# nkwangyh/CubemapSLAM

Hardware: AMD Instinct MI355X
Metric: frames/sec (extract+match+localBA) on Lafida cam0 (higher is better)
Workload: dtype u8 (extract/match), f64 (BA)

## Files before the change

cubemapslam_amd/api.py:

```python
import time
import ctypes as C
import os
import numpy as np

_HERE = os.path.dirname(os.path.abspath(__file__))
LIB_PATH = os.environ.get("CMS_HIP_LIB") or os.path.join(_HERE, "lib", "libcubemapslam_hip.so")


class CmsError(RuntimeError):
    pass


class Camera(C.Structure):
    _fields_ = [("c", C.c_double), ("d", C.c_double), ("e", C.c_double), ("u0", C.c_double), ("v0", C.c_double),
                ("invpol", C.c_double * 12), ("pol", C.c_double * 5), ("Iw", C.c_int), ("Ih", C.c_int),
                ("face", C.c_int), ("fov_deg", C.c_double)]


class OrbParams(C.Structure):
    _fields_ = [("nfeatures", C.c_int), ("scale_factor", C.c_float), ("nlevels", C.c_int),
                ("ini_th_fast", C.c_int), ("min_th_fast", C.c_int)]


class Geometry(C.Structure):
    _fields_ = [("W", C.c_int), ("F", C.c_int), ("nlevels", C.c_int), ("kp_cap", C.c_int), ("max_batch", C.c_int),
                ("level_w", C.c_int * 12), ("level_h", C.c_int * 12), ("level_quota", C.c_int * 12),
                ("level_cells", C.c_int * 12), ("scale", C.c_float * 12), ("inv_scale", C.c_float * 12),
                ("sigma2", C.c_float * 12), ("inv_sigma2", C.c_float * 12), ("pyramid_bytes_per_frame", C.c_size_t),
                ("candidate_entries_per_frame", C.c_size_t), ("fisheye_stride", C.c_int)]


class BaStats(C.Structure):
    _fields_ = [("iterations_done", C.c_int * 2), ("chi2_initial", C.c_double * 2), ("chi2_final", C.c_double * 2),
                ("lambda_final", C.c_double * 2), ("n_outliers_mid", C.c_int), ("n_outliers_final", C.c_int)]


KP_DTYPE = np.dtype([("x", "<f4"), ("y", "<f4"), ("size", "<f4"), ("angle", "<f4"), ("response", "<f4"),
                     ("octave", "<i4")])

_lib = None


def lib():
    global _lib
    if _lib is None:
        if not os.path.exists(LIB_PATH):
            raise CmsError("libcubemapslam_hip.so is missing -- build it with `python -m cubemapslam_amd.build` "
                           "(there is no CPU fallback)")
        L = C.CDLL(LIB_PATH)
        L.cms_last_error.restype = C.c_char_p
        for n in ("cms_ctx_stream", "cms_frames_input", "cms_ba_stream"):
            getattr(L, n).restype = C.c_void_p
            getattr(L, n).argtypes = [C.c_void_p]
        L.cms_ctx_create.argtypes = [C.c_void_p, C.c_int, C.c_void_p, C.c_void_p, C.c_int]
        L.cms_ctx_destroy.argtypes = [C.c_void_p]
        L.cms_ctx_destroy.restype = None
        L.cms_ctx_geometry.argtypes = [C.c_void_p, C.c_void_p]
        L.cms_remap.argtypes = [C.c_void_p, C.c_void_p, C.c_int, C.c_void_p, C.c_int]
        L.cms_set_mask.argtypes = [C.c_void_p, C.c_void_p, C.c_int]
        L.cms_extract.argtypes = [C.c_void_p, C.c_void_p, C.c_int, C.c_void_p, C.c_void_p, C.c_int, C.c_void_p]
        L.cms_remap_extract.argtypes = [C.c_void_p, C.c_void_p, C.c_int, C.c_void_p, C.c_void_p, C.c_int, C.c_void_p]
        L.cms_frames_upload.argtypes = [C.c_void_p, C.c_void_p, C.c_int, C.c_size_t, C.c_int]
        L.cms_frames_upload_async.argtypes = [C.c_void_p, C.c_void_p, C.c_int, C.c_size_t, C.c_int]
        L.cms_frames_upload_wait.argtypes = [C.c_void_p]
        L.cms_frames_upload_device.argtypes = [C.c_void_p, C.c_void_p, C.c_int]
        L.cms_frames_process_device.argtypes = [C.c_void_p, C.c_void_p, C.c_int]
        L.cms_host_alloc.argtypes = [C.c_void_p, C.c_size_t]
        L.cms_host_free.argtypes = [C.c_void_p]
        L.cms_host_free.restype = None
        L.cms_ba_profile_kernel.argtypes = [C.c_void_p, C.c_int]
        L.cms_ba_profile_get.argtypes = [C.c_void_p, C.c_void_p, C.c_void_p]
        L.cms_ba_debug_compose.argtypes = [C.c_int, C.c_void_p, C.c_int, C.c_int, C.c_void_p, C.c_void_p, C.c_int, C.c_void_p, C.c_void_p, C.c_void_p, C.c_void_p]
        L.cms_frames_process.argtypes = [C.c_void_p, C.c_int, C.c_int]
        L.cms_frames_sync.argtypes = [C.c_void_p]
        L.cms_frames_results.argtypes = [C.c_void_p, C.c_void_p, C.c_void_p, C.c_void_p]
        L.cms_frames_fetch.argtypes = [C.c_void_p, C.c_int, C.c_void_p, C.c_void_p, C.c_int, C.c_void_p]
        L.cms_debug_lut.argtypes = [C.c_void_p, C.c_void_p, C.c_void_p]
        L.cms_debug_cubemap.argtypes = [C.c_void_p, C.c_int, C.c_void_p, C.c_int]
        L.cms_debug_level.argtypes = [C.c_void_p, C.c_int, C.c_int, C.c_void_p, C.c_int]
        L.cms_debug_candidates.argtypes = [C.c_void_p, C.c_int, C.c_int, C.c_void_p, C.c_int, C.c_void_p]
        L.cms_debug_distributed.argtypes = [C.c_void_p, C.c_int, C.c_int, C.c_void_p, C.c_int, C.c_void_p]
        L.cms_profile_enable.argtypes = [C.c_void_p, C.c_int]
        L.cms_profile_get.argtypes = [C.c_void_p, C.c_void_p]
        L.cms_hamming_best2.argtypes = [C.c_void_p, C.c_void_p, C.c_int, C.c_void_p, C.c_int] + [C.c_void_p] * 9
        L.cms_hamming_best2_device.argtypes = [C.c_void_p, C.c_void_p, C.c_void_p, C.c_int] + [C.c_void_p] * 10
        L.cms_hamming_matrix.argtypes = [C.c_void_p, C.c_void_p, C.c_int, C.c_void_p, C.c_int, C.c_void_p]
        L.cms_ba_create.argtypes = [C.c_void_p, C.c_int, C.c_int, C.c_void_p, C.c_void_p, C.c_int, C.c_void_p, C.c_int,
                                    C.c_void_p, C.c_void_p, C.c_void_p, C.c_void_p, C.c_void_p, C.c_double, C.c_double,
                                    C.c_double, C.c_double]
        L.cms_ba_reset.argtypes = [C.c_void_p]
        L.cms_ba_optimize.argtypes = [C.c_void_p, C.c_int, C.c_int, C.c_void_p, C.c_void_p]
        L.cms_ba_read.argtypes = [C.c_void_p, C.c_void_p, C.c_void_p, C.c_void_p]
        L.cms_ba_destroy.argtypes = [C.c_void_p]
        L.cms_ba_destroy.restype = None
        L.cms_ba_run.argtypes = [C.c_int, C.c_int, C.c_void_p, C.c_void_p, C.c_int, C.c_void_p, C.c_int, C.c_void_p,
                                 C.c_void_p, C.c_void_p, C.c_void_p, C.c_void_p, C.c_double, C.c_double, C.c_double,
                                 C.c_double, C.c_int, C.c_int, C.c_void_p, C.c_void_p, C.c_void_p]
        L.cms_ba_linearize.argtypes = [C.c_int, C.c_int, C.c_void_p, C.c_void_p, C.c_int, C.c_void_p, C.c_int, C.c_void_p,
                                       C.c_void_p, C.c_void_p, C.c_void_p, C.c_void_p, C.c_double, C.c_double, C.c_double,
                                       C.c_double, C.c_int, C.c_double] + [C.c_void_p] * 7
        L.cms_area_set_keypoints.argtypes = [C.c_void_p, C.c_int, C.c_int, C.c_void_p]
        L.cms_area_grid.argtypes = [C.c_void_p, C.c_int]
        L.cms_features_in_area.argtypes = [C.c_void_p, C.c_int, C.c_int] + [C.c_void_p] * 7 + [C.c_int, C.c_void_p]
        L.cms_features_in_area_device.argtypes = [C.c_void_p, C.c_int, C.c_int] + [C.c_void_p] * 8 + [C.c_int, C.c_int, C.c_void_p]
        L.cms_features_in_area_batch_device.argtypes = [C.c_void_p, C.c_int] + [C.c_void_p] * 9 + [C.c_int, C.c_void_p]
        L.cms_area_set_descriptors.argtypes = [C.c_void_p, C.c_int, C.c_int, C.c_void_p]
        L.cms_search_local_points.argtypes = ([C.c_void_p, C.c_int, C.c_void_p, C.c_int] + [C.c_void_p] * 5 + [C.c_float] * 3 + [C.c_int, C.c_int] +
                                              [C.c_void_p] * 9)
        L.cms_search_by_projection.argtypes = ([C.c_void_p, C.c_int, C.c_void_p, C.c_int] + [C.c_void_p] * 5 + [C.c_float, C.c_int, C.c_int, C.c_int] +
                                               [C.c_void_p] * 3)
        L.cms_project_last_frame_device.argtypes = [C.c_void_p, C.c_int] + [C.c_void_p] * 5 + [C.c_float] + [C.c_void_p] * 5
        L.cms_rotation_filter_device.argtypes = [C.c_void_p, C.c_int] + [C.c_void_p] * 5 + [C.c_int]
        L.cms_is_in_frustum_device.argtypes = [C.c_void_p, C.c_int] + [C.c_void_p] * 6 + [C.c_float, C.c_float] + [C.c_void_p] * 8
        L.cms_search_local_points_device.argtypes = [C.c_void_p, C.c_int] + [C.c_void_p] * 5 + [C.c_float, C.c_int] + [C.c_void_p] * 3
        L.cms_create_new_map_points.argtypes = [C.c_void_p, C.c_int, C.c_void_p, C.c_void_p, C.c_void_p, C.c_int, C.c_int] + [C.c_void_p] * 5
        L.cms_kfstore_create.argtypes = [C.c_void_p, C.c_void_p, C.c_int, C.c_int, C.c_int]
        L.cms_kfstore_destroy.argtypes = [C.c_void_p]
        L.cms_kfstore_destroy.restype = None
        L.cms_kfstore_put.argtypes = [C.c_void_p, C.c_int, C.c_void_p]
        L.cms_kfstore_update.argtypes = [C.c_void_p, C.c_int] + [C.c_void_p] * 5
        L.cms_kfstore_fuse_search.argtypes = [C.c_void_p, C.c_int] + [C.c_void_p] * 8 + [C.c_float, C.c_void_p, C.c_void_p]
        L.cms_kfstore_fuse_search_sets.argtypes = [C.c_void_p, C.c_int] + [C.c_void_p] * 6 + [C.c_int] + [C.c_void_p] * 3 + [C.c_float, C.c_void_p, C.c_void_p]
        L.cms_kfstore_put_from_frame.argtypes = [C.c_void_p, C.c_int, C.c_void_p, C.c_int, C.c_int, C.c_void_p, C.c_void_p, C.c_void_p, C.c_float, C.c_void_p, C.c_int,
                                                 C.c_void_p, C.c_void_p, C.c_void_p]
        L.cms_kfstore_update_poses.argtypes = [C.c_void_p, C.c_int] + [C.c_void_p] * 4
        L.cms_kfstore_debug_fetch.argtypes = [C.c_void_p, C.c_int] + [C.c_void_p] * 12
        L.cms_ba_debug_fetch_plan.argtypes = [C.c_void_p] * 14
        L.cms_kfstore_create_new_map_points.argtypes = [C.c_void_p, C.c_int, C.c_void_p, C.c_void_p, C.c_void_p, C.c_int, C.c_int] + [C.c_void_p] * 5
        L.cms_distinctive_descriptors.argtypes = [C.c_void_p, C.c_int, C.c_void_p, C.c_void_p, C.c_void_p]
        L.cms_update_normal_and_depth.argtypes = [C.c_void_p, C.c_int] + [C.c_void_p] * 8
        L.cms_fuse_search.argtypes = [C.c_void_p, C.c_int, C.c_void_p, C.c_int] + [C.c_void_p] * 6 + [C.c_float, C.c_void_p, C.c_void_p]
        L.cms_pose_create.argtypes = [C.c_void_p, C.c_int, C.c_int, C.c_int]
        L.cms_pose_destroy.argtypes = [C.c_void_p]
        L.cms_pose_destroy.restype = None
        L.cms_pose_stream.argtypes = [C.c_void_p]
        L.cms_pose_stream.restype = C.c_void_p
        _edge = [C.c_void_p] * 5 + [C.c_double] * 4
        L.cms_pose_upload.argtypes = [C.c_void_p, C.c_int] + _edge + [C.c_void_p]
        L.cms_pose_launch.argtypes = [C.c_void_p]
        L.cms_pose_fetch.argtypes = [C.c_void_p, C.c_void_p, C.c_void_p, C.c_void_p, C.c_void_p]
        L.cms_pose_optimize_batch.argtypes = [C.c_void_p, C.c_int] + _edge + [C.c_void_p] * 4
        L.cms_pose_optimize.argtypes = [C.c_int, C.c_int] + [C.c_void_p] * 4 + [C.c_double] * 4 + [C.c_void_p] * 4
        _lib = L
    return _lib


def _p(a):
    if a is None:
        return None
    if isinstance(a, int):
        return C.c_void_p(a)
    return a.ctypes.data_as(C.c_void_p)


def _chk(rc, what):
    if rc < 0:
        raise CmsError("%s failed (%d): %s" % (what, rc, lib().cms_last_error().decode()))
    return rc


class _Handle:
    _entries = None

    def _create(self, *args, out_last=False):
        self.h = C.c_void_p()
        args = args + (C.byref(self.h),) if out_last else (C.byref(self.h),) + args
        _chk(getattr(lib(), self._entries[0])(*args), self._entries[0])

    def close(self):
        if getattr(self, "h", None):
            getattr(lib(), self._entries[1])(self.h)
            self.h = C.c_void_p()

    def __del__(self):
        try:
            self.close()
        except Exception:
            pass


def make_camera(d):
    cam = Camera()
    for k in ("c", "d", "e", "u0", "v0", "Iw", "Ih", "face", "fov_deg"):
        setattr(cam, k, d[k])
    for i in range(12):
        cam.invpol[i] = d["invpol"][i] if i < len(d["invpol"]) else 0.0
    for i in range(5):
        cam.pol[i] = d["pol"][i] if i < len(d["pol"]) else 0.0
    return cam


RT_DTYPE = np.dtype([(n, "<u2") for n in ("tx", "ty", "x0", "y0", "nd", "rows", "flags", "pad")])
RT_LDS_MAX = 32768


def remap_lut_host(cam):
    cam = make_camera(cam) if isinstance(cam, dict) else cam
    W = 3 * cam.face
    out = np.zeros((W, (W + 3) // 4 * 4), np.uint32)
    f = lib().cms_remap_lut_host
    f.argtypes = [C.c_void_p, C.c_void_p, C.c_int]
    _chk(f(C.byref(cam), _p(out), out.shape[1]), "cms_remap_lut_host")
    return out[:, :W]


def remap_tiles_host(cam, lut, tile_w, tile_h, lds_budget=RT_LDS_MAX):
    cam = make_camera(cam) if isinstance(cam, dict) else cam
    lut = np.ascontiguousarray(lut, np.uint32)
    W = 3 * cam.face
    cap = ((W + tile_w - 1) // tile_w) * ((W + tile_h - 1) // tile_h)
    out = np.zeros(cap, RT_DTYPE)
    n_live, n_all, lds = C.c_int(), C.c_int(), C.c_int()
    f = lib().cms_remap_tiles_host
    f.argtypes = [C.c_void_p, C.c_void_p] + [C.c_int] * 4 + [C.c_void_p, C.c_int] + [C.c_void_p] * 3
    _chk(f(C.byref(cam), _p(lut), lut.strides[0] // 4, tile_w, tile_h, lds_budget, _p(out), cap, C.byref(n_live), C.byref(n_all), C.byref(lds)),
         "cms_remap_tiles_host")
    return out[:n_all.value].copy(), n_live.value, lds.value


def fast_cells_host(cam, which, nfeatures=2000, scale_factor=1.2, nlevels=8, ini_th=20, min_th=7):
    cam = make_camera(cam) if isinstance(cam, dict) else cam
    orb = OrbParams(nfeatures, scale_factor, nlevels, ini_th, min_th)
    f = lib().cms_fast_cells_host
    f.argtypes = [C.c_void_p, C.c_void_p, C.c_int, C.c_void_p, C.c_int, C.c_void_p]
    n = C.c_int()
    _chk(f(C.byref(cam), C.byref(orb), which, None, 0, C.byref(n)), "cms_fast_cells_host")
    out = np.zeros(max(n.value, 1), np.int32)
    _chk(f(C.byref(cam), C.byref(orb), which, _p(out), len(out), C.byref(n)), "cms_fast_cells_host")
    out = out[:n.value]
    return out & 15, (out >> 4) & 255, (out >> 12) & 255


class Context(_Handle):
    _entries = ("cms_ctx_create", "cms_ctx_destroy")

    def __init__(self, cam, nfeatures=2000, scale_factor=1.2, nlevels=8, ini_th=20, min_th=7, max_batch=1, device=0):
        self.cam = make_camera(cam) if isinstance(cam, dict) else cam
        self.orb = OrbParams(nfeatures, scale_factor, nlevels, ini_th, min_th)
        self._create(device, C.byref(self.cam), C.byref(self.orb), max_batch)
        self.geom = Geometry()
        _chk(lib().cms_ctx_geometry(self.h, C.byref(self.geom)), "cms_ctx_geometry")
        self.W = self.geom.W
        self.max_batch = max_batch

    @property
    def stream(self):
        return lib().cms_ctx_stream(self.h)

    def set_mask(self, mask):
        mask = np.ascontiguousarray(mask, np.uint8)
        _chk(lib().cms_set_mask(self.h, _p(mask), mask.strides[0]), "cms_set_mask")

    def set_distance_bounds_mode(self, scaled):
        f = lib().cms_set_distance_bounds_mode
        f.argtypes = [C.c_void_p, C.c_int]
        _chk(f(self.h, int(scaled)), "cms_set_distance_bounds_mode")

    def set_gaussian_mode(self, column_mode):
        f = lib().cms_set_gaussian_mode
        f.argtypes = [C.c_void_p, C.c_int]
        _chk(f(self.h, int(column_mode)), "cms_set_gaussian_mode")

    def remap(self, fisheye, cubemap=None):
        fisheye = np.ascontiguousarray(fisheye, np.uint8)
        if cubemap is None:
            cubemap = np.zeros((self.W, self.W), np.uint8)
        _chk(lib().cms_remap(self.h, _p(fisheye), fisheye.strides[0], _p(cubemap), cubemap.strides[0]), "cms_remap")
        return cubemap

    def extract(self, cubemap, cap=None):
        cubemap = np.ascontiguousarray(cubemap, np.uint8)
        cap = cap or self.geom.kp_cap
        kps = np.zeros(cap, KP_DTYPE)
        desc = np.zeros((cap, 32), np.uint8)
        n = C.c_int()
        _chk(lib().cms_extract(self.h, _p(cubemap), cubemap.strides[0], _p(kps), _p(desc), cap, C.byref(n)), "cms_extract")
        return kps[:n.value].copy(), desc[:n.value].copy()

    def remap_extract(self, fisheye, cap=None):
        fisheye = np.ascontiguousarray(fisheye, np.uint8)
        cap = cap or self.geom.kp_cap
        kps = np.zeros(cap, KP_DTYPE)
        desc = np.zeros((cap, 32), np.uint8)
        n = C.c_int()
        _chk(lib().cms_remap_extract(self.h, _p(fisheye), fisheye.strides[0], _p(kps), _p(desc), cap, C.byref(n)), "cms_remap_extract")
        return kps[:n.value].copy(), desc[:n.value].copy()

    def remap_extract_rays(self, fisheye, cap=None):
        fisheye = np.ascontiguousarray(fisheye, np.uint8)
        cap = cap or self.geom.kp_cap
        kps = np.zeros(cap, KP_DTYPE); desc = np.zeros((cap, 32), np.uint8); rays = np.zeros((cap, 3), np.float32)
        n = C.c_int()
        _chk(lib().cms_remap_extract_rays(self.h, _p(fisheye), fisheye.strides[0], _p(kps), _p(desc), _p(rays), cap, C.byref(n)), "cms_remap_extract_rays")
        return kps[:n.value].copy(), desc[:n.value].copy(), rays[:n.value].copy()

    def fetch_rays(self, b):
        cap = self.geom.kp_cap
        rays = np.zeros((cap, 3), np.float32)
        n = C.c_int()
        _chk(lib().cms_frames_fetch_rays(self.h, b, _p(rays), cap, C.byref(n)), "cms_frames_fetch_rays")
        return rays[:n.value].copy()

    def rays_ptr(self):
        a = C.c_void_p()
        _chk(lib().cms_frames_rays(self.h, C.byref(a)), "cms_frames_rays")
        return a.value

    def upload(self, frames):
        frames = np.ascontiguousarray(frames, np.uint8)
        assert frames.ndim == 3
        _chk(lib().cms_frames_upload(self.h, _p(frames), frames.strides[1], frames.strides[0], frames.shape[0]), "cms_frames_upload")

    def upload_async(self, frames):
        assert frames.ndim == 3 and frames.dtype == np.uint8 and frames.flags.c_contiguous
        _chk(lib().cms_frames_upload_async(self.h, _p(frames), frames.strides[1], frames.strides[0], frames.shape[0]), "cms_frames_upload_async")

    def upload_device(self, d_ptr, B):
        _chk(lib().cms_frames_upload_device(self.h, C.c_void_p(int(d_ptr)), B), "cms_frames_upload_device")

    def process_device(self, d_ptr, B):
        _chk(lib().cms_frames_process_device(self.h, C.c_void_p(int(d_ptr)), B), "cms_frames_process_device")

    def stream_wait_extracted(self, hip_stream):
        f = lib().cms_stream_wait_extracted
        f.argtypes = [C.c_void_p, C.c_void_p]
        _chk(f(self.h, C.c_void_p(int(hip_stream))), "cms_stream_wait_extracted")

    def upload_wait(self):
        _chk(lib().cms_frames_upload_wait(self.h), "cms_frames_upload_wait")

    def process(self, B, from_fisheye=True):
        _chk(lib().cms_frames_process(self.h, B, 1 if from_fisheye else 0), "cms_frames_process")

    def sync(self):
        _chk(lib().cms_frames_sync(self.h), "cms_frames_sync")

    def fetch(self, b):
        cap = self.geom.kp_cap
        kps = np.zeros(cap, KP_DTYPE)
        desc = np.zeros((cap, 32), np.uint8)
        n = C.c_int()
        _chk(lib().cms_frames_fetch(self.h, b, _p(kps), _p(desc), cap, C.byref(n)), "cms_frames_fetch")
        return kps[:n.value].copy(), desc[:n.value].copy()

    def results_ptrs(self):
        a, b, c = C.c_void_p(), C.c_void_p(), C.c_void_p()
        _chk(lib().cms_frames_results(self.h, C.byref(a), C.byref(b), C.byref(c)), "cms_frames_results")
        return a.value, b.value, c.value

    def input_ptr(self):
        return lib().cms_frames_input(self.h)

    def profile(self, on=True):
        lib().cms_profile_enable(self.h, 1 if on else 0)

    def profile_ms(self):
        ms = np.zeros(7, np.float32)
        _chk(lib().cms_profile_get(self.h, _p(ms)), "cms_profile_get")
        return dict(zip(("remap", "pyramid", "fast", "octree", "cull", "describe", "total"), ms.tolist()))

    def debug_lut(self):
        W = self.W
        out = np.zeros((W, (W + 3) // 4 * 4), np.uint32)
        s = C.c_int()
        _chk(lib().cms_debug_lut(self.h, _p(out), C.byref(s)), "cms_debug_lut")
        return out[:, :W]

    def debug_level(self, b, l):
        w, h = self.geom.level_w[l], self.geom.level_h[l]
        out = np.zeros((h, w), np.uint8)
        _chk(lib().cms_debug_level(self.h, b, l, _p(out), w), "cms_debug_level")
        return out

    def debug_candidates(self, b, l):
        cap = self.geom.level_w[l] * self.geom.level_h[l] // 4 + 4096
        out = np.zeros((cap, 3), np.int32)
        n = C.c_int()
        _chk(lib().cms_debug_candidates(self.h, b, l, _p(out), cap, C.byref(n)), "cms_debug_candidates")
        return out[:n.value].copy()

    def debug_distributed(self, b, l):
        cap = self.geom.level_quota[l] + 8
        out = np.zeros((cap, 3), np.int32)
        n = C.c_int()
        _chk(lib().cms_debug_distributed(self.h, b, l, _p(out), cap, C.byref(n)), "cms_debug_distributed")
        return out[:n.value].copy()

    def hamming_best2(self, qdesc, tdesc, cand_off, cand_idx, tlevel=None, texcl=None):
        qdesc = np.ascontiguousarray(qdesc, np.uint8); tdesc = np.ascontiguousarray(tdesc, np.uint8)
        cand_off = np.ascontiguousarray(cand_off, np.int32); cand_idx = np.ascontiguousarray(cand_idx, np.int32)
        tl = np.ascontiguousarray(tlevel, np.int32) if tlevel is not None else None
        tx = np.ascontiguousarray(texcl, np.uint8) if texcl is not None else None
        nq = len(qdesc)
        outs = [np.zeros(max(nq, 1), np.int32) for _ in range(5)]
        _chk(lib().cms_hamming_best2(self.h, _p(qdesc), nq, _p(tdesc), len(tdesc), _p(cand_off), _p(cand_idx), _p(tl), _p(tx),
                                     *[_p(o) for o in outs]), "cms_hamming_best2")
        keys = ("best_idx", "best_dist", "best_level", "second_dist", "second_level")
        return {k: o[:nq] for k, o in zip(keys, outs)}

    def area_set_keypoints(self, b, kps):
        kps = np.ascontiguousarray(kps, KP_DTYPE)
        _chk(lib().cms_area_set_keypoints(self.h, b, len(kps), _p(kps)), "cms_area_set_keypoints")

    def area_grid(self, B):
        _chk(lib().cms_area_grid(self.h, B), "cms_area_grid")

    def features_in_area(self, b, qx, qy, qr, qmin, qmax, cap=None):
        qx = np.ascontiguousarray(qx, np.float32); qy = np.ascontiguousarray(qy, np.float32); qr = np.ascontiguousarray(qr, np.float32)
        qmin = np.ascontiguousarray(qmin, np.int32); qmax = np.ascontiguousarray(qmax, np.int32)
        nq = len(qx)
        cap = cap or max(1, 64 * nq + 1024)
        off = np.zeros(nq + 1, np.int32); idx = np.zeros(cap, np.int32); tot = C.c_int(0)
        _chk(lib().cms_features_in_area(self.h, b, nq, _p(qx), _p(qy), _p(qr), _p(qmin), _p(qmax), _p(off), _p(idx), cap, C.byref(tot)),
             "cms_features_in_area")
        return off, idx[:tot.value]

    def features_in_area_device(self, b, nq, d_q5, d_cnt, d_off, d_idx, cap, idx_base, d_total):
        _chk(lib().cms_features_in_area_device(self.h, b, nq, *[C.c_void_p(int(a)) for a in d_q5], C.c_void_p(int(d_cnt)), C.c_void_p(int(d_off)),
                                               C.c_void_p(int(d_idx)), cap, idx_base, C.c_void_p(int(d_total))), "cms_features_in_area_device")

    def features_in_area_batch_device(self, nq, d_qframe, d_q5, d_cnt, d_off, d_idx, cap, d_total):
        _chk(lib().cms_features_in_area_batch_device(self.h, nq, C.c_void_p(int(d_qframe)), *[C.c_void_p(int(a)) for a in d_q5], C.c_void_p(int(d_cnt)),
                                                     C.c_void_p(int(d_off)), C.c_void_p(int(d_idx)), cap, C.c_void_p(int(d_total))),
             "cms_features_in_area_batch_device")

    def area_set_descriptors(self, b, desc):
        desc = np.ascontiguousarray(desc, np.uint8)
        _chk(lib().cms_area_set_descriptors(self.h, b, len(desc), _p(desc)), "cms_area_set_descriptors")

    def search_local_points(self, b, pose15, pos, normal, min_dist, max_dist, mp_desc, kp_mp, viewing_cos_limit=0.5, th=1.0, nnratio=0.8,
                            th_high=100):
        pose15 = np.ascontiguousarray(pose15, np.float32).reshape(15)
        pos = np.ascontiguousarray(pos, np.float32).reshape(-1, 3); normal = np.ascontiguousarray(normal, np.float32).reshape(-1, 3)
        n = len(pos)
        min_dist = np.ascontiguousarray(min_dist, np.float32); max_dist = np.ascontiguousarray(max_dist, np.float32)
        mp_desc = np.ascontiguousarray(mp_desc, np.uint8).reshape(n, 32)
        assert kp_mp.dtype == np.int32 and kp_mp.flags.c_contiguous
        vis = np.zeros(n, np.uint8); px = np.zeros(n, np.float32); py = np.zeros(n, np.float32); lvl = np.zeros(n, np.int32)
        vc = np.zeros(n, np.float32); match = np.full(n, -1, np.int32)
        nm = C.c_int(0); rounds = C.c_int(0)
        _chk(lib().cms_search_local_points(self.h, b, _p(pose15), n, _p(pos), _p(normal), _p(min_dist), _p(max_dist), _p(mp_desc),
                                           viewing_cos_limit, th, nnratio, th_high, len(kp_mp), _p(kp_mp), _p(vis), _p(px), _p(py), _p(lvl),
                                           _p(vc), _p(match), C.addressof(nm), C.addressof(rounds)), "cms_search_local_points")
        return dict(in_view=vis, proj_x=px, proj_y=py, level=lvl, view_cos=vc, match=match, n_matches=nm.value, rounds=rounds.value)

    def search_by_projection(self, b, pose12, valid, Xw, octave, angle, mp_desc, kp_mp, th=15.0, check_ori=True, th_high=100):
        a = [np.ascontiguousarray(pose12, np.float32), np.ascontiguousarray(valid, np.uint8), np.ascontiguousarray(Xw, np.float32),
             np.ascontiguousarray(octave, np.int32), np.ascontiguousarray(angle, np.float32), np.ascontiguousarray(mp_desc, np.uint8)]
        n = len(a[1])
        match = np.full(n, -1, np.int32); nm = C.c_int(0)
        assert kp_mp.dtype == np.int32
        _chk(lib().cms_search_by_projection(self.h, b, _p(a[0]), n, *[_p(v) for v in a[1:]], th, int(check_ori), th_high, len(kp_mp), _p(kp_mp), _p(match),
                                            C.addressof(nm)), "cms_search_by_projection")
        return match, nm.value

    def search_by_projection_keyframe(self, b, pose12, kf_angle, pos, min_dist, max_dist, mp_desc, kp_mp, th=10.0, orb_dist=100, check_ori=True):
        a = [np.ascontiguousarray(pose12, np.float32).reshape(12), np.ascontiguousarray(kf_angle, np.float32), np.ascontiguousarray(pos, np.float32).reshape(-1, 3),
             np.ascontiguousarray(min_dist, np.float32), np.ascontiguousarray(max_dist, np.float32), np.ascontiguousarray(mp_desc, np.uint8).reshape(-1, 32)]
        n = len(a[1])
        assert all(len(v) == n for v in a[2:])
        assert kp_mp.dtype == np.int32 and kp_mp.flags.c_contiguous
        match = np.full(max(n, 1), -1, np.int32); nm = C.c_int(0)
        L = lib()
        L.cms_search_by_projection_keyframe.argtypes = ([C.c_void_p, C.c_int, C.c_void_p, C.c_int] + [C.c_void_p] * 5 + [C.c_float, C.c_int, C.c_int, C.c_int] +
                                                        [C.c_void_p] * 3)
        _chk(L.cms_search_by_projection_keyframe(self.h, b, _p(a[0]), n, *[_p(v) for v in a[1:]], float(th), int(orb_dist), int(check_ori), len(kp_mp), _p(kp_mp),
                                                 _p(match), C.addressof(nm)), "cms_search_by_projection_keyframe")
        return match[:n], nm.value

    def search_for_initialization(self, b2, k1, d1, prev_matched, window=100, nnratio=0.9, check_ori=True):
        k1 = np.ascontiguousarray(k1, KP_DTYPE); d1 = np.ascontiguousarray(d1, np.uint8)
        assert prev_matched.dtype == np.float32 and prev_matched.flags.c_contiguous and prev_matched.shape == (len(k1), 2)
        m12 = np.full(max(len(k1), 1), -1, np.int32); nm = C.c_int(0)
        f = lib().cms_search_for_initialization
        f.argtypes = [C.c_void_p, C.c_int, C.c_int, C.c_void_p, C.c_void_p, C.c_void_p, C.c_int, C.c_float, C.c_int, C.c_void_p, C.c_void_p]
        _chk(f(self.h, b2, len(k1), _p(k1), _p(d1), _p(prev_matched), int(window), float(nnratio), int(check_ori), _p(m12), C.addressof(nm)),
             "cms_search_for_initialization")
        return m12[:len(k1)], nm.value

    def project_last_frame_device(self, n, d_qframe, d_pose12, d_valid, d_Xw, d_oct, th, d_q5):
        v = lambda a: C.c_void_p(int(a)) if a else None
        _chk(lib().cms_project_last_frame_device(self.h, n, v(d_qframe), v(d_pose12), v(d_valid), v(d_Xw), v(d_oct), th, *[v(a) for a in d_q5]),
             "cms_project_last_frame_device")

    def rotation_filter_device(self, B, d_mp_off, d_last_angle, d_kp_mp, d_mp_match, d_n_matches, check_orientation=True):
        v = lambda a: C.c_void_p(int(a)) if a else None
        _chk(lib().cms_rotation_filter_device(self.h, B, v(d_mp_off), v(d_last_angle), v(d_kp_mp), v(d_mp_match), v(d_n_matches), int(check_orientation)),
             "cms_rotation_filter_device")

    def is_in_frustum_device(self, nmp, d_mp_frame, d_pose15, d_pos, d_normal, d_min, d_max, viewing_cos_limit, th, d_outs5, d_q3):
        v = lambda a: C.c_void_p(int(a)) if a else None
        _chk(lib().cms_is_in_frustum_device(self.h, nmp, v(d_mp_frame), v(d_pose15), v(d_pos), v(d_normal), v(d_min), v(d_max),
                                            viewing_cos_limit, th, *[v(a) for a in d_outs5], *[v(a) for a in d_q3]), "cms_is_in_frustum_device")

    def search_local_points_device(self, B, d_mp_off, d_mp_desc, d_cand_off, d_cand_idx, d_pair_dist, nnratio, th_high, d_kp_mp, d_mp_match,
                                   d_rounds=0):
        v = lambda a: C.c_void_p(int(a)) if a else None
        _chk(lib().cms_search_local_points_device(self.h, B, v(d_mp_off), v(d_mp_desc), v(d_cand_off), v(d_cand_idx), v(d_pair_dist), nnratio,
                                                  th_high, v(d_kp_mp), v(d_mp_match), v(d_rounds)), "cms_search_local_points_device")

    def hamming_best2_device(self, qdesc, q_row, nq, tdesc, cand_off, cand_idx, t_level, t_excl, outs):
        _chk(lib().cms_hamming_best2_device(self.h, _p(qdesc), _p(q_row), nq, _p(tdesc), _p(cand_off), _p(cand_idx), _p(t_level),
                                            _p(t_excl), *[_p(o) for o in outs]), "cms_hamming_best2_device")

    def hamming_matrix(self, a, b):
        a = np.ascontiguousarray(a, np.uint8); b = np.ascontiguousarray(b, np.uint8)
        out = np.zeros((len(a), len(b)), np.uint16)
        _chk(lib().cms_hamming_matrix(self.h, _p(a), len(a), _p(b), len(b), _p(out)), "cms_hamming_matrix")
        return out


    def compute_bow(self, vocab, rows, n, levelsup=4):
        rows = np.ascontiguousarray(rows, np.int32); n = np.ascontiguousarray(n, np.int32)
        assert len(rows) == len(n)
        L = lib()
        L.cms_frames_compute_bow.argtypes = [C.c_void_p, C.c_void_p, C.c_int, C.c_int, C.c_void_p, C.c_void_p]
        _chk(L.cms_frames_compute_bow(self.h, vocab.h, int(levelsup), len(rows), _p(rows), _p(n)), "cms_frames_compute_bow")

    def fetch_bow(self, b):
        L = lib()
        L.cms_frames_fetch_bow.argtypes = [C.c_void_p, C.c_int, C.c_void_p, C.c_void_p, C.c_void_p, C.c_int, C.c_void_p, C.c_void_p, C.c_void_p, C.c_void_p, C.c_int, C.c_int]
        nw, nn = C.c_int(), C.c_int()
        cap = self.geom.kp_cap
        o = _bow_arrays(cap, cap, cap)
        _chk(L.cms_frames_fetch_bow(self.h, b, C.byref(nw), _p(o["word_id"]), _p(o["word_val"]), len(o["word_id"]), C.byref(nn), _p(o["node_id"]), _p(o["node_off"]),
                                    _p(o["node_feat"]), len(o["node_id"]), cap), "cms_frames_fetch_bow")
        return _bow_trim(o, nw.value, nn.value)


class PinnedArray:

    def __init__(self, shape):
        n = int(np.prod(shape))
        self.p = C.c_void_p()
        _chk(lib().cms_host_alloc(C.byref(self.p), n), "cms_host_alloc")
        self.array = np.ctypeslib.as_array((C.c_uint8 * n).from_address(self.p.value)).reshape(shape)

    def close(self):
        if self.p:
            self.array = None
            lib().cms_host_free(self.p)
            self.p = None

    def __del__(self):
        try:
            self.close()
        except Exception:
            pass


class Keyframe(C.Structure):
    _fields_ = [("n", C.c_int), ("kps", C.c_void_p), ("desc", C.c_void_p), ("rays", C.c_void_p), ("mp", C.c_void_p),
                ("Rcw", C.c_float * 9), ("tcw", C.c_float * 3), ("Ow", C.c_float * 3),
                ("nnodes", C.c_int), ("node_id", C.c_void_p), ("node_off", C.c_void_p), ("node_feat", C.c_void_p), ("median_depth", C.c_float)]


def make_keyframe(kf):
    n = len(kf["x"])
    kps = np.zeros(n, KP_DTYPE); kps["x"] = kf["x"]; kps["y"] = kf["y"]; kps["octave"] = kf["octave"]; kps["angle"] = kf["angle"]
    keep = [kps, np.ascontiguousarray(kf["desc"], np.uint8), np.ascontiguousarray(kf["rays"], np.float32), np.ascontiguousarray(kf["mp"], np.int32),
            np.ascontiguousarray(kf["node_id"], np.int32), np.ascontiguousarray(kf["node_off"], np.int32), np.ascontiguousarray(kf["node_feat"], np.int32)]
    K = Keyframe()
    K.n = n; K.kps = keep[0].ctypes.data; K.desc = keep[1].ctypes.data; K.rays = keep[2].ctypes.data; K.mp = keep[3].ctypes.data
    K.Rcw[:] = [float(v) for v in np.asarray(kf["R"], np.float32).reshape(9)]
    K.tcw[:] = [float(v) for v in kf["t"]]; K.Ow[:] = [float(v) for v in kf["Ow"]]
    K.nnodes = len(keep[4]); K.node_id = keep[4].ctypes.data; K.node_off = keep[5].ctypes.data; K.node_feat = keep[6].ctypes.data
    K.median_depth = float(kf["median_depth"])
    return K, keep


def search_for_triangulation(ctx, K1, K2, E12=None, check_orientation=False):
    m = np.full(max(K1.n, 1), -1, np.int32)
    n = C.c_int()
    e = None if E12 is None else np.ascontiguousarray(E12, np.float32)
    lib().cms_search_for_triangulation.argtypes = [C.c_void_p, C.c_void_p, C.c_void_p, C.c_void_p, C.c_int, C.c_void_p, C.c_void_p]
    _chk(lib().cms_search_for_triangulation(ctx.h, C.byref(K1), C.byref(K2), _p(e) if e is not None else None, int(check_orientation), _p(m), C.byref(n)),
         "cms_search_for_triangulation")
    return m[:K1.n].copy(), n.value


def create_new_map_points(ctx, jobs, check_orientation=False, cap=None):
    nj = len(jobs)
    cur = (Keyframe * max(nj, 1))(*[j[0] for j in jobs])
    flat = [k for j in jobs for k in j[1]]
    neigh = (Keyframe * max(len(flat), 1))(*flat)
    off = np.concatenate([[0], np.cumsum([len(j[1]) for j in jobs])]).astype(np.int32)
    cap = cap if cap is not None else max([j[0].n for j in jobs] + [1])
    n_new = np.zeros(max(nj, 1), np.int32)
    on = np.zeros((max(nj, 1), cap), np.int32); o1 = np.zeros_like(on); o2 = np.zeros_like(on); ox = np.zeros((max(nj, 1), cap, 3), np.float32)
    _chk(lib().cms_create_new_map_points(ctx.h, nj, C.addressof(cur), _p(off), C.addressof(neigh), int(check_orientation), cap, _p(n_new), _p(on), _p(o1),
                                         _p(o2), _p(ox)), "cms_create_new_map_points")
    return [(on[j, :n_new[j]].copy(), o1[j, :n_new[j]].copy(), o2[j, :n_new[j]].copy(), ox[j, :n_new[j]].copy()) for j in range(nj)]


class BowJob(C.Structure):
    _fields_ = [("slot", C.c_int), ("b", C.c_int), ("n", C.c_int), ("nnodes", C.c_int), ("node_id", C.c_void_p), ("node_off", C.c_void_p),
                ("node_feat", C.c_void_p), ("kf_skip", C.c_void_p)]


class BowKfJob(C.Structure):
    _fields_ = [("slot1", C.c_int), ("n1", C.c_int), ("slot2", C.c_int), ("n2", C.c_int), ("skip1", C.c_void_p), ("skip2", C.c_void_p)]


class Sim3SearchJob(C.Structure):
    _fields_ = [("slot1", C.c_int), ("n1", C.c_int), ("slot2", C.c_int), ("n2", C.c_int), ("s12", C.c_float), ("R12", C.c_float * 9), ("t12", C.c_float * 3),
                ("off1", C.c_int), ("off2", C.c_int)]


class Sim3ProjJob(C.Structure):
    _fields_ = [("slot", C.c_int), ("n", C.c_int), ("Scw", C.c_float * 12), ("set", C.c_int)]


class KfProjJob(C.Structure):
    _fields_ = [("slot", C.c_int), ("b", C.c_int), ("n", C.c_int), ("pose12", C.c_float * 12), ("nmp", C.c_int), ("kf_feat", C.c_void_p), ("pos", C.c_void_p),
                ("min_dist", C.c_void_p), ("max_dist", C.c_void_p), ("mp_desc", C.c_void_p), ("kp_mp", C.c_void_p), ("match", C.c_void_p)]


class KfdbJob(C.Structure):
    _fields_ = [("mode", C.c_int), ("group", C.c_int), ("query", C.c_int), ("b", C.c_int), ("slot", C.c_int), ("nwords", C.c_int), ("word_id", C.c_void_p),
                ("word_val", C.c_void_p), ("min_score", C.c_float), ("n_connected", C.c_int), ("connected", C.c_void_p)]


KFDB_RELOC, KFDB_LOOP = 0, 1
KFDB_QUERY = {"row": 0, "slot": 1, "words": 2}


def kfdb_jobs(jobs):
    arr = (KfdbJob * max(len(jobs), 1))()
    keep = []
    for q, j in zip(arr, jobs):
        form = j["query"]
        q.mode = int(j["mode"]); q.group = int(j.get("group", 0)); q.query = KFDB_QUERY[form[0]]
        if form[0] == "row":
            q.b = int(form[1])
        elif form[0] == "slot":
            q.slot = int(form[1])
        else:
            ids = np.ascontiguousarray(form[1], np.int32); vals = np.ascontiguousarray(form[2], np.float64)
            assert len(ids) == len(vals)
            keep += [ids, vals]
            q.nwords = len(ids); q.word_id = ids.ctypes.data if len(ids) else None; q.word_val = vals.ctypes.data if len(ids) else None
        conn = np.ascontiguousarray(j.get("connected", ()), np.int32)
        keep.append(conn)
        q.min_score = float(j.get("min_score", 0.0)); q.n_connected = len(conn); q.connected = conn.ctypes.data if len(conn) else None
    return arr, keep


def kfdb_results(njobs, K, cap, cand, n_cand, common, score):
    return [([int(c) for c in cand[j, :min(int(n_cand[j]), cap)]], common[j].copy(), score[j].view(np.uint32).copy()) for j in range(njobs)]


def _bow_fv(fv):
# ... 1219 lines not shown
```

cubemapslam_amd/csrc/cms_api_area.hip:

```cpp
#include <vector>

static int cms_area_grid_attr(int device) {
  static bool done[64] = {false};
  return cms_lds_ceiling_once((const void*)k_area_grid, (CMS_AREA_MAXKP + 1) * 8, device, done);
}
static int cms_area_reserve(cms_ctx* c) {
  if (c->d_area_sorted) return CMS_OK;
  if (c->g.kp_cap > CMS_AREA_MAXKP) return cms_fail(CMS_ERR_UNSUPPORTED, "frame grid: more than 16383 key points per frame");
  { const int rca = cms_area_grid_attr(c->device); if (rca) return rca; }
  const size_t B = (size_t)c->max_batch;
  HIPCHK(hipMalloc((void**)&c->d_area_sorted, B * c->g.kp_cap * sizeof(uint16_t)));
  HIPCHK(hipMalloc((void**)&c->d_area_cell_start, B * (CMS_AREA_CELLS + 1) * sizeof(int)));
  HIPCHK(hipMalloc((void**)&c->d_area_nvalid, B * sizeof(int)));
  return CMS_OK;
}

static int cms_area_tmp_reserve(cms_ctx* c, int nq) {
  if ((size_t)nq <= c->area_tmp_cap) return CMS_OK;
  if (c->d_area_tmp) hipFree(c->d_area_tmp);
  c->d_area_tmp = nullptr; c->area_tmp_cap = 0;
  const size_t cap = (size_t)nq + (size_t)nq / 4 + 1024;
  HIPCHK(hipMalloc((void**)&c->d_area_tmp, cap * CMS_AREA_TMP * sizeof(int)));
  c->area_tmp_cap = cap;
  return CMS_OK;
}
static int cms_area_psum_reserve(cms_ctx* c, int nparts) {
  if (nparts <= c->area_psum_cap) return CMS_OK;
  if (c->d_area_psum) hipFree(c->d_area_psum);
  c->d_area_psum = nullptr; c->area_psum_cap = 0;
  const int cap = nparts + nparts / 4 + 64;
  HIPCHK(hipMalloc((void**)&c->d_area_psum, (size_t)cap * sizeof(int)));
  c->area_psum_cap = cap;
  return CMS_OK;
}

static CmsAreaArgs cms_area_args(const CmsKeyPoint* kp, const uint16_t* sorted_idx, const int* cell_start, int kp_cap, int F, float inv) {
  CmsAreaArgs a = {};
  a.kp = kp; a.sorted_idx = sorted_idx; a.cell_start = cell_start; a.kp_cap = kp_cap; a.F = F; a.inv = inv;
  return a;
}
static CmsAreaArgs cms_area_args_frames(const cms_ctx* c, int b) {
  return cms_area_args((const CmsKeyPoint*)c->d_kps + (size_t)b * c->g.kp_cap, c->d_area_sorted + (size_t)b * c->g.kp_cap,
                       c->d_area_cell_start + (size_t)b * (CMS_AREA_CELLS + 1), c->g.kp_cap, c->g.F, cms_grid_inv(c));
}
static void cms_area_queries(CmsAreaArgs& a, int nq, const void* q_frame, const void* qx, const void* qy, const void* qr, const void* qmin, const void* qmax,
                             void* cnt, void* off, void* idx, int cap, int idx_base) {
  a.nq = nq; a.q_frame = (const int*)q_frame;
  a.qx = (const float*)qx; a.qy = (const float*)qy; a.qr = (const float*)qr; a.qmin = (const int*)qmin; a.qmax = (const int*)qmax;
  a.cnt = (int*)cnt; a.off = (int*)off; a.idx = (int*)idx; a.cap = cap; a.idx_base = idx_base;
}
struct CmsWindowCols {
  size_t o0 = 0, stride = 0;
  float *qx, *qy, *qr; int *qmin, *qmax, *level, *slot, *rec, *cnt, *off, *idx;
  void take(CmsBlock& b, size_t E) {
    o0 = b.size; stride = cms_align(E * 4);
    for (int k = 0; k < 9; ++k) b.take(E * 4);
    b.take(E * 4, 4);
  }
  void at(uint8_t* p, size_t o_idx) {
    float* f = (float*)(p + o0); int* i = (int*)(p + o0);
    const size_t n = stride / 4;
    qx = f; qy = f + n; qr = f + 2 * n; qmin = i + 3 * n; qmax = i + 4 * n; level = i + 5 * n; slot = i + 6 * n; rec = i + 7 * n; cnt = i + 8 * n; off = i + 9 * n;
    idx = (int*)(p + o_idx);
  }
};
static void cms_area_queries(CmsAreaArgs& a, int nq, const CmsWindowCols& w, int cap) {
  cms_area_queries(a, nq, w.slot, w.qx, w.qy, w.qr, w.qmin, w.qmax, w.cnt, w.off, w.idx, cap, 0);
}
static int cms_area_launch(cms_ctx* c, hipStream_t s, CmsAreaArgs a, void* d_total) {
  const int nq = a.nq, qgrid = cms_area_search_grid(nq);
  int rc = cms_area_psum_reserve(c, qgrid);
  if (rc) return rc;
  rc = cms_area_tmp_reserve(c, nq);
  if (rc) return rc;
  a.tmp = c->d_area_tmp; a.psum = c->d_area_psum;
  hipLaunchKernelGGL(k_area_query, dim3(qgrid), dim3(CMS_AREA_QT), 0, s, a);
  hipLaunchKernelGGL(k_area_lists, dim3(cms_area_tile_grid(nq)), dim3(CMS_AREA_LT), 0, s, a, (int*)d_total);
  HIPCHK(hipGetLastError());
  return CMS_OK;
}

extern "C" int cms_area_set_keypoints(cms_ctx* c, int b, int n, const cms_keypoint* kps) {
  if (!c || b < 0 || b >= c->max_batch || n < 0 || n > c->g.kp_cap || (n > 0 && !kps)) return cms_fail(CMS_ERR_ARG, "cms_area_set_keypoints: bad argument");
  HIPCHK(hipSetDevice(c->device));
  if (n > 0) HIPCHK(hipMemcpyAsync(c->d_kps + (size_t)b * c->g.kp_cap, kps, (size_t)n * sizeof(cms_keypoint), hipMemcpyHostToDevice, c->stream));
  HIPCHK(hipMemcpyAsync(c->d_kp_cnt + b, &n, sizeof(int), hipMemcpyHostToDevice, c->stream));
  HIPCHK(hipStreamSynchronize(c->stream));
  return CMS_OK;
}

extern "C" int cms_area_grid(cms_ctx* c, int B) {
  if (!c || B < 1 || B > c->max_batch) return cms_fail(CMS_ERR_ARG, "cms_area_grid: bad batch");
  HIPCHK(hipSetDevice(c->device));
  int rc = cms_area_reserve(c);
  if (rc) return rc;
  hipLaunchKernelGGL(k_area_grid, dim3(B), dim3(1024), (size_t)(c->g.kp_cap + 1) * 8, c->stream, (const CmsKeyPoint*)c->d_kps, (const int*)c->d_kp_cnt, c->g.kp_cap, c->g.F, cms_grid_inv(c),
                     c->d_area_sorted, c->d_area_cell_start, c->d_area_nvalid);
  HIPCHK(hipGetLastError());
  c->area_frames = B;
  return CMS_OK;
}

extern "C" int cms_features_in_area_device(cms_ctx* c, int b, int nq, const void* d_qx, const void* d_qy, const void* d_qr, const void* d_qmin,
                                           const void* d_qmax, void* d_cnt_scratch, void* d_cand_off, void* d_cand_idx, int cap, int idx_base,
                                           void* d_total) {
  if (!c || b < 0 || b >= c->area_frames || nq < 0 || cap < 0) return cms_fail(CMS_ERR_ARG, "cms_features_in_area_device: bad argument (cms_area_grid first)");
  if (nq == 0) return CMS_OK;
  HIPCHK(hipSetDevice(c->device));
  CmsAreaArgs a = cms_area_args_frames(c, b);
  cms_area_queries(a, nq, nullptr, d_qx, d_qy, d_qr, d_qmin, d_qmax, d_cnt_scratch, d_cand_off, d_cand_idx, cap, idx_base);
  return cms_area_launch(c, c->stream, a, d_total);
}

extern "C" int cms_features_in_area_batch_device(cms_ctx* c, int nq, const void* d_qframe, const void* d_qx, const void* d_qy, const void* d_qr,
                                                 const void* d_qmin, const void* d_qmax, void* d_cnt_scratch, void* d_cand_off, void* d_cand_idx,
                                                 int cap, void* d_total) {
  if (!c || nq < 0 || cap < 0 || c->area_frames < 1 || !d_qframe) return cms_fail(CMS_ERR_ARG, "cms_features_in_area_batch_device: bad argument (cms_area_grid first)");
  if (nq == 0) return CMS_OK;
  HIPCHK(hipSetDevice(c->device));
  CmsAreaArgs a = cms_area_args_frames(c, 0);
  cms_area_queries(a, nq, d_qframe, d_qx, d_qy, d_qr, d_qmin, d_qmax, d_cnt_scratch, d_cand_off, d_cand_idx, cap, 0);
  return cms_area_launch(c, c->stream, a, d_total);
}

extern "C" int cms_features_in_area(cms_ctx* c, int b, int nq, const float* qx, const float* qy, const float* qr, const int* qmin, const int* qmax,
                                    int* cand_off, int* cand_idx, int cap, int* total) {
  if (!c || nq < 0 || cap < 0 || !cand_off || (nq > 0 && (!qx || !qy || !qr || !qmin || !qmax))) return cms_fail(CMS_ERR_ARG, "cms_features_in_area: bad argument");
  if (b < 0 || b >= c->area_frames) return cms_fail(CMS_ERR_ARG, "cms_features_in_area: no grid for this frame (cms_area_grid first)");
  cand_off[0] = 0;
  if (total) *total = 0;
  if (nq == 0) return CMS_OK;
  HIPCHK(hipSetDevice(c->device));
  const size_t qb = (size_t)nq * 4;
  const size_t bytes = 5 * qb + qb  + (qb + 4)  + (size_t)cap * 4 + 64;
  hipStream_t s = c->stream;
  int rc = c->stage.reserve(s, bytes, 0);
  if (rc) return rc;
  uint8_t* p = c->stage.d;
  void* dq[5];
  const void* hq[5] = {qx, qy, qr, qmin, qmax};
  for (int i = 0; i < 5; ++i) { dq[i] = p; p += qb; HIPCHK(hipMemcpyAsync(dq[i], hq[i], qb, hipMemcpyHostToDevice, s)); }
  void* d_cnt = p; p += qb;
  void* d_off = p; p += qb + 4;
  void* d_tot = p; p += 16;
  void* d_idx = p;
  rc = cms_features_in_area_device(c, b, nq, dq[0], dq[1], dq[2], dq[3], dq[4], d_cnt, d_off, d_idx, cap, 0, d_tot);
  if (rc) return rc;
  int tot = 0;
  HIPCHK(hipMemcpyAsync(cand_off, d_off, qb + 4, hipMemcpyDeviceToHost, s));
  HIPCHK(hipMemcpyAsync(&tot, d_tot, sizeof(int), hipMemcpyDeviceToHost, s));
  HIPCHK(hipStreamSynchronize(s));
  if (total) *total = tot;
  if (tot > cap) return cms_fail(CMS_ERR_OVERFLOW, "cms_features_in_area: candidate capacity too small");
  if (tot > 0 && cand_idx) HIPCHK(hipMemcpy(cand_idx, d_idx, (size_t)tot * 4, hipMemcpyDeviceToHost));
  return CMS_OK;
}
```

cubemapslam_amd/csrc/cms_api_frames.hip:

```cpp
#include <chrono>
#include <thread>
#include <hip/hip_runtime.h>
#include <math.h>
#include <stdio.h>
#include <stdlib.h>
#include <string.h>
#include <algorithm>
#include <string>
#include <vector>
#include "../../include/cubemapslam_hip.h"
#include "cms_types.h"
#include "cms_stage.h"
#include "orb_pattern.inc"

static bool cms_cu_mask_from_env(uint32_t* words, int* n_words) {
  const char* v = getenv("CMS_CTX_CU_MASK");
  if (!v || !*v) return false;
  int n = 0;
  while (*v && n < 8) {
    char* end = nullptr;
    words[n++] = (uint32_t)strtoul(v, &end, 16);
    if (end == v) return false;
    v = *end == ',' ? end + 1 : end;
    if (*end && *end != ',') return false;
  }
  *n_words = n;
  return n > 0;
}

struct CmsCtxBow;
static void cms_ctx_bow_free(CmsCtxBow* b);
static void cms_ctx_bow_invalidate(CmsCtxBow* b);

struct CmsHipMem;
using CmsStage = CmsStageT<CmsHipMem>;

static thread_local std::string g_cms_err;
static int cms_fail(int code, const char* what, hipError_t e = hipSuccess) {
  char buf[512];
  if (e != hipSuccess) snprintf(buf, sizeof(buf), "%s: %s", what, hipGetErrorString(e));
  else snprintf(buf, sizeof(buf), "%s", what);
  g_cms_err = buf;
  return code;
}
#define HIPCHK(call)                                                        \
  do {                                                                      \
    hipError_t _e = (call);                                                 \
    if (_e != hipSuccess) return cms_fail(CMS_ERR_HIP, #call, _e);          \
  } while (0)

extern "C" const char* cms_last_error(void) { return g_cms_err.c_str(); }
extern "C" int cms_device_count(void) {
  int n = 0;
  if (hipGetDeviceCount(&n) != hipSuccess) return 0;
  return n;
}

struct cms_ctx {
  int device = 0;
  cms_camera cam;
  cms_orb_params orb;
  int max_batch = 0;
  CmsGeom g;
  float scale[CMS_MAX_LEVELS], inv_scale[CMS_MAX_LEVELS], sigma2[CMS_MAX_LEVELS], inv_sigma2[CMS_MAX_LEVELS];
  hipStream_t stream = nullptr;
  int fstride = 0;
  size_t fish_pitch = 0;
  int lut_stride = 0, mstride = 0;
  bool have_mask = false;
  int dirty_frames = 0;
  uint8_t* d_fish = nullptr; uint32_t* d_lut = nullptr; uint8_t* d_pyr = nullptr; uint8_t* d_mask = nullptr;
  cms_remap_tile* d_rtiles = nullptr; int rt_mode = 1, rt_tw = 64, rt_live = 0, rt_all = 0, rt_lds = 0;
  CmsResizeTab* d_tab = nullptr; float* d_pattern = nullptr;
  uint32_t* d_cand = nullptr; uint16_t* d_node = nullptr; int* d_cand_cnt = nullptr; int* d_overflow = nullptr;
  uint32_t* d_qt_out = nullptr; int* d_qt_cnt = nullptr;
  uint32_t* d_cell_cand = nullptr; int* d_cell_cnt = nullptr;
  int* d_cells_all = nullptr; int* d_cells_live = nullptr; int n_cells_all = 0, n_cells_live = 0;
  uint16_t* d_area_sorted = nullptr; int* d_area_cell_start = nullptr; int* d_area_nvalid = nullptr; int area_frames = 0;
  int* d_area_psum = nullptr; int area_psum_cap = 0;
  int* d_area_tmp = nullptr; size_t area_tmp_cap = 0;
  uint8_t* h_fish_stage = nullptr; int fish_stage_frames = 0;
  hipStream_t copy_stream = nullptr; hipEvent_t ev_upload_done = nullptr, ev_remap_done = nullptr;
  bool upload_pending = false, remap_recorded = false;
  int dist_bounds_scaled = 0;
  hipEvent_t ev_block = nullptr; int last_batch = 0;
  hipEvent_t ev_extracted = nullptr; bool extracted_recorded = false;
  CmsKeyPoint* d_kps = nullptr; uint32_t* d_aux = nullptr; uint8_t* d_desc = nullptr; int* d_kp_cnt = nullptr;
  uint32_t* d_order = nullptr; uint32_t* d_aux_sorted = nullptr; int* d_walk_cnt = nullptr; float* d_rays = nullptr;
  CmsStage stage;
  bool prof = false;
  bool desc_spatial = false;
  hipEvent_t ev[8] = {nullptr, nullptr, nullptr, nullptr, nullptr, nullptr, nullptr, nullptr};
  size_t fast_lds = 0, qt_lds = 0;
  CmsCtxBow* bow = nullptr;
};

static inline double cms_horner12(const double* c, double x) {
  double r = 0.0;
  for (int i = 11; i >= 0; --i) r = r * x + c[i];
  return r;
}
static void cms_cubemap_to_fisheye(const cms_camera& cam, double up, double vp, double* uf, double* vf) {
  const int F = cam.face;
  const double half = F / 2.0;
  float i = (float)up, j = (float)vp;
  *uf = -1; *vf = -1;
  const float fi = i / (float)F, fj = j / (float)F;
  int face = CMS_FACE_UNKNOWN;
  if (fi >= 0 && fi < 1 && fj >= 1 && fj < 2) face = CMS_FACE_LEFT;
  else if (fi >= 1 && fi < 2 && fj >= 0 && fj < 1) face = CMS_FACE_UPPER;
  else if (fi >= 1 && fi < 2 && fj >= 1 && fj < 2) face = CMS_FACE_FRONT;
  else if (fi >= 1 && fi < 2 && fj >= 2 && fj < 3) face = CMS_FACE_LOWER;
  else if (fi >= 2 && fi < 3 && fj >= 1 && fj < 2) face = CMS_FACE_RIGHT;
  if (face == CMS_FACE_UNKNOWN) return;
  i = i - (float)((int)(i / (float)F) * F);
  j = j - (float)((int)(j / (float)F) * F);
  const double lx = ((double)i - half) * 1.0 / half, ly = ((double)j - half) * 1.0 / half, lz = 1.0;
  double x, y, z;
  switch (face) {
    case CMS_FACE_FRONT: x = lx; y = ly; z = lz; break;
    case CMS_FACE_LEFT: x = -lz; y = ly; z = lx; break;
    case CMS_FACE_RIGHT: x = lz; y = ly; z = -lx; break;
    case CMS_FACE_LOWER: x = lx; y = lz; z = -ly; break;
    default: x = lx; y = -lz; z = ly; break;
  }
  double norm = sqrt(x * x + y * y);
  if (norm == 0.0) norm = 1e-14;
  const double theta = atan(-z / norm);
  const double rho = cms_horner12(cam.invpol, theta);
  const double uu = x / norm * rho, vv = y / norm * rho;
  *uf = uu * cam.c + vv * cam.d + cam.u0;
  *vf = uu * cam.e + vv + cam.v0;
  if (*uf < 0 || *uf >= cam.Iw || *vf < 0 || *vf >= cam.Ih) { *uf = -1; *vf = -1; }
}
static void cms_build_lut(const cms_camera& cam, int lut_stride, std::vector<uint32_t>& lut) {
  const int W = 3 * cam.face;
  lut.assign((size_t)W * lut_stride, 0u);
  for (int y = 0; y < W; ++y)
    for (int x = 0; x < W; ++x) {
      double u, v;
      cms_cubemap_to_fisheye(cam, (double)x, (double)y, &u, &v);
      if (u < 0 || v < 0 || u >= cam.Iw || v >= cam.Ih) continue;
      const float mu = (float)u, mv = (float)v;
      const int sx = (int)lrint((double)(mu * 32.f)), sy = (int)lrint((double)(mv * 32.f));
      const uint32_t X = (uint32_t)(sx >> 5), Y = (uint32_t)(sy >> 5), ax = (uint32_t)(sx & 31), ay = (uint32_t)(sy & 31);
      lut[(size_t)y * lut_stride + x] = X | (Y << 11) | (ax << 22) | (ay << 27);
    }
}

extern "C" int cms_remap_lut_host(const cms_camera* cam, uint32_t* lut, int lut_stride) {
  if (!cam || !lut || cam->face < 1 || lut_stride < 3 * cam->face) return cms_fail(CMS_ERR_ARG, "cms_remap_lut_host: bad argument");
  std::vector<uint32_t> v;
  cms_build_lut(*cam, lut_stride, v);
  memcpy(lut, v.data(), v.size() * 4);
  return CMS_OK;
}
extern "C" int cms_remap_tiles_host(const cms_camera* cam, const uint32_t* lut, int lut_stride, int tile_w, int tile_h, int lds_budget,
                                    cms_remap_tile* out, int cap, int* n_live, int* n_all, int* lds_bytes) {
  if (!cam || !lut || !out || !n_live || !n_all || !lds_bytes || cam->face < 1 || lut_stride < 3 * cam->face || !cms_rt_shape_ok(tile_w, tile_h) || lds_budget < 0)
    return cms_fail(CMS_ERR_ARG, "cms_remap_tiles_host: bad argument");
  std::vector<cms_remap_tile> v;
  cms_rt_build(cam->face, lut, lut_stride, tile_w, tile_h, lds_budget, v, n_live, lds_bytes);
  *n_all = (int)v.size();
  if ((int)v.size() > cap) return cms_fail(CMS_ERR_OVERFLOW, "cms_remap_tiles_host: caller capacity too small");
  memcpy(out, v.data(), v.size() * sizeof(cms_remap_tile));
  return CMS_OK;
}

static inline short cms_sat_short(float v) {
  const long iv = lrint((double)v);
  return (short)(iv < -32768 ? -32768 : iv > 32767 ? 32767 : iv);
}
static void cms_resize_table(int sn, int dn, bool clamp_frac, CmsResizeTab* out) {
  const double inv_scale = (double)dn / sn, scale = 1. / inv_scale;
  for (int d = 0; d < dn; ++d) {
    float f = (float)((d + 0.5) * scale - 0.5);
    int s = (int)floorf(f);
    f -= s;
    if (clamp_frac) {
      if (s < 0) { f = 0; s = 0; }
      if (s >= sn - 1) { f = 0; s = sn - 1; }
    }
    out[d].s = (short)s;
    out[d].a0 = cms_sat_short((1.f - f) * 2048);
    out[d].a1 = cms_sat_short(f * 2048);
    out[d].pad = 0;
  }
}

#include "cms_api_util.h"

struct CmsLevelSetup {
  float scale[CMS_MAX_LEVELS], inv_scale[CMS_MAX_LEVELS], sigma2[CMS_MAX_LEVELS], inv_sigma2[CMS_MAX_LEVELS];
  size_t tab_off = 0;
  int maxq = 0, wCellMax = 0, hCellMax = 0;
};
static int cms_level_geometry(const cms_camera* cam, const cms_orb_params* orb, CmsGeom& g, CmsLevelSetup* x) {
  if (orb->nlevels < 1 || orb->nlevels > CMS_MAX_LEVELS) return cms_fail(CMS_ERR_UNSUPPORTED, "nlevels must be 1..12");
  if (cam->face < 32 || 3 * cam->face > 4095) return cms_fail(CMS_ERR_UNSUPPORTED, "face size must satisfy 32 <= F and 3F <= 4095");
  memset(&g, 0, sizeof(g));
  const int L = orb->nlevels, F = cam->face, W = 3 * F;
  float *scale = x->scale, *inv_scale = x->inv_scale, *sigma2 = x->sigma2, *inv_sigma2 = x->inv_sigma2;
  g.nlevels = L; g.W = W; g.F = F; g.ini_th = orb->ini_th_fast; g.min_th = orb->min_th_fast;
  const double scaleFactor = orb->scale_factor;
  scale[0] = 1.0f; sigma2[0] = 1.0f;
  for (int i = 1; i < L; ++i) { scale[i] = (float)(scale[i - 1] * scaleFactor); sigma2[i] = scale[i] * scale[i]; }
  for (int i = 0; i < L; ++i) { inv_scale[i] = 1.0f / scale[i]; inv_sigma2[i] = 1.0f / sigma2[i]; }
  {
    const float factor = (float)(1.0f / scaleFactor);
    float nDesired = orb->nfeatures * (1 - factor) / (1 - (float)pow((double)factor, (double)L));
    int sum = 0;
    for (int l = 0; l < L - 1; ++l) { g.lv[l].quota = (int)lrint((double)nDesired); sum += g.lv[l].quota; nDesired *= factor; }
    g.lv[L - 1].quota = orb->nfeatures - sum > 0 ? orb->nfeatures - sum : 0;
  }
  size_t off = 0, cand_off = 0; size_t& tab_off = x->tab_off;
  int cell0 = 0, kp_off = 0; int &maxq = x->maxq, &wCellMax = x->wCellMax, &hCellMax = x->hCellMax;
  for (int l = 0; l < L; ++l) {
    CmsLevel& lv = g.lv[l];
    lv.w = (int)lrint((double)((float)W * inv_scale[l]));
    lv.h = lv.w;
    if (lv.w < 2 * CMS_MINB + 30) { return cms_fail(CMS_ERR_UNSUPPORTED, "pyramid level too small for the FAST cell grid"); }
    lv.stride = (int)cms_align((size_t)lv.w + 8, 128);
    lv.off = off;
    off += cms_align((size_t)lv.stride * (lv.h + 1), 256);
    const float width = (float)(lv.w - 2 * CMS_MINB), height = (float)(lv.h - 2 * CMS_MINB);
    lv.nCols = (int)(width / 30.f); lv.nRows = (int)(height / 30.f);
    lv.wCell = (int)ceilf(width / lv.nCols); lv.hCell = (int)ceilf(height / lv.nRows);
    lv.cell0 = cell0; cell0 += lv.nCols * lv.nRows;
    lv.cand_cap = (lv.w * lv.h) / 4 + 4096;
    lv.cand_off = cand_off; cand_off += cms_align((size_t)lv.cand_cap, 64);
    lv.kp_off = kp_off; kp_off += lv.quota + 3;
    lv.scale = scale[l];
    lv.patch_size = (float)(int)(31 * scale[l]);
    lv.tab_off = tab_off; tab_off += (size_t)lv.w + lv.h;
    if (lv.quota > maxq) maxq = lv.quota;
    if (lv.wCell > wCellMax) wCellMax = lv.wCell;
    if (lv.hCell > hCellMax) hCellMax = lv.hCell;
// ... 742 lines not shown
```

cubemapslam_amd/csrc/cms_api_reloc.hip:

```cpp
#include <algorithm>
#include <cstring>
#include <vector>

namespace {
int reloc_run(cms_ctx* c, cms_kfstore* st, int njobs, const cms_kfproj_job* jobs, const float* kf_angle, float th, int orb_dist, int check_orientation,
              int* n_matches, const char* who) {
  const int kp_cap = c->g.kp_cap;
  std::vector<int> mp_off((size_t)njobs + 1, 0);
  for (int j = 0; j < njobs; ++j) mp_off[(size_t)j + 1] = mp_off[(size_t)j] + jobs[j].nmp;
  const int n = mp_off[(size_t)njobs];
  for (int j = 0; j < njobs; ++j) n_matches[j] = 0;
  if (n == 0) return CMS_OK;
  if (c->g.nlevels > 16) return cms_fail(CMS_ERR_UNSUPPORTED, "SearchByProjection (key frame): more than 16 pyramid levels");
  HIPCHK(hipSetDevice(c->device));
  hipStream_t s = c->stream;
  if (st) {
    const int rc = kfstore_wait_puts(st, s, njobs, [&](int j) { return jobs[j].slot; });
    if (rc) return rc;
  }
  const size_t n4 = (size_t)n * 4, j4 = (size_t)njobs * 4, kp4 = (size_t)kp_cap * 4;
  CmsBlock blk;
  const size_t o_pose = blk.take(12 * j4), o_jframe = blk.take(j4), o_jkp0 = blk.take(j4), o_mpoff = blk.take(j4, 4), o_ptjob = blk.take(n4), o_feat = blk.take(n4),
               o_pos = blk.take(3 * n4), o_min = blk.take(n4), o_max = blk.take(n4), o_desc = blk.take((size_t)n * 32), o_kpmp = blk.take(njobs * kp4);
  const size_t in_bytes = blk.size;
  const size_t o_match = blk.take(n4), o_nm = blk.take(j4), o_tot = blk.take(16);
  const size_t out_begin = o_kpmp, out_end = blk.size;
  const size_t o_qf = blk.take(n4), o_qx = blk.take(n4), o_qy = blk.take(n4), o_qr = blk.take(n4), o_qmin = blk.take(n4), o_qmax = blk.take(n4), o_ang = blk.take(n4),
               o_cnt = blk.take(n4), o_off = blk.take(n4, 4);
  const size_t o_idx = blk.size;
  return cms_retry_capacity(64 * n + 1024, who, [&](int cap, int& tot) -> int {
    const size_t o_pd = o_idx + cms_align((size_t)cap * 4);
    int rc = c->stage.reserve(s, o_pd + cms_align((size_t)cap * 2), out_end);
    if (rc) return rc;
    uint8_t* p = c->stage.d;
    uint8_t* h = c->stage.h;
    std::memcpy(h + o_mpoff, mp_off.data(), j4 + 4);
    for (int j = 0; j < njobs; ++j) {
      const cms_kfproj_job& q = jobs[j];
      const size_t m0 = (size_t)mp_off[(size_t)j], m = (size_t)q.nmp;
      std::memcpy(h + o_pose + 48 * (size_t)j, q.pose12, 48);
      reinterpret_cast<int*>(h + o_jframe)[j] = q.b;
      reinterpret_cast<int*>(h + o_jkp0)[j] = st ? st->h_kf[(size_t)q.slot].f0 : -1;
      int* km = reinterpret_cast<int*>(h + o_kpmp) + (size_t)j * kp_cap;
      for (int k = 0; k < kp_cap; ++k) km[k] = k < q.n ? q.kp_mp[k] : -1;
      if (m == 0) continue;
      int* pj = reinterpret_cast<int*>(h + o_ptjob) + m0;
      for (size_t k = 0; k < m; ++k) pj[k] = j;
      std::memcpy(h + o_feat + 4 * m0, st ? (const void*)q.kf_feat : (const void*)kf_angle, 4 * m);
      std::memcpy(h + o_pos + 12 * m0, q.pos, 12 * m); std::memcpy(h + o_min + 4 * m0, q.min_dist, 4 * m); std::memcpy(h + o_max + 4 * m0, q.max_dist, 4 * m);
      std::memcpy(h + o_desc + 32 * m0, q.mp_desc, 32 * m);
    }
    rc = c->stage.up(s, in_bytes, who);
    if (rc) return rc;
    CmsProjectKfArgs a = {};
    a.n = n; a.pt_job = (const int*)(p + o_ptjob); a.pose12 = (const float*)(p + o_pose); a.job_frame = (const int*)(p + o_jframe); a.job_kp0 = (const int*)(p + o_jkp0);
    a.kf_kp = st ? st->d_kp : nullptr; a.kf_feat = (const int*)(p + o_feat); a.kf_angle = (const float*)(p + o_feat);
    a.pos = (const float*)(p + o_pos); a.min_dist = (const float*)(p + o_min); a.max_dist = (const float*)(p + o_max);
    a.th = th; a.cos_fov = cms_cos_fov(c); a.log_scale = cms_log_scale(c); a.nlevels = c->g.nlevels; a.F = c->g.F;
    a.bounds_scaled = c->dist_bounds_scaled;
    cms_level_table(a.sf, c, c->scale, 0.0f);
    a.q_frame = (int*)(p + o_qf); a.qx = (float*)(p + o_qx); a.qy = (float*)(p + o_qy); a.qr = (float*)(p + o_qr); a.qmin = (int*)(p + o_qmin); a.qmax = (int*)(p + o_qmax);
    a.angle = (float*)(p + o_ang);
    hipLaunchKernelGGL(k_project_keyframe, dim3((n + 255) / 256), dim3(256), 0, s, a);
    HIPCHK(hipGetLastError());
    rc = cms_features_in_area_batch_device(c, n, p + o_qf, p + o_qx, p + o_qy, p + o_qr, p + o_qmin, p + o_qmax, p + o_cnt, p + o_off, p + o_idx, cap, p + o_tot);
    if (rc) return rc;
    CmsSearchLocalArgs g = track_search_local_args(c, p + o_mpoff, p + o_desc, p + o_off, p + o_idx, p + o_pd, (int*)(p + o_kpmp), p + o_match, nullptr, -1.0f, orb_dist, 0,
                                                   p + o_tot, cap);
    g.wg_frame = (const int*)(p + o_jframe);
    hipLaunchKernelGGL(k_search_local, dim3(njobs), dim3(1024), 0, s, g);
    CmsRotFilterArgs r = {};
    r.mp_off = g.mp_off; r.last_angle = (const float*)(p + o_ang); r.kp = g.kp; r.kp_mp = g.kp_mp; r.mp_match = g.mp_match; r.n_matches = (int*)(p + o_nm);
    r.check_orientation = check_orientation; r.total = g.total; r.cap = cap; r.wg_frame = g.wg_frame; r.kp_cap = kp_cap;
    hipLaunchKernelGGL(k_rot_filter, dim3(njobs), dim3(1024), 0, s, r);
    HIPCHK(hipGetLastError());
    rc = c->stage.back_and_wait(s, out_begin, out_end, who);
    if (rc) return rc;
    tot = *reinterpret_cast<const int*>(h + o_tot);
    if (tot > cap) return CMS_OK;
    for (int j = 0; j < njobs; ++j) {
      const cms_kfproj_job& q = jobs[j];
      if (q.nmp == 0) continue;
      const int* km = reinterpret_cast<const int*>(h + o_kpmp) + (size_t)j * kp_cap;
      const int* rows = reinterpret_cast<const int*>(h + o_match) + mp_off[(size_t)j];
      if (q.n > 0) std::memcpy(q.kp_mp, km, (size_t)q.n * 4);
      track_rows_to_frame(c, q.b, q.nmp, rows, q.match);
      for (int k = 0; k < q.nmp; ++k) if (q.match[k] >= 0 && q.match[k] < q.n) q.kp_mp[q.match[k]] = k;
      n_matches[j] = reinterpret_cast<const int*>(h + o_nm)[j];
    }
    return CMS_OK;
  });
}
int reloc_check_job(const cms_ctx* c, const cms_kfproj_job& q, const char* who) {
  if (q.b < 0 || q.b >= c->area_frames) return cms_fail(CMS_ERR_ARG, (std::string(who) + ": no grid for this frame (cms_area_grid first)").c_str());
  if (q.n < 0 || q.n > c->g.kp_cap || q.nmp < 0 || (q.n > 0 && !q.kp_mp) || (q.nmp > 0 && (!q.pos || !q.min_dist || !q.max_dist || !q.mp_desc || !q.match)))
    return cms_fail(CMS_ERR_ARG, (std::string(who) + ": bad argument").c_str());
  return CMS_OK;
}
}

extern "C" int cms_kfstore_search_by_projection(cms_kfstore* st, cms_ctx* src, int njobs, const cms_kfproj_job* jobs, float th, int orb_dist, int check_orientation,
                                                int* n_matches) {
  const char* who = "cms_kfstore_search_by_projection";
  if (!st || !src || njobs < 0 || (njobs > 0 && (!jobs || !n_matches))) return cms_fail(CMS_ERR_ARG, "cms_kfstore_search_by_projection: bad argument");
  if (njobs == 0) return CMS_OK;
  if (src->device != st->c->device) return cms_fail(CMS_ERR_ARG, "cms_kfstore_search_by_projection: the frame context and the store must share the device");
  if (src->g.kp_cap > CMS_TRACK_KPMAX) return cms_fail(CMS_ERR_UNSUPPORTED, "cms_kfstore_search_by_projection: more than 4096 key points per frame");
  std::vector<uint8_t> row_named((size_t)std::max(src->area_frames, 1), 0);
  for (int j = 0; j < njobs; ++j) {
    const cms_kfproj_job& q = jobs[j];
    if (q.slot < 0 || q.slot >= st->maxkf || !st->used[(size_t)q.slot]) return cms_fail(CMS_ERR_ARG, "cms_kfstore_search_by_projection: empty slot");
    const int rc = reloc_check_job(src, q, who);
    if (rc) return rc;
    if (row_named[(size_t)q.b]) return cms_fail(CMS_ERR_ARG, "cms_kfstore_search_by_projection: two jobs name the same frame row");
    row_named[(size_t)q.b] = 1;
    if (q.nmp > 0 && !q.kf_feat) return cms_fail(CMS_ERR_ARG, "cms_kfstore_search_by_projection: bad argument");
    const int kn = st->h_kf[(size_t)q.slot].n;
    for (int k = 0; k < q.nmp; ++k) {
      if (q.kf_feat[k] < 0 || q.kf_feat[k] >= kn) return cms_fail(CMS_ERR_ARG, "cms_kfstore_search_by_projection: key-frame feature index out of range");
      if (k > 0 && q.kf_feat[k] <= q.kf_feat[k - 1]) return cms_fail(CMS_ERR_ARG, "cms_kfstore_search_by_projection: key-frame feature indices must ascend");
    }
  }
  return reloc_run(src, st, njobs, jobs, nullptr, th, orb_dist, check_orientation, n_matches, who);
}

extern "C" int cms_search_by_projection_keyframe(cms_ctx* c, int b, const float* pose12, int nmp, const float* kf_angle, const float* pos, const float* min_dist,
                                                 const float* max_dist, const uint8_t* mp_desc, float th, int orb_dist, int check_orientation, int nkp, int* kp_mp,
                                                 int* match, int* n_matches) {
  const char* who = "cms_search_by_projection_keyframe";
  if (!c || !pose12 || (nmp > 0 && !kf_angle)) return cms_fail(CMS_ERR_ARG, "cms_search_by_projection_keyframe: bad argument");
  if (c->g.kp_cap > CMS_TRACK_KPMAX) return cms_fail(CMS_ERR_UNSUPPORTED, "cms_search_by_projection_keyframe: more than 4096 key points per frame");
  cms_kfproj_job q = {};
  q.slot = -1; q.b = b; q.n = nkp; std::memcpy(q.pose12, pose12, 48); q.nmp = nmp; q.pos = pos; q.min_dist = min_dist; q.max_dist = max_dist; q.mp_desc = mp_desc; q.kp_mp = kp_mp; q.match = match;
  const int rc = reloc_check_job(c, q, who);
  if (rc) return rc;
  int nm = 0;
  const int rr = reloc_run(c, nullptr, 1, &q, kf_angle, th, orb_dist, check_orientation, &nm, who);
  if (n_matches) *n_matches = nm;
  return rr;
}
```

cubemapslam_amd/csrc/cms_api_track.hip:

```cpp
#include <cmath>
#include <vector>

extern "C" int cms_area_set_descriptors(cms_ctx* c, int b, int n, const uint8_t* desc) {
  if (!c || b < 0 || b >= c->max_batch || n < 0 || n > c->g.kp_cap || (n > 0 && !desc)) return cms_fail(CMS_ERR_ARG, "cms_area_set_descriptors: bad argument");
  HIPCHK(hipSetDevice(c->device));
  if (n > 0) HIPCHK(hipMemcpyAsync(c->d_desc + (size_t)b * c->g.kp_cap * 32, desc, (size_t)n * 32, hipMemcpyHostToDevice, c->stream));
  HIPCHK(hipStreamSynchronize(c->stream));
  return CMS_OK;
}

extern "C" int cms_set_distance_bounds_mode(cms_ctx* c, int scaled) {
  if (!c || scaled < 0 || scaled > 1) return cms_fail(CMS_ERR_ARG, "cms_set_distance_bounds_mode: mode must be 0 or 1");
  c->dist_bounds_scaled = scaled;
  return CMS_OK;
}

extern "C" int cms_is_in_frustum_device(cms_ctx* c, int nmp, const void* d_mp_frame, const void* d_pose15, const void* d_pos, const void* d_normal,
                                        const void* d_min_dist, const void* d_max_dist, float viewing_cos_limit, float th, void* d_in_view,
                                        void* d_proj_x, void* d_proj_y, void* d_level, void* d_view_cos, void* d_qr, void* d_qmin, void* d_qmax) {
  if (!c || nmp < 0 || (nmp > 0 && (!d_pose15 || !d_pos || !d_normal || !d_min_dist || !d_max_dist || !d_in_view || !d_proj_x || !d_proj_y ||
                                    !d_level || !d_view_cos)) || (d_qr && (!d_qmin || !d_qmax)))
    return cms_fail(CMS_ERR_ARG, "cms_is_in_frustum_device: bad argument");
  if (nmp == 0) return CMS_OK;
  if (c->g.nlevels > 16) return cms_fail(CMS_ERR_UNSUPPORTED, "cms_is_in_frustum_device: more than 16 pyramid levels");
  HIPCHK(hipSetDevice(c->device));
  CmsFrustumArgs a;
  a.pose15 = (const float*)d_pose15; a.mp_frame = (const int*)d_mp_frame; a.n = nmp;
  a.P = (const float*)d_pos; a.normal = (const float*)d_normal; a.min_dist = (const float*)d_min_dist; a.max_dist = (const float*)d_max_dist;
  a.viewing_cos_limit = viewing_cos_limit; a.th = th; a.bounds_scaled = c->dist_bounds_scaled;
  a.log_scale = cms_log_scale(c);
  a.nlevels = c->g.nlevels; a.F = c->g.F;
  cms_level_table(a.sf, c, c->scale, 0.0f);
  a.in_view = (uint8_t*)d_in_view; a.proj_x = (float*)d_proj_x; a.proj_y = (float*)d_proj_y; a.level = (int*)d_level; a.view_cos = (float*)d_view_cos;
  a.qr = (float*)d_qr; a.qmin = (int*)d_qmin; a.qmax = (int*)d_qmax;
  hipLaunchKernelGGL(k_in_frustum, dim3((nmp + 255) / 256), dim3(256), 0, c->stream, a);
  HIPCHK(hipGetLastError());
  return CMS_OK;
}

static CmsSearchLocalArgs track_search_local_args(const cms_ctx* c, const void* mp_off, const void* mp_desc, const void* cand_off, const void* cand_idx, void* pair_dist,
                                                  int* kp_mp, void* mp_match, void* rounds, float nnratio, int th_high, int frame0, const void* total, int cap) {
  CmsSearchLocalArgs a = {};
  a.mp_off = (const int*)mp_off; a.mp_desc = (const uint4*)mp_desc; a.cand_off = (const int*)cand_off; a.cand_idx = (const int*)cand_idx;
  a.t_desc = (const uint4*)c->d_desc; a.kp = (const CmsKeyPoint*)c->d_kps; a.kp_cap = c->g.kp_cap;
  a.pair_dist = (uint16_t*)pair_dist; a.kp_mp = kp_mp; a.mp_match = (int*)mp_match; a.rounds = (int*)rounds;
  a.nnratio = nnratio; a.th_high = th_high; a.frame0 = frame0; a.total = (const int*)total; a.cap = cap;
  return a;
}

extern "C" int cms_search_local_points_device(cms_ctx* c, int B, const void* d_mp_off, const void* d_mp_desc, const void* d_cand_off,
                                              const void* d_cand_idx, void* d_pair_dist, float nnratio, int th_high, void* d_kp_mp,
                                              void* d_mp_match, void* d_rounds) {
  if (!c || B < 1 || B > c->area_frames || !d_mp_off || !d_mp_desc || !d_cand_off || !d_cand_idx || !d_pair_dist || !d_kp_mp || !d_mp_match)
    return cms_fail(CMS_ERR_ARG, "cms_search_local_points_device: bad argument (cms_area_grid first)");
  if (c->g.kp_cap > CMS_TRACK_KPMAX) return cms_fail(CMS_ERR_UNSUPPORTED, "cms_search_local_points_device: more than 4096 key points per frame");
  HIPCHK(hipSetDevice(c->device));
  const CmsSearchLocalArgs a = track_search_local_args(c, d_mp_off, d_mp_desc, d_cand_off, d_cand_idx, d_pair_dist, (int*)d_kp_mp, d_mp_match, d_rounds, nnratio, th_high, 0, nullptr, 0);
  hipLaunchKernelGGL(k_search_local, dim3(B), dim3(1024), 0, c->stream, a);
  HIPCHK(hipGetLastError());
  return CMS_OK;
}

static void track_stage_one_frame(const cms_ctx* c, uint8_t* h, size_t o_qf, size_t o_mpoff, size_t o_kpmp, int b, int n, int nkp, const int* kp_mp) {
  { int* qf = reinterpret_cast<int*>(h + o_qf); for (int i = 0; i < n; ++i) qf[i] = b; }
  { int* mo = reinterpret_cast<int*>(h + o_mpoff); mo[0] = 0; mo[1] = n; }
  { int* km = reinterpret_cast<int*>(h + o_kpmp); for (int k = 0; k < c->g.kp_cap; ++k) km[k] = k < nkp ? kp_mp[k] : -1; }
}
static int* track_kp_mp_of_frame(const cms_ctx* c, uint8_t* p, size_t o_kpmp, int b) { return (int*)(p + o_kpmp) - (size_t)b * c->g.kp_cap; }
static int track_rows_to_frame(const cms_ctx* c, int b, int n, const int* rows, int* match) {
  int nm = 0;
  for (int i = 0; i < n; ++i) { match[i] = rows[i] >= 0 ? rows[i] - b * c->g.kp_cap : -1; nm += rows[i] >= 0; }
  return nm;
}

extern "C" int cms_search_local_points(cms_ctx* c, int b, const float* pose15, int nmp, const float* pos, const float* normal,
                                       const float* min_dist, const float* max_dist, const uint8_t* mp_desc, float viewing_cos_limit, float th,
                                       float nnratio, int th_high, int nkp, int* kp_mp, uint8_t* in_view, float* proj_x, float* proj_y,
                                       int* level, float* view_cos, int* mp_match, int* n_matches, int* rounds) {
  if (!c || !pose15 || nmp < 0 || nkp < 0 || nkp > (c ? c->g.kp_cap : 0) || (nmp > 0 && (!pos || !normal || !min_dist || !max_dist || !mp_desc || !mp_match)) ||
      (nkp > 0 && !kp_mp))
    return cms_fail(CMS_ERR_ARG, "cms_search_local_points: bad argument");
  if (b < 0 || b >= c->area_frames) return cms_fail(CMS_ERR_ARG, "cms_search_local_points: no grid for this frame (cms_area_grid first)");
  if (c->g.kp_cap > CMS_TRACK_KPMAX) return cms_fail(CMS_ERR_UNSUPPORTED, "cms_search_local_points: more than 4096 key points per frame");
  if (n_matches) *n_matches = 0;
  if (rounds) *rounds = 0;
  if (nmp == 0) return CMS_OK;
  HIPCHK(hipSetDevice(c->device));
  hipStream_t s = c->stream;
  const size_t n4 = (size_t)nmp * 4, kp4 = (size_t)c->g.kp_cap * 4;
  CmsBlock blk;
  const size_t o_pose = blk.take(64), o_pos = blk.take(3 * n4), o_nrm = blk.take(3 * n4), o_min = blk.take(n4), o_max = blk.take(n4), o_desc = blk.take((size_t)nmp * 32),
               o_qf = blk.take(n4), o_mpoff = blk.take(16), o_kpmp = blk.take(kp4);
  const size_t in_bytes = blk.size;
  const size_t o_vis = blk.take(nmp), o_px = blk.take(n4), o_py = blk.take(n4), o_lvl = blk.take(n4), o_vc = blk.take(n4), o_match = blk.take(n4), o_tot = blk.take(16),
               o_rounds = blk.take(16);
  const size_t out_begin = o_kpmp, out_end = blk.size;
  const size_t o_qr = blk.take(n4), o_qmin = blk.take(n4), o_qmax = blk.take(n4), o_cnt = blk.take(n4), o_off = blk.take(n4, 4);
  const size_t o_idx = blk.size;
  return cms_retry_capacity(64 * nmp + 1024, "cms_search_local_points", [&](int cap, int& tot) -> int {
    const size_t o_pd = o_idx + cms_align((size_t)cap * 4);
    int rc = c->stage.reserve(s, o_pd + cms_align((size_t)cap * 2), out_end);
    if (rc) return rc;
    uint8_t* p = c->stage.d;
    uint8_t* h = c->stage.h;
    memcpy(h + o_pose, pose15, 60);
    memcpy(h + o_pos, pos, 3 * n4); memcpy(h + o_nrm, normal, 3 * n4); memcpy(h + o_min, min_dist, n4); memcpy(h + o_max, max_dist, n4);
    memcpy(h + o_desc, mp_desc, (size_t)nmp * 32);
    track_stage_one_frame(c, h, o_qf, o_mpoff, o_kpmp, b, nmp, nkp, kp_mp);
    rc = c->stage.up(s, in_bytes, "cms_search_local_points");
    if (rc) return rc;
    rc = cms_is_in_frustum_device(c, nmp, nullptr, p + o_pose, p + o_pos, p + o_nrm, p + o_min, p + o_max, viewing_cos_limit, th, p + o_vis,
                                  p + o_px, p + o_py, p + o_lvl, p + o_vc, p + o_qr, p + o_qmin, p + o_qmax);
    if (rc) return rc;
    rc = cms_features_in_area_batch_device(c, nmp, p + o_qf, p + o_px, p + o_py, p + o_qr, p + o_qmin, p + o_qmax, p + o_cnt, p + o_off, p + o_idx,
                                           cap, p + o_tot);
    if (rc) return rc;
    const CmsSearchLocalArgs a = track_search_local_args(c, p + o_mpoff, p + o_desc, p + o_off, p + o_idx, p + o_pd, track_kp_mp_of_frame(c, p, o_kpmp, b), p + o_match,
                                                         p + o_rounds, nnratio, th_high, b, p + o_tot, cap);
    hipLaunchKernelGGL(k_search_local, dim3(1), dim3(1024), 0, s, a);
    HIPCHK(hipGetLastError());
    rc = c->stage.back_and_wait(s, out_begin, out_end, "cms_search_local_points");
    if (rc) return rc;
    tot = *reinterpret_cast<const int*>(h + o_tot);
    if (tot > cap) return CMS_OK;
    if (nkp > 0) memcpy(kp_mp, h + o_kpmp, (size_t)nkp * 4);
    if (in_view) memcpy(in_view, h + o_vis, nmp);
    if (proj_x) memcpy(proj_x, h + o_px, n4);
    if (proj_y) memcpy(proj_y, h + o_py, n4);
    if (level) memcpy(level, h + o_lvl, n4);
    if (view_cos) memcpy(view_cos, h + o_vc, n4);
    const int nm = track_rows_to_frame(c, b, nmp, reinterpret_cast<const int*>(h + o_match), mp_match);
    if (n_matches) *n_matches = nm;
    if (rounds) *rounds = *reinterpret_cast<const int*>(h + o_rounds);
    return CMS_OK;
  });
}

extern "C" int cms_project_last_frame_device(cms_ctx* c, int n, const void* d_qframe, const void* d_pose12, const void* d_valid, const void* d_Xw,
                                             const void* d_oct, float th, void* d_qx, void* d_qy, void* d_qr, void* d_qmin, void* d_qmax) {
  if (!c || n < 0 || (n > 0 && (!d_pose12 || !d_valid || !d_Xw || !d_oct || !d_qx || !d_qy || !d_qr || !d_qmin || !d_qmax)))
    return cms_fail(CMS_ERR_ARG, "cms_project_last_frame_device: bad argument");
  if (n == 0) return CMS_OK;
  HIPCHK(hipSetDevice(c->device));
  CmsProjectLastArgs a;
  a.pose12 = (const float*)d_pose12; a.q_frame = (const int*)d_qframe; a.n = n; a.valid = (const uint8_t*)d_valid; a.Xw = (const float*)d_Xw;
  a.oct = (const int*)d_oct; a.th = th; a.F = c->g.F;
  a.cos_fov = cms_cos_fov(c);
  cms_level_table(a.sf, c, c->scale, 0.0f);
  a.qx = (float*)d_qx; a.qy = (float*)d_qy; a.qr = (float*)d_qr; a.qmin = (int*)d_qmin; a.qmax = (int*)d_qmax;
  hipLaunchKernelGGL(k_project_last, dim3((n + 255) / 256), dim3(256), 0, c->stream, a);
  HIPCHK(hipGetLastError());
  return CMS_OK;
}
extern "C" int cms_rotation_filter_device(cms_ctx* c, int B, const void* d_mp_off, const void* d_last_angle, void* d_kp_mp, void* d_mp_match,
                                          void* d_n_matches, int check_orientation) {
  if (!c || B < 1 || !d_mp_off || !d_last_angle || !d_kp_mp || !d_mp_match) return cms_fail(CMS_ERR_ARG, "cms_rotation_filter_device: bad argument");
  HIPCHK(hipSetDevice(c->device));
  CmsRotFilterArgs a = {};
  a.mp_off = (const int*)d_mp_off; a.last_angle = (const float*)d_last_angle; a.kp = (const CmsKeyPoint*)c->d_kps; a.kp_mp = (int*)d_kp_mp;
  a.mp_match = (int*)d_mp_match; a.n_matches = (int*)d_n_matches; a.check_orientation = check_orientation; a.total = nullptr; a.cap = 0;
  hipLaunchKernelGGL(k_rot_filter, dim3(B), dim3(1024), 0, c->stream, a);
  HIPCHK(hipGetLastError());
  return CMS_OK;
}

extern "C" int cms_search_by_projection(cms_ctx* c, int b, const float* pose12, int nlast, const uint8_t* valid, const float* Xw, const int* octave,
                                        const float* angle, const uint8_t* mp_desc, float th, int check_orientation, int th_high, int nkp, int* kp_mp,
                                        int* match, int* n_matches) {
  if (!c || !pose12 || nlast < 0 || nkp < 0 || nkp > (c ? c->g.kp_cap : 0) || (nlast > 0 && (!valid || !Xw || !octave || !angle || !mp_desc || !match)) ||
      (nkp > 0 && !kp_mp))
    return cms_fail(CMS_ERR_ARG, "cms_search_by_projection: bad argument");
  if (b < 0 || b >= c->area_frames) return cms_fail(CMS_ERR_ARG, "cms_search_by_projection: no grid for this frame (cms_area_grid first)");
  if (c->g.kp_cap > CMS_TRACK_KPMAX) return cms_fail(CMS_ERR_UNSUPPORTED, "cms_search_by_projection: more than 4096 key points per frame");
  if (n_matches) *n_matches = 0;
  if (nlast == 0) return CMS_OK;
  for (int i = 0; i < nlast; ++i)
    if (valid[i] && (octave[i] < 0 || octave[i] >= c->g.nlevels)) return cms_fail(CMS_ERR_ARG, "cms_search_by_projection: octave out of range");
  HIPCHK(hipSetDevice(c->device));
  hipStream_t s = c->stream;
  const size_t n4 = (size_t)nlast * 4, kp4 = (size_t)c->g.kp_cap * 4;
  CmsBlock blk;
  const size_t o_pose = blk.take(64), o_valid = blk.take(nlast), o_xw = blk.take(3 * n4), o_oct = blk.take(n4), o_ang = blk.take(n4), o_desc = blk.take((size_t)nlast * 32),
               o_qf = blk.take(n4), o_mpoff = blk.take(16), o_kpmp = blk.take(kp4);
  const size_t in_bytes = blk.size;
  const size_t o_match = blk.take(n4), o_nm = blk.take(16), o_tot = blk.take(16);
  const size_t out_begin = o_kpmp, out_end = blk.size;
  const size_t o_qx = blk.take(n4), o_qy = blk.take(n4), o_qr = blk.take(n4), o_qmin = blk.take(n4), o_qmax = blk.take(n4), o_cnt = blk.take(n4), o_off = blk.take(n4, 4);
  const size_t o_idx = blk.size;
  return cms_retry_capacity(64 * nlast + 1024, "cms_search_by_projection", [&](int cap, int& tot) -> int {
    const size_t o_pd = o_idx + cms_align((size_t)cap * 4);
    int rc = c->stage.reserve(s, o_pd + cms_align((size_t)cap * 2), out_end);
    if (rc) return rc;
    uint8_t* p = c->stage.d;
    uint8_t* h = c->stage.h;
    memcpy(h + o_pose, pose12, 48);
    memcpy(h + o_valid, valid, nlast); memcpy(h + o_xw, Xw, 3 * n4); memcpy(h + o_oct, octave, n4); memcpy(h + o_ang, angle, n4);
    memcpy(h + o_desc, mp_desc, (size_t)nlast * 32);
    track_stage_one_frame(c, h, o_qf, o_mpoff, o_kpmp, b, nlast, nkp, kp_mp);
    rc = c->stage.up(s, in_bytes, "cms_search_by_projection");
    if (rc) return rc;
    rc = cms_project_last_frame_device(c, nlast, nullptr, p + o_pose, p + o_valid, p + o_xw, p + o_oct, th, p + o_qx, p + o_qy, p + o_qr, p + o_qmin, p + o_qmax);
    if (rc) return rc;
    rc = cms_features_in_area_batch_device(c, nlast, p + o_qf, p + o_qx, p + o_qy, p + o_qr, p + o_qmin, p + o_qmax, p + o_cnt, p + o_off, p + o_idx, cap, p + o_tot);
    if (rc) return rc;
    const CmsSearchLocalArgs a = track_search_local_args(c, p + o_mpoff, p + o_desc, p + o_off, p + o_idx, p + o_pd, track_kp_mp_of_frame(c, p, o_kpmp, b), p + o_match,
                                                         nullptr, -1.0f, th_high, b, p + o_tot, cap);
    hipLaunchKernelGGL(k_search_local, dim3(1), dim3(1024), 0, s, a);
    CmsRotFilterArgs r = {};
    r.mp_off = a.mp_off; r.last_angle = (const float*)(p + o_ang); r.kp = a.kp; r.kp_mp = a.kp_mp;
    r.mp_match = a.mp_match; r.n_matches = (int*)(p + o_nm); r.check_orientation = check_orientation; r.total = a.total; r.cap = cap;
    hipLaunchKernelGGL(k_rot_filter, dim3(1), dim3(1024), 0, s, r);
    HIPCHK(hipGetLastError());
    rc = c->stage.back_and_wait(s, out_begin, out_end, "cms_search_by_projection");
    if (rc) return rc;
    tot = *reinterpret_cast<const int*>(h + o_tot);
    if (tot > cap) return CMS_OK;
    if (nkp > 0) memcpy(kp_mp, h + o_kpmp, (size_t)nkp * 4);
    track_rows_to_frame(c, b, nlast, reinterpret_cast<const int*>(h + o_match), match);
    if (n_matches) *n_matches = *reinterpret_cast<const int*>(h + o_nm);
    return CMS_OK;
  });
}

extern "C" int cms_search_for_initialization(cms_ctx* c, int b2, int n1, const cms_keypoint* kps1, const uint8_t* desc1, float* prev_matched,
                                             int window_size, float nnratio, int check_orientation, int* matches12, int* n_matches) {
  if (!c || n1 < 0 || (n1 > 0 && (!kps1 || !desc1 || !prev_matched || !matches12)) || window_size < 0)
    return cms_fail(CMS_ERR_ARG, "cms_search_for_initialization: bad argument");
  if (b2 < 0 || b2 >= c->area_frames) return cms_fail(CMS_ERR_ARG, "cms_search_for_initialization: no grid for this frame (cms_area_grid first)");
  if (n_matches) *n_matches = 0;
  if (n1 == 0) return CMS_OK;
  HIPCHK(hipSetDevice(c->device));
  static bool lds_done[64] = {false};
  { const int rca = cms_lds_ceiling_once((const void*)k_init_greedy, 160 * 1024 - 1024, c->device, lds_done); if (rca) return rca; }
  const size_t lds = (size_t)c->g.kp_cap * 8;
  if (lds > 160 * 1024 - 1024) return cms_fail(CMS_ERR_UNSUPPORTED, "cms_search_for_initialization: too many key points per frame for the LDS tables");
  hipStream_t s = c->stream;
  std::vector<int> qi;
  for (int i = 0; i < n1; ++i) if (kps1[i].octave <= 0) qi.push_back(i);
  const int nq = (int)qi.size();
  for (int i = 0; i < n1; ++i) matches12[i] = -1;
  if (nq == 0) return CMS_OK;
  const size_t q4 = (size_t)nq * 4, n4 = (size_t)n1 * 4;
  CmsBlock blk;
  const size_t o_qi = blk.take(q4), o_qx = blk.take(q4), o_qy = blk.take(q4), o_qr = blk.take(q4), o_qmin = blk.take(q4), o_qmax = blk.take(q4), o_qf = blk.take(q4),
               o_desc = blk.take((size_t)n1 * 32), o_ang = blk.take(n4), o_prev = blk.take(2 * n4);
  const size_t in_bytes = blk.size;
  const size_t o_m12 = blk.take(n4), o_nm = blk.take(16), o_tot = blk.take(16);
  const size_t out_begin = o_prev, out_end = blk.size;
  const size_t o_bin = blk.take(n1), o_cnt = blk.take(q4), o_off = blk.take(q4, 4);
  const size_t o_idx = blk.size;
  return cms_retry_capacity(128 * nq + 4096, "cms_search_for_initialization", [&](int cap, int& tot) -> int {
    const size_t o_pd = o_idx + cms_align((size_t)cap * 4);
    int rc = c->stage.reserve(s, o_pd + cms_align((size_t)cap * 2), out_end);
    if (rc) return rc;
    uint8_t* p = c->stage.d;
    uint8_t* h = c->stage.h;
    {
      int* hq = reinterpret_cast<int*>(h + o_qi); float* hx = reinterpret_cast<float*>(h + o_qx); float* hy = reinterpret_cast<float*>(h + o_qy);
      float* hr = reinterpret_cast<float*>(h + o_qr); int* hmin = reinterpret_cast<int*>(h + o_qmin); int* hmax = reinterpret_cast<int*>(h + o_qmax);
      int* hf = reinterpret_cast<int*>(h + o_qf);
      for (int q = 0; q < nq; ++q) {
        hq[q] = qi[q]; hx[q] = prev_matched[2 * qi[q]]; hy[q] = prev_matched[2 * qi[q] + 1]; hr[q] = (float)window_size; hmin[q] = 0; hmax[q] = 0; hf[q] = b2;
      }
      float* ha = reinterpret_cast<float*>(h + o_ang);
      for (int i = 0; i < n1; ++i) ha[i] = kps1[i].angle;
      memcpy(h + o_desc, desc1, (size_t)n1 * 32);
      memcpy(h + o_prev, prev_matched, 2 * n4);
    }
    rc = c->stage.up(s, in_bytes, "cms_search_for_initialization");
    if (rc) return rc;
    rc = cms_features_in_area_batch_device(c, nq, p + o_qf, p + o_qx, p + o_qy, p + o_qr, p + o_qmin, p + o_qmax, p + o_cnt, p + o_off, p + o_idx, cap, p + o_tot);
    if (rc) return rc;
    CmsInitArgs a;
    a.nq = nq; a.q_i1 = (const int*)(p + o_qi); a.cand_off = (const int*)(p + o_off); a.cand_idx = (const int*)(p + o_idx);
    a.desc1 = (const uint4*)(p + o_desc); a.t_desc = (const uint4*)c->d_desc; a.kp2 = (const CmsKeyPoint*)c->d_kps; a.row0 = b2 * c->g.kp_cap; a.kp_cap = c->g.kp_cap;
    a.angle1 = (const float*)(p + o_ang); a.pair_dist = (uint16_t*)(p + o_pd);
    a.n1 = n1; a.matches12 = (int*)(p + o_m12); a.prev_matched = (float*)(p + o_prev); a.n_matches = (int*)(p + o_nm); a.bin_of = (int8_t*)(p + o_bin);
    a.nnratio = nnratio; a.check_orientation = check_orientation; a.total = (const int*)(p + o_tot); a.cap = cap;
    hipLaunchKernelGGL(k_init_dist, dim3(nq), dim3(64), 0, s, a);
    hipLaunchKernelGGL(k_init_greedy, dim3(1), dim3(64), lds, s, a);
    HIPCHK(hipGetLastError());
    rc = c->stage.back_and_wait(s, out_begin, out_end, "cms_search_for_initialization");
    if (rc) return rc;
    tot = *reinterpret_cast<const int*>(h + o_tot);
    if (tot > cap) return CMS_OK;
    memcpy(matches12, h + o_m12, n4);
    memcpy(prev_matched, h + o_prev, 2 * n4);
    if (n_matches) *n_matches = *reinterpret_cast<const int*>(h + o_nm);
    return CMS_OK;
  });
}
```

cubemapslam_amd/csrc/cms_api_tri.hip:

```cpp
#include <algorithm>
#include <cmath>
#include <cstdlib>
#include <cstring>
#include <memory>
#include <mutex>
#include <vector>

namespace {
inline float tri_h_small(const float* a, const float* b, int bs) {
  float t = a[0] * b[0];
  t = t + a[1] * b[bs];
  t = t + a[2] * b[2 * bs];
  return t;
}
void tri_h_e12(const float* R1w, const float* t1w, const float* R2w, const float* t2w, float* E12) {
  float R12[9], M[9], t12[3];
  for (int r = 0; r < 3; ++r)
    for (int c = 0; c < 3; ++c) {
      double s = 0;
      for (int k = 0; k < 3; ++k) s += (double)R1w[3 * r + k] * (double)R2w[3 * c + k];
      R12[3 * r + c] = (float)(s * 1.0);
      M[3 * r + c] = (float)(s * -1.0);
    }
  for (int r = 0; r < 3; ++r) t12[r] = (float)((double)tri_h_small(M + 3 * r, t2w, 1) * 1.0 + (double)t1w[r] * 1.0);
// ... 236 lines not shown
  int max_n1 = 1;
  CmsBlock blk;
  const size_t o_pair = blk.take(sizeof(CmsTriPair), 16), o_job = blk.take(sizeof(CmsTriJob), 16), o_m = blk.size;
  int rc = tri_flatten_upload(c, 2, kf_at, 1, "cms_search_for_triangulation: bad key frame (at most 4096 features)", kfs, median, dev, o_work, max_n1,
                              [&](int mn1) { return o_m + cms_align((size_t)mn1 * 4 + 16) + 256; });
  if (rc) return rc;
  uint8_t* p = c->stage.d + o_work;
  const size_t o_n = o_m + cms_align((size_t)max_n1 * 4 + 16);
  CmsTriPair pr;
  pr.kf2 = 1; pr.skip = 0;
  if (E12) std::memcpy(pr.E12, E12, sizeof(pr.E12));
  else tri_h_e12(kfs[0].Rcw, kfs[0].tcw, kfs[1].Rcw, kfs[1].tcw, pr.E12);
  float C2[3];
  for (int r = 0; r < 3; ++r) C2[r] = (float)((double)tri_h_small(kfs[1].Rcw + 3 * r, kfs[0].Ow, 1) * 1.0 + (double)kfs[1].tcw[r] * 1.0);
  track_rays_to_cubemap(c->g.F, C2[0], C2[1], C2[2], pr.ex, pr.ey);
  CmsTriJob jb; jb.kf1 = 0; jb.pair0 = 0; jb.npairs = 1;
  hipStream_t s = c->stream;
  HIPCHK(hipMemcpyAsync(p + o_pair, &pr, sizeof(pr), hipMemcpyHostToDevice, s));
  HIPCHK(hipMemcpyAsync(p + o_job, &jb, sizeof(jb), hipMemcpyHostToDevice, s));
  CmsTriArgs a;
  std::memset(&a, 0, sizeof(a));
  a.kf = dev.kf; a.pair = (const CmsTriPair*)(p + o_pair); a.job = (const CmsTriJob*)(p + o_job);
  a.kp = dev.kp; a.desc = dev.desc; a.rays = dev.rays; a.mp = dev.mp; a.feat_node = dev.feat_node;
  a.node_id = dev.node_id; a.node_off = dev.node_off; a.node_feat = dev.node_feat;
  a.F = c->g.F;
  a.check_orientation = check_orientation;
  cms_level_table(a.sf, c, c->scale, 1.0f); cms_level_table(a.sigma2, c, c->sigma2, 1.0f);
  hipLaunchKernelGGL(k_tri_search, dim3(1), dim3(1024), 0, s, a, (int*)(p + o_m), (int*)(p + o_n));
  HIPCHK(hipGetLastError());
  HIPCHK(hipMemcpyAsync(matches12, p + o_m, (size_t)kf1->n * 4, hipMemcpyDeviceToHost, s));
  HIPCHK(hipMemcpyAsync(n_matches, p + o_n, 4, hipMemcpyDeviceToHost, s));
  HIPCHK(hipStreamSynchronize(s));
  return CMS_OK;
}

struct CmsStoreBow;
static void cms_store_bow_free(CmsStoreBow* b);
static void cms_store_bow_invalidate(CmsStoreBow* b, int slot);
struct CmsStoreKfdb;
static CmsStoreKfdb* cms_store_kfdb_new(int max_keyframes);
static void cms_store_kfdb_free(CmsStoreKfdb* d);
static void cms_store_kfdb_refill(CmsStoreKfdb* d, int slot);
struct CmsStoreMpUpd;
static void cms_store_mpupd_free(CmsStoreMpUpd* u);
struct cms_kfstore {
  cms_ctx* c = nullptr;
  CmsStoreBow* bow = nullptr;
  CmsStoreKfdb* kfdb = nullptr;
  CmsStoreMpUpd* mpupd = nullptr;
  int maxkf = 0, maxf = 0, maxn = 0;
  CmsTriKF* d_kf = nullptr; CmsKeyPoint* d_kp = nullptr; uint8_t* d_desc = nullptr; float* d_rays = nullptr; int* d_mp = nullptr; int* d_fn = nullptr;
  int* d_nid = nullptr; int* d_noff = nullptr; int* d_nfeat = nullptr;
  uint8_t* d_work = nullptr; size_t work_bytes = 0;
  uint16_t* d_sorted = nullptr; int* d_cell_start = nullptr; int* d_nvalid = nullptr; int* d_kp_cnt = nullptr;
  std::vector<CmsTriKF> h_kf; std::vector<float> h_median; std::vector<uint8_t> used;
  struct PutCall { hipEvent_t ev = nullptr; ~PutCall() { if (ev) (void)hipEventDestroy(ev); } };
  int* h_ff = nullptr; size_t ff_stride = 0; std::vector<std::shared_ptr<PutCall>> ff_call;
  void* h_items = nullptr; int items_gen = 0; std::shared_ptr<PutCall> items_call[2];
  unsigned upd_call = 0; hipEvent_t upd_ev[4] = {nullptr, nullptr, nullptr, nullptr}; bool upd_ev_set[4] = {false, false, false, false};
  std::vector<uint8_t> busy; hipEvent_t order_ev = nullptr;
  std::mutex put_mu; std::vector<std::shared_ptr<PutCall>> pending_puts;
  float* h_upd = nullptr; std::vector<uint8_t> upd_par;
};

static hipError_t kfstore_order_behind_puts(cms_kfstore* st);
template <class SlotOfJob>
static int kfstore_wait_puts(const cms_kfstore* st, hipStream_t stream, int njobs, SlotOfJob&& slot_of_job) {
  for (int j = 0; j < njobs; ++j) {
    const auto& call = st->ff_call[(size_t)slot_of_job(j)];
    if (call) HIPCHK(hipStreamWaitEvent(stream, call->ev, 0));
  }
  return CMS_OK;
}
extern "C" void cms_kfstore_destroy(cms_kfstore* st) {
  if (!st) return;
  if (st->c) (void)hipSetDevice(st->c->device);
  void* bufs[] = {st->d_kf, st->d_kp, st->d_desc, st->d_rays, st->d_mp, st->d_fn, st->d_nid, st->d_noff, st->d_nfeat, st->d_work,
                  st->d_sorted, st->d_cell_start, st->d_nvalid, st->d_kp_cnt};
  for (void* b : bufs) if (b) (void)hipFree(b);
  cms_store_bow_free(st->bow);
  cms_store_kfdb_free(st->kfdb);
  cms_store_mpupd_free(st->mpupd);
  if (st->h_ff) (void)hipHostFree(st->h_ff);
  if (st->h_items) (void)hipHostFree(st->h_items);
  if (st->h_upd) (void)hipHostFree(st->h_upd);
  for (hipEvent_t e : st->upd_ev) if (e) (void)hipEventDestroy(e);
  if (st->order_ev) (void)hipEventDestroy(st->order_ev);
  delete st;
}

extern "C" int cms_kfstore_create(cms_kfstore** out, cms_ctx* c, int max_keyframes, int max_features, int max_nodes) {
  if (!out || !c || max_keyframes < 1 || max_features < 1 || max_features > CMS_AREA_MAXKP || max_nodes < 1)
    return cms_fail(CMS_ERR_ARG, "cms_kfstore_create: bad argument (at most 16383 features per key frame)");
  HIPCHK(hipSetDevice(c->device));
  { const int rca = cms_area_grid_attr(c->device); if (rca) return rca; }
  cms_kfstore* st = new cms_kfstore();
  st->c = c; st->maxkf = max_keyframes; st->maxf = max_features; st->maxn = max_nodes;
  const size_t K = (size_t)max_keyframes, Fq = (size_t)max_features, Nq = (size_t)max_nodes;
#define KF_ALLOC(ptr, bytes) do { if (hipMalloc((void**)&(ptr), (bytes)) != hipSuccess) { cms_kfstore_destroy(st); return cms_fail(CMS_ERR_HIP, "cms_kfstore_create: out of device memory"); } } while (0)
  KF_ALLOC(st->d_kf, K * sizeof(CmsTriKF));
  KF_ALLOC(st->d_kp, K * Fq * sizeof(CmsKeyPoint));
  KF_ALLOC(st->d_desc, K * Fq * 32);
  KF_ALLOC(st->d_rays, K * Fq * 12);
  KF_ALLOC(st->d_mp, K * Fq * 4);
  KF_ALLOC(st->d_fn, K * Fq * 4);
  KF_ALLOC(st->d_nid, K * Nq * 4);
  KF_ALLOC(st->d_noff, K * (Nq + 1) * 4);
  KF_ALLOC(st->d_nfeat, K * Fq * 4);
  KF_ALLOC(st->d_sorted, K * Fq * sizeof(uint16_t));
  KF_ALLOC(st->d_cell_start, K * (CMS_AREA_CELLS + 1) * sizeof(int));
  KF_ALLOC(st->d_nvalid, K * sizeof(int));
  KF_ALLOC(st->d_kp_cnt, K * sizeof(int));
#undef KF_ALLOC
  st->kfdb = cms_store_kfdb_new(max_keyframes);
  if (!st->kfdb) { cms_kfstore_destroy(st); return cms_fail(CMS_ERR_HIP, "cms_kfstore_create: out of device memory"); }
  st->h_kf.assign(K, CmsTriKF{}); st->h_median.assign(K, 1.0f); st->used.assign(K, 0); st->busy.assign(K, 0);
  st->ff_call.assign(K, nullptr);
  *out = st;
  return CMS_OK;
}

extern "C" int cms_kfstore_put(cms_kfstore* st, int slot, const cms_keyframe* kf) {
  if (!st || !kf || slot < 0 || slot >= st->maxkf) return cms_fail(CMS_ERR_ARG, "cms_kfstore_put: bad argument");
  int rc = tri_check_keyframe(*kf, "cms_kfstore_put: bad key frame");
  if (rc) return rc;
  if (kf->n > st->maxf || kf->nnodes > st->maxn) return cms_fail(CMS_ERR_ARG, "cms_kfstore_put: key frame larger than the store's slots");
  cms_ctx* c = st->c;
  HIPCHK(hipSetDevice(c->device));
  HIPCHK(kfstore_order_behind_puts(st));
  hipStream_t s = c->stream;
  const size_t f0 = (size_t)slot * st->maxf, n0 = (size_t)slot * st->maxn, o0 = (size_t)slot * (st->maxn + 1);
  CmsTriKF d;
  d.f0 = (int)f0; d.n = kf->n; d.node0 = (int)n0; d.nnodes = kf->nnodes; d.noff0 = (int)o0; d.nfeat0 = (int)f0;
  std::memcpy(d.Rcw, kf->Rcw, sizeof(d.Rcw)); std::memcpy(d.tcw, kf->tcw, sizeof(d.tcw)); std::memcpy(d.Ow, kf->Ow, sizeof(d.Ow));
  std::vector<int> fn((size_t)kf->n + 1, -1);
  tri_feat_node(*kf, fn.data());
  const int zero = 0;
  if (kf->n > 0) {
    HIPCHK(hipMemcpyAsync(st->d_kp + f0, kf->kps, (size_t)kf->n * sizeof(CmsKeyPoint), hipMemcpyHostToDevice, s));
    HIPCHK(hipMemcpyAsync(st->d_desc + 32 * f0, kf->desc, 32 * (size_t)kf->n, hipMemcpyHostToDevice, s));
    HIPCHK(hipMemcpyAsync(st->d_rays + 3 * f0, kf->rays, 12 * (size_t)kf->n, hipMemcpyHostToDevice, s));
    HIPCHK(hipMemcpyAsync(st->d_mp + f0, kf->mp, 4 * (size_t)kf->n, hipMemcpyHostToDevice, s));
    HIPCHK(hipMemcpyAsync(st->d_fn + f0, fn.data(), 4 * (size_t)kf->n, hipMemcpyHostToDevice, s));
  }
  if (kf->nnodes > 0) {
    HIPCHK(hipMemcpyAsync(st->d_nid + n0, kf->node_id, 4 * (size_t)kf->nnodes, hipMemcpyHostToDevice, s));
    HIPCHK(hipMemcpyAsync(st->d_noff + o0, kf->node_off, 4 * ((size_t)kf->nnodes + 1), hipMemcpyHostToDevice, s));
    if (kf->node_off[kf->nnodes] > 0) HIPCHK(hipMemcpyAsync(st->d_nfeat + f0, kf->node_feat, 4 * (size_t)kf->node_off[kf->nnodes], hipMemcpyHostToDevice, s));
  } else {
    HIPCHK(hipMemcpyAsync(st->d_noff + o0, &zero, 4, hipMemcpyHostToDevice, s));
  }
  HIPCHK(hipMemcpyAsync(st->d_kf + slot, &d, sizeof(d), hipMemcpyHostToDevice, s));
  HIPCHK(hipMemcpyAsync(st->d_kp_cnt + slot, &kf->n, sizeof(int), hipMemcpyHostToDevice, s));
  hipLaunchKernelGGL(k_area_grid, dim3(1), dim3(1024), (size_t)(st->maxf + 1) * 8, s, (const CmsKeyPoint*)(st->d_kp + f0), (const int*)(st->d_kp_cnt + slot), st->maxf, c->g.F,
                     cms_grid_inv(c), st->d_sorted + f0, st->d_cell_start + (size_t)slot * (CMS_AREA_CELLS + 1), st->d_nvalid + slot);
  HIPCHK(hipGetLastError());
  HIPCHK(hipStreamSynchronize(s));
  st->h_kf[(size_t)slot] = d; st->h_median[(size_t)slot] = kf->median_depth; st->used[(size_t)slot] = 1;
  cms_store_bow_invalidate(st->bow, slot);
  cms_store_kfdb_refill(st->kfdb, slot);
  return CMS_OK;
}

struct CmsKfFromFrame {
  const CmsKeyPoint* kp; const uint8_t* desc; const float* rays; const uint16_t* sorted; const int* cell_start; const int* nvalid;
  CmsKeyPoint* o_kp; uint8_t* o_desc; float* o_rays; uint16_t* o_sorted; int* o_cell_start; int* o_nvalid; int* o_kp_cnt;
  int* o_mp; int* o_fn; int* o_nid; int* o_noff; int* o_nfeat; CmsTriKF* o_kf;
  const int* h_mp; const int* h_fn; const int* h_nid; const int* h_noff; const int* h_nfeat;
  CmsTriKF kf; int n, nnodes, nfeat;
};
extern "C" __global__ void __launch_bounds__(256) k_kf_put_from_frame(const CmsKfFromFrame* __restrict__ items) {
  const CmsKfFromFrame a = items[blockIdx.y];
  const int gs = gridDim.x * blockDim.x, t0 = blockIdx.x * blockDim.x + threadIdx.x;
  const int n = a.n;
  {
    const uint32_t* s = reinterpret_cast<const uint32_t*>(a.kp); uint32_t* d = reinterpret_cast<uint32_t*>(a.o_kp);
    for (int i = t0; i < 6 * n; i += gs) d[i] = s[i];
  }
  {
    const uint4* s = reinterpret_cast<const uint4*>(a.desc); uint4* d = reinterpret_cast<uint4*>(a.o_desc);
    for (int i = t0; i < 2 * n; i += gs) d[i] = s[i];
  }
  for (int i = t0; i < 3 * n; i += gs) a.o_rays[i] = a.rays[i];
  for (int i = t0; i < n; i += gs) { a.o_sorted[i] = a.sorted[i]; a.o_mp[i] = a.h_mp ? a.h_mp[i] : -1; a.o_fn[i] = a.h_fn[i]; }
  for (int i = t0; i <= CMS_AREA_CELLS; i += gs) a.o_cell_start[i] = a.cell_start[i];
  for (int i = t0; i < a.nnodes; i += gs) a.o_nid[i] = a.h_nid[i];
  for (int i = t0; i <= a.nnodes; i += gs) a.o_noff[i] = a.nnodes > 0 ? a.h_noff[i] : 0;
  for (int i = t0; i < a.nfeat; i += gs) a.o_nfeat[i] = a.h_nfeat[i];
  if (t0 == 0) { *a.o_nvalid = *a.nvalid; *a.o_kp_cnt = n; *a.o_kf = a.kf; }
}
static hipError_t kfstore_order_behind_puts(cms_kfstore* st) {
  std::vector<std::shared_ptr<cms_kfstore::PutCall>> w;
  { std::lock_guard<std::mutex> lk(st->put_mu); w.swap(st->pending_puts); }
  for (auto& c : w) { const hipError_t e = hipStreamWaitEvent(st->c->stream, c->ev, 0); if (e != hipSuccess) return e; }
  return hipSuccess;
}
static int kfstore_ff_reserve(cms_kfstore* st) {
  if (st->h_ff) return CMS_OK;
  st->ff_stride = ((size_t)3 * st->maxf + 2 * (size_t)st->maxn + 1 + 63) & ~(size_t)63;
  HIPCHK(hipHostMalloc((void**)&st->h_ff, (size_t)st->maxkf * st->ff_stride * sizeof(int), hipHostMallocMapped | hipHostMallocCoherent));
  HIPCHK(hipHostMalloc((void**)&st->h_items, 2 * (size_t)st->maxkf * sizeof(CmsKfFromFrame), hipHostMallocMapped | hipHostMallocCoherent));
  return CMS_OK;
}
static int kf_put_check(cms_kfstore* st, int slot, cms_ctx* src, int b, int n, const float* Rcw, const float* tcw, const float* Ow,
                        const int* mp, int nnodes, const int* node_id, const int* node_off, const int* node_feat) {
  if (slot < 0 || slot >= st->maxkf || b < 0 || b >= src->max_batch || n < 0 || nnodes < 0 || !Rcw || !tcw || !Ow ||
      (nnodes > 0 && (!node_id || !node_off || !node_feat)))
    return cms_fail(CMS_ERR_ARG, "cms_kfstore_put_from_frame: bad argument");
  cms_ctx* c = st->c;
  if (b >= src->area_frames) return cms_fail(CMS_ERR_ARG, "cms_kfstore_put_from_frame: no frame grid for this frame (cms_area_grid on the batch first)");
  if (n > st->maxf || n > src->g.kp_cap || nnodes > st->maxn) return cms_fail(CMS_ERR_ARG, "cms_kfstore_put_from_frame: key frame larger than the store's slots");
  {
    cms_keyframe chk;
    std::memset(&chk, 0, sizeof(chk));
    chk.n = n; chk.nnodes = nnodes; chk.node_id = node_id; chk.node_off = node_off; chk.node_feat = node_feat;
    chk.kps = reinterpret_cast<const cms_keypoint*>(st); chk.desc = reinterpret_cast<const uint8_t*>(st); chk.rays = reinterpret_cast<const float*>(st); chk.mp = reinterpret_cast<const int*>(st);
    const int rc = tri_check_keyframe(chk, "cms_kfstore_put_from_frame: bad key frame");
    if (rc) return rc;
  }
  const int nfeat = nnodes > 0 ? node_off[nnodes] : 0;
  if (nfeat > st->maxf) return cms_fail(CMS_ERR_ARG, "cms_kfstore_put_from_frame: FeatureVector lists more features than the slot holds");
  (void)c; (void)mp;
  return CMS_OK;
}
static int kf_put_fill(cms_kfstore* st, int slot, cms_ctx* src, int b, int n, const float* Rcw, const float* tcw, const float* Ow,
                       const int* mp, int nnodes, const int* node_id, const int* node_off, const int* node_feat, CmsKfFromFrame& a) {
  const int nfeat = nnodes > 0 ? node_off[nnodes] : 0;
  if (st->ff_call[(size_t)slot]) { HIPCHK(hipEventSynchronize(st->ff_call[(size_t)slot]->ev)); st->ff_call[(size_t)slot].reset(); }
  int* h = st->h_ff + (size_t)slot * st->ff_stride;
  int* h_mp = h; int* h_fn = h + st->maxf; int* h_nfeat = h + 2 * (size_t)st->maxf; int* h_nid = h + 3 * (size_t)st->maxf; int* h_noff = h_nid + st->maxn;
  if (mp && n > 0) std::memcpy(h_mp, mp, 4 * (size_t)n);
  {
    static thread_local std::vector<int> fn;
    fn.assign((size_t)std::max(n, 1), -1);
    for (int e = 0; e < nnodes; ++e)
      for (int q = node_off[e]; q < node_off[e + 1]; ++q) fn[(size_t)node_feat[q]] = e;
    if (n > 0) std::memcpy(h_fn, fn.data(), 4 * (size_t)n);
  }
  if (nnodes > 0) { std::memcpy(h_nid, node_id, 4 * (size_t)nnodes); std::memcpy(h_noff, node_off, 4 * ((size_t)nnodes + 1)); std::memcpy(h_nfeat, node_feat, 4 * (size_t)nfeat); }
  const size_t f0 = (size_t)slot * st->maxf, n0 = (size_t)slot * st->maxn, o0 = (size_t)slot * (st->maxn + 1);
  std::memset(&a, 0, sizeof(a));
  CmsTriKF& d = a.kf;
  d.f0 = (int)f0; d.n = n; d.node0 = (int)n0; d.nnodes = nnodes; d.noff0 = (int)o0; d.nfeat0 = (int)f0;
  std::memcpy(d.Rcw, Rcw, sizeof(d.Rcw)); std::memcpy(d.tcw, tcw, sizeof(d.tcw)); std::memcpy(d.Ow, Ow, sizeof(d.Ow));
  const size_t sb = (size_t)b * src->g.kp_cap;
  a.kp = (const CmsKeyPoint*)src->d_kps + sb; a.desc = src->d_desc + 32 * sb; a.rays = src->d_rays + 3 * sb; a.sorted = src->d_area_sorted + sb;
  a.cell_start = src->d_area_cell_start + (size_t)b * (CMS_AREA_CELLS + 1); a.nvalid = src->d_area_nvalid + b;
  a.o_kp = st->d_kp + f0; a.o_desc = st->d_desc + 32 * f0; a.o_rays = st->d_rays + 3 * f0; a.o_sorted = st->d_sorted + f0;
  a.o_cell_start = st->d_cell_start + (size_t)slot * (CMS_AREA_CELLS + 1); a.o_nvalid = st->d_nvalid + slot; a.o_kp_cnt = st->d_kp_cnt + slot;
  a.o_mp = st->d_mp + f0; a.o_fn = st->d_fn + f0; a.o_nid = st->d_nid + n0; a.o_noff = st->d_noff + o0; a.o_nfeat = st->d_nfeat + f0; a.o_kf = st->d_kf + slot;
  a.h_mp = mp ? h_mp : nullptr; a.h_fn = h_fn; a.h_nid = h_nid; a.h_noff = h_noff; a.h_nfeat = h_nfeat;
  a.n = n; a.nnodes = nnodes; a.nfeat = nfeat;
  return CMS_OK;
}
extern "C" int cms_kfstore_put_from_frames(cms_kfstore* st, cms_ctx* src, int n_items, const cms_kf_from_frame* items) {
  if (!st || !src || n_items < 0 || n_items > st->maxkf || (n_items > 0 && !items)) return cms_fail(CMS_ERR_ARG, "cms_kfstore_put_from_frames: bad argument");
  if (n_items == 0) return CMS_OK;
  cms_ctx* c = st->c;
  if (src->device != c->device || src->g.F != c->g.F || src->g.W != c->g.W) return cms_fail(CMS_ERR_ARG, "cms_kfstore_put_from_frame: the frame context and the store must share device and cubemap geometry");
  HIPCHK(hipSetDevice(c->device));
  { const int rc = kfstore_ff_reserve(st); if (rc) return rc; }
  {
    std::vector<uint8_t> seen((size_t)st->maxkf, 0);
    for (int i = 0; i < n_items; ++i) {
      const cms_kf_from_frame& q = items[i];
      const int rc = kf_put_check(st, q.slot, src, q.b, q.n, q.Rcw, q.tcw, q.Ow, q.mp, q.nnodes, q.node_id, q.node_off, q.node_feat);
      if (rc) return rc;
      if (seen[(size_t)q.slot]) return cms_fail(CMS_ERR_ARG, "cms_kfstore_put_from_frames: a slot is named twice");
      seen[(size_t)q.slot] = 1;
    }
  }
  const int gen = (st->items_gen ^= 1);
  if (st->items_call[gen]) { HIPCHK(hipEventSynchronize(st->items_call[gen]->ev)); st->items_call[gen].reset(); }
  CmsKfFromFrame* h_items = reinterpret_cast<CmsKfFromFrame*>(st->h_items) + (size_t)gen * st->maxkf;
  int max_n = 0;
  for (int i = 0; i < n_items; ++i) {
    const cms_kf_from_frame& q = items[i];
    const int rc = kf_put_fill(st, q.slot, src, q.b, q.n, q.Rcw, q.tcw, q.Ow, q.mp, q.nnodes, q.node_id, q.node_off, q.node_feat, h_items[i]);
    if (rc) return rc;
    max_n = std::max(max_n, q.n);
  }
  hipStream_t s = src->stream;
  {
    bool wait = false;
    for (int i = 0; i < n_items; ++i) wait = wait || (st->busy[(size_t)items[i].slot] != 0);
    if (wait && c->stream != s) {
      if (!st->order_ev) HIPCHK(hipEventCreateWithFlags(&st->order_ev, hipEventDisableTiming));
      HIPCHK(hipEventRecord(st->order_ev, c->stream));
      HIPCHK(hipStreamWaitEvent(s, st->order_ev, 0));
      std::fill(st->busy.begin(), st->busy.end(), 0);
    }
  }
  hipLaunchKernelGGL(k_kf_put_from_frame, dim3(std::max(1, std::min(32, (6 * max_n + 255) / 256)), n_items), dim3(256), 0, s, (const CmsKfFromFrame*)h_items);
  HIPCHK(hipGetLastError());
  auto call = std::make_shared<cms_kfstore::PutCall>();
  HIPCHK(hipEventCreateWithFlags(&call->ev, hipEventDisableTiming));
  HIPCHK(hipEventRecord(call->ev, s));
  if (c->stream != s) { std::lock_guard<std::mutex> lk(st->put_mu); st->pending_puts.push_back(call); }
  for (int i = 0; i < n_items; ++i) {
    const cms_kf_from_frame& q = items[i];
    st->ff_call[(size_t)q.slot] = call;
    st->h_kf[(size_t)q.slot] = h_items[i].kf; st->h_median[(size_t)q.slot] = q.median_depth; st->used[(size_t)q.slot] = 1;
    cms_store_bow_invalidate(st->bow, q.slot);
    cms_store_kfdb_refill(st->kfdb, q.slot);
  }
  st->items_call[gen] = call;
  return CMS_OK;
// ... 366 lines not shown
```

cubemapslam_amd/csrc/cms_area_kernels.hip:

```cpp
#include <hip/hip_runtime.h>
#include <stdint.h>
#include "cms_types.h"
#include "cms_area_table.h"
#include "cms_area_offsets.h"

#define CMS_AREA_CELLS (5 * CMS_AREA_G * CMS_AREA_G)
#define CMS_AREA_MAXKP 16383

extern "C" __global__ void __launch_bounds__(1024)
k_area_grid(const CmsKeyPoint* __restrict__ kps, const int* __restrict__ kp_cnt, int kp_cap, int F, float inv,
            uint16_t* __restrict__ sorted_idx, int* __restrict__ cell_start, int* __restrict__ n_valid_out) {
  extern __shared__ uint32_t area_lds[];
  uint32_t* keys = area_lds;
  uint32_t* sorted = area_lds + (kp_cap + 1);
  __shared__ int s_nvalid;
  const int b = blockIdx.x, tid = threadIdx.x, T = blockDim.x;
  const int n = min(kp_cnt[b], min(kp_cap, CMS_AREA_MAXKP));
  const CmsKeyPoint* kp = kps + (size_t)b * kp_cap;
  if (tid == 0) s_nvalid = 0;
  __syncthreads();
  for (int i = tid; i < n; i += T) {
    const float x = kp[i].x, y = kp[i].y;
    const double fi = (double)(x / (float)F), fj = (double)(y / (float)F);
    int f = -1;
    if (fi >= 0 && fi < 1 && fj >= 1 && fj < 2) f = 1;
    else if (fi >= 1 && fi < 2 && fj >= 0 && fj < 1) f = 3;
    else if (fi >= 1 && fi < 2 && fj >= 1 && fj < 2) f = 0;
    else if (fi >= 1 && fi < 2 && fj >= 2 && fj < 3) f = 4;
    else if (fi >= 2 && fi < 3 && fj >= 1 && fj < 2) f = 2;
    uint32_t key = 0xFFFFC000u | (uint32_t)i;
    if (f >= 0) {
      const int px = (int)(x * inv) % CMS_AREA_G, py = (int)(y * inv) % CMS_AREA_G;
      key = ((uint32_t)((f * CMS_AREA_G + px) * CMS_AREA_G + py) << 14) | (uint32_t)i;
      atomicAdd(&s_nvalid, 1);
    }
    keys[i] = key;
  }
  __syncthreads();
  for (int i = tid; i < n; i += T) {
    const uint32_t k = keys[i];
    int r = 0;
    for (int q = 0; q < n; ++q) r += keys[q] < k ? 1 : 0;
    sorted[r] = k;
  }
  __syncthreads();
  const int nv = s_nvalid;
  uint16_t* si = sorted_idx + (size_t)b * kp_cap;
  int* cs = cell_start + (size_t)b * (CMS_AREA_CELLS + 1);
  for (int s = tid; s < nv; s += T) {
    const int c = (int)(sorted[s] >> 14), prev = s ? (int)(sorted[s - 1] >> 14) : -1;
    si[s] = (uint16_t)(sorted[s] & 0x3FFFu);
    for (int cc = prev + 1; cc <= c; ++cc) cs[cc] = s;
  }
  const int last = nv ? (int)(sorted[nv - 1] >> 14) : -1;
  for (int cc = last + 1 + tid; cc <= CMS_AREA_CELLS; cc += T) cs[cc] = nv;
  if (tid == 0) n_valid_out[b] = nv;
}

struct CmsAreaArgs {
  const CmsKeyPoint* kp;
  const uint16_t* sorted_idx;
  const int* cell_start;
  const float* qx; const float* qy; const float* qr; const int* qmin; const int* qmax;
  const int* q_frame;
  int kp_cap;
  int nq, F; float inv;
  int* cnt;
  int* off;
  int* idx; int cap; int idx_base;
  int* tmp;
  int* psum;
};
#define CMS_AREA_TMP 8

__device__ __forceinline__ int cms_area_pick(int k, int v0, int v1, int v2) { return k == 0 ? v0 : (k == 1 ? v1 : v2); }

template <bool FILL>
__device__ __forceinline__ int cms_area_search(const CmsAreaArgs& a, int qq, bool in, int gl, int base) {
  const float x = a.qx[qq], y = a.qy[qq], r = a.qr[qq];
  const bool live = in && !(r < 0.0f);
  const int minLevel = a.qmin[qq], maxLevel = a.qmax[qq];
  const bool check = (minLevel > 0) || (maxLevel >= 0);
  CmsAreaRectI rc[3] = {};
  const int nr = live ? cms_area_rects(x, y, r, a.F, a.inv, rc) : 0;
  int n = 0;
  int* tmpq = a.tmp + (size_t)qq * CMS_AREA_TMP;
  const int fr = a.q_frame ? a.q_frame[qq] : 0;
  const CmsKeyPoint* kp = a.kp + (size_t)fr * a.kp_cap;
  const uint16_t* sorted_idx = a.sorted_idx + (size_t)fr * a.kp_cap;
  const int* cell_start = a.cell_start + (size_t)fr * (CMS_AREA_CELLS + 1);
  const int idx_base = a.idx_base + (a.q_frame ? fr * a.kp_cap : 0);
  for (int k = 0; k < 3; ++k) {
    const bool has = k < nr;
    const int x0 = has ? max(0, cms_area_pick(k, rc[0].x0, rc[1].x0, rc[2].x0)) : 0, x1 = has ? min(CMS_AREA_G - 1, cms_area_pick(k, rc[0].x1, rc[1].x1, rc[2].x1)) : -1;
    const int y0 = has ? max(0, cms_area_pick(k, rc[0].y0, rc[1].y0, rc[2].y0)) : 0, y1 = has ? min(CMS_AREA_G - 1, cms_area_pick(k, rc[0].y1, rc[1].y1, rc[2].y1)) : -1;
    const int face = has ? cms_area_pick(k, rc[0].face, rc[1].face, rc[2].face) : 0;
    const int ncol = (x1 >= x0 && y1 >= y0) ? x1 - x0 + 1 : 0;
    int maxcol = ncol;
    for (int o = 32; o > 0; o >>= 1) maxcol = max(maxcol, __shfl_xor(maxcol, o));
    for (int cb = 0; cb < maxcol; cb += CMS_AREA_QL) {
      const int ix = x0 + cb + gl;
      const bool col = cb + gl < ncol;
      int s0 = 0, s1 = 0;
      if (col) {
        const int c0 = (face * CMS_AREA_G + ix) * CMS_AREA_G + y0;
        s0 = cell_start[c0]; s1 = cell_start[c0 + (y1 - y0) + 1];
      }
      int h0 = 0, h1 = 0, h2 = 0, h3 = 0;
      int nh = 0;
      for (int s = s0; s < s1; ++s) {
        const int j = sorted_idx[s];
        const CmsKeyPoint p = kp[j];
        if (check) {
          if (p.octave < minLevel) continue;
          if (maxLevel >= 0 && p.octave > maxLevel) continue;
        }
        if (fabsf(p.x - x) < r && fabsf(p.y - y) < r) {
          if (nh == 0) h0 = j; else if (nh == 1) h1 = j; else if (nh == 2) h2 = j; else if (nh == 3) h3 = j;
          ++nh;
        }
      }
      int incl = nh;
#pragma unroll
      for (int o = 1; o < CMS_AREA_QL; o <<= 1) { const int t = __shfl_up(incl, o, CMS_AREA_QL); if (gl >= o) incl += t; }
      const int tot = __shfl(incl, CMS_AREA_QL - 1, CMS_AREA_QL);
      if (!FILL && nh > 0) {
        int w = n + incl - nh;
        if (w < CMS_AREA_TMP) {
          if (nh <= 4) {
            tmpq[w] = idx_base + h0;
            if (nh > 1 && w + 1 < CMS_AREA_TMP) tmpq[w + 1] = idx_base + h1;
            if (nh > 2 && w + 2 < CMS_AREA_TMP) tmpq[w + 2] = idx_base + h2;
            if (nh > 3 && w + 3 < CMS_AREA_TMP) tmpq[w + 3] = idx_base + h3;
          } else {
            for (int s = s0; s < s1 && w < CMS_AREA_TMP; ++s) {
              const int j = sorted_idx[s];
              const CmsKeyPoint p = kp[j];
              if (check && (p.octave < minLevel || (maxLevel >= 0 && p.octave > maxLevel))) continue;
              if (fabsf(p.x - x) < r && fabsf(p.y - y) < r) { tmpq[w] = idx_base + j; ++w; }
            }
          }
        }
      }
      if (FILL && nh > 0) {
        int w = base + n + incl - nh;
        if (nh <= 4) {
          if (cms_area_fits(w, a.cap)) a.idx[w] = idx_base + h0;
          if (nh > 1 && cms_area_fits(w + 1, a.cap)) a.idx[w + 1] = idx_base + h1;
          if (nh > 2 && cms_area_fits(w + 2, a.cap)) a.idx[w + 2] = idx_base + h2;
          if (nh > 3 && cms_area_fits(w + 3, a.cap)) a.idx[w + 3] = idx_base + h3;
        } else {
          for (int s = s0; s < s1; ++s) {
            const int j = sorted_idx[s];
            const CmsKeyPoint p = kp[j];
            if (check && (p.octave < minLevel || (maxLevel >= 0 && p.octave > maxLevel))) continue;
            if (fabsf(p.x - x) < r && fabsf(p.y - y) < r) { if (cms_area_fits(w, a.cap)) a.idx[w] = idx_base + j; ++w; }
          }
        }
      }
      n += tot;
    }
  }
  return n;
}

extern "C" __global__ void __launch_bounds__(CMS_AREA_QT) k_area_query(CmsAreaArgs a) {
  __shared__ int part[CMS_AREA_QT / 64];
  const int gl = threadIdx.x & (CMS_AREA_QL - 1);
  const int q = (blockIdx.x * CMS_AREA_QT + threadIdx.x) / CMS_AREA_QL;
  const bool in = q < a.nq;
  const int n = cms_area_search<false>(a, in ? q : 0, in, gl, 0);
  if (in && gl == 0) a.cnt[q] = n;
  int v = n;
  for (int o = CMS_AREA_QL; o < 64; o <<= 1) v += __shfl_xor(v, o);
  if ((threadIdx.x & 63) == 0) part[threadIdx.x >> 6] = v;
  __syncthreads();
  if (threadIdx.x == 0) { int t = 0; for (int w = 0; w < CMS_AREA_QT / 64; ++w) t += part[w]; a.psum[blockIdx.x] = t; }
}

extern "C" __global__ void __launch_bounds__(CMS_AREA_LT) k_area_lists(CmsAreaArgs a, int* __restrict__ total) {
  __shared__ int s_cnt[CMS_AREA_TILE], s_off[CMS_AREA_TILE];
  __shared__ int part[CMS_AREA_TILE_K * CMS_AREA_LW], pbefore[CMS_AREA_LW];
  const int tid = threadIdx.x, lane = tid & 63, wv = tid >> 6;
  const int tile = blockIdx.x, q0 = tile * CMS_AREA_TILE;
  int before = 0;
  {
    const int4* p4 = (const int4*)a.psum;
    const int n4 = cms_area_parts_before(tile) / 4;
    for (int b = tid; b < n4; b += CMS_AREA_LT) { const int4 v = p4[b]; before += (v.x + v.y) + (v.z + v.w); }
  }
  for (int o = 32; o > 0; o >>= 1) before += __shfl_xor(before, o);
  if (lane == 0) pbefore[wv] = before;
  int c[CMS_AREA_TILE_K], incl[CMS_AREA_TILE_K];
#pragma unroll
  for (int k = 0; k < CMS_AREA_TILE_K; ++k) {
    const int q = q0 + cms_area_tile_slot(tid, k);
    c[k] = q < a.nq ? a.cnt[q] : 0;
    int s = c[k];
#pragma unroll
    for (int o = 1; o < 64; o <<= 1) { const int t = __shfl_up(s, o); if (lane >= o) s += t; }
    incl[k] = s;
    if (lane == 63) part[k * CMS_AREA_LW + wv] = s;
  }
  __syncthreads();
  int tile_base = 0;
  for (int w = 0; w < CMS_AREA_LW; ++w) tile_base += pbefore[w];
#pragma unroll
  for (int k = 0; k < CMS_AREA_TILE_K; ++k) {
// ... 31 lines not shown
```

cubemapslam_amd/csrc/cms_track_kernels.hip:

```cpp
#include <hip/hip_runtime.h>
#include <stdint.h>

struct CmsFrustumArgs {
  const float* pose15;
  const int* mp_frame;
  int n;
  const float* P; const float* normal; const float* min_dist; const float* max_dist;
  float viewing_cos_limit, log_scale, th;
  int nlevels, F;
  int bounds_scaled;
  float sf[16];
  uint8_t* in_view; float* proj_x; float* proj_y; int* level; float* view_cos;
  float* qr; int* qmin; int* qmax;
};

#include "cms_project_helpers.h"

__device__ __forceinline__ bool track_distance_in_bounds(int scaled, float min_in, float max_in, const float* PO, float& dist, float& raw_max) {
  float maxDistance, minDistance;
  track_distance_bounds(scaled, min_in, max_in, minDistance, maxDistance, raw_max);
  double s = 0;
#pragma unroll
  for (int k = 0; k < 3; ++k) s = __dadd_rn(s, __dmul_rn((double)PO[k], (double)PO[k]));
  dist = (float)sqrt(s);
  return !(dist < minDistance || dist > maxDistance);
}
extern "C" __global__ void __launch_bounds__(256) k_in_frustum(CmsFrustumArgs a) {
  const int i = blockIdx.x * blockDim.x + threadIdx.x;
  if (i >= a.n) return;
  const float* ps = a.pose15 + 15 * (size_t)(a.mp_frame ? a.mp_frame[i] : 0);
  uint8_t vis = 0; float u = -1.0f, v = -1.0f, vc = 0.0f; int lvl = -1;
  const float px = a.P[3 * (size_t)i], py = a.P[3 * (size_t)i + 1], pz = a.P[3 * (size_t)i + 2];
  float Pc[3];
#pragma unroll
  for (int r = 0; r < 3; ++r) {
    float t = __fmul_rn(ps[3 * r], px);
    t = __fadd_rn(t, __fmul_rn(ps[3 * r + 1], py));
    t = __fadd_rn(t, __fmul_rn(ps[3 * r + 2], pz));
    Pc[r] = (float)((double)t * 1.0 + (double)ps[9 + r] * 1.0);
  }
  const float mnMax = (float)(3 * a.F);
  do {
    const int face = track_rays_to_cubemap(a.F, Pc[0], Pc[1], Pc[2], u, v);
    if (face < 0) break;
    if (u < 0.0f || u > mnMax || v < 0.0f || v > mnMax) break;
    const float PO[3] = {__fsub_rn(px, ps[12]), __fsub_rn(py, ps[13]), __fsub_rn(pz, ps[14])};
    float maxd, dist;
    if (!track_distance_in_bounds(a.bounds_scaled, a.min_dist[i], a.max_dist[i], PO, dist, maxd)) break;
    double d = 0;
#pragma unroll
    for (int k = 0; k < 3; ++k) d = __dadd_rn(d, __dmul_rn((double)PO[k], (double)a.normal[3 * (size_t)i + k]));
    vc = (float)(d / (double)dist);
    if (vc < a.viewing_cos_limit) break;
    lvl = track_predict_scale(maxd, dist, a.log_scale, a.nlevels); vis = 1;
  } while (false);
  if (!vis) { u = -1.0f; v = -1.0f; vc = 0.0f; }
  a.in_view[i] = vis; a.proj_x[i] = u; a.proj_y[i] = v; a.level[i] = lvl; a.view_cos[i] = vc;
  if (a.qr) {
    float r = (double)vc > 0.998 ? 2.5f : 4.0f;
    if (a.th != 1.0f) r = __fmul_rn(r, a.th);
    a.qr[i] = vis ? __fmul_rn(r, a.sf[lvl]) : -1.0f;
    a.qmin[i] = lvl - 1; a.qmax[i] = lvl;
  }
}

struct CmsSearchLocalArgs {
  const int* mp_off;
  const uint4* mp_desc;
  const int* cand_off; const int* cand_idx;
  const uint4* t_desc; const CmsKeyPoint* kp; int kp_cap;
  uint16_t* pair_dist;
  int* kp_mp;
  int* mp_match;
  int* rounds;
  float nnratio; int th_high;
  int frame0;
  const int* wg_frame;
  const int* total; int cap;
};

__device__ __forceinline__ int track_hamming256(const uint4& a0, const uint4& a1, const uint4& b0, const uint4& b1) {
  return __popc(a0.x ^ b0.x) + __popc(a0.y ^ b0.y) + __popc(a0.z ^ b0.z) + __popc(a0.w ^ b0.w) +
         __popc(a1.x ^ b1.x) + __popc(a1.y ^ b1.y) + __popc(a1.z ^ b1.z) + __popc(a1.w ^ b1.w);
}

#define CMS_TRACK_KPMAX 4096
extern "C" __global__ void __launch_bounds__(1024) k_search_local(CmsSearchLocalArgs a) {
  __shared__ int min_open[CMS_TRACK_KPMAX];
  const int f = blockIdx.x, tid = threadIdx.x, nt = blockDim.x;
  if (a.total && *a.total > a.cap) return;
  const int m0 = a.mp_off[f], m1 = a.mp_off[f + 1];
  const int frame = a.wg_frame ? a.wg_frame[f] : f + a.frame0;
  const int row0 = frame * a.kp_cap;
  int* const kp_mp = a.wg_frame ? a.kp_mp + ((ptrdiff_t)f - frame) * a.kp_cap : a.kp_mp;
  {
    const int sub = tid & 3;
    for (int i = m0 + (tid >> 2); i < m1; i += nt >> 2) {
      const int c0 = a.cand_off[i], c1 = a.cand_off[i + 1];
      if (c0 == c1) continue;
      const uint4 q0 = a.mp_desc[2 * (size_t)i], q1 = a.mp_desc[2 * (size_t)i + 1];
      for (int c = c0 + sub; c < c1; c += 4) {
        const size_t row = (size_t)a.cand_idx[c];
        a.pair_dist[c] = (uint16_t)track_hamming256(q0, q1, a.t_desc[2 * row], a.t_desc[2 * row + 1]);
      }
    }
  }
  for (int i = m0 + tid; i < m1; i += nt) a.mp_match[i] = a.cand_off[i] == a.cand_off[i + 1] ? -1 : -2;
  __syncthreads();
  int round = 0;
  for (;;) {
    for (int k = tid; k < a.kp_cap; k += nt) min_open[k] = 0x7FFFFFFF;
    __syncthreads();
    for (int i = m0 + tid; i < m1; i += nt) {
      if (a.mp_match[i] != -2) continue;
      for (int c = a.cand_off[i]; c < a.cand_off[i + 1]; ++c) {
        const int row = a.cand_idx[c];
        if (kp_mp[row] < 0) atomicMin(&min_open[row - row0], i);
      }
    }
    __syncthreads();
    int open = 0;
    for (int i = m0 + tid; i < m1; i += nt) {
      if (a.mp_match[i] != -2) continue;
      bool ok = true;
      for (int c = a.cand_off[i]; c < a.cand_off[i + 1] && ok; ++c) {
        const int row = a.cand_idx[c];
        ok = kp_mp[row] >= 0 || min_open[row - row0] == i;
      }
      if (ok) a.mp_match[i] = -3; else ++open;
    }
    __syncthreads();
    for (int i = m0 + tid; i < m1; i += nt) {
      if (a.mp_match[i] != -3) continue;
      int bestDist = 256, bestLevel = -1, bestDist2 = 256, bestLevel2 = -1, bestRow = -1;
      for (int c = a.cand_off[i]; c < a.cand_off[i + 1]; ++c) {
        const int row = a.cand_idx[c];
        if (kp_mp[row] >= 0) continue;
        const int dist = a.pair_dist[c];
        if (dist < bestDist) { bestDist2 = bestDist; bestDist = dist; bestLevel2 = bestLevel; bestLevel = a.kp[row].octave; bestRow = row; }
        else if (dist < bestDist2) { bestLevel2 = a.kp[row].octave; bestDist2 = dist; }
      }
      int m = -1;
      const bool ratio_ok = a.nnratio < 0.0f || !(bestLevel == bestLevel2 && (float)bestDist > __fmul_rn(a.nnratio, (float)bestDist2));
      if (bestDist <= a.th_high && ratio_ok) m = bestRow;
      if (m >= 0) kp_mp[m] = i;
      a.mp_match[i] = m;
    }
    ++round;
    if (__syncthreads_count(open > 0) == 0) break;
  }
  if (a.rounds && tid == 0) a.rounds[f] = round;
}


struct CmsProjectLastArgs {
  const float* pose12;
  const int* q_frame;
  int n; const uint8_t* valid; const float* Xw; const int* oct;
  float th, cos_fov; int F; float sf[16];
  float* qx; float* qy; float* qr; int* qmin; int* qmax;
};
extern "C" __global__ void __launch_bounds__(256) k_project_last(CmsProjectLastArgs a) {
  const int i = blockIdx.x * blockDim.x + threadIdx.x;
  if (i >= a.n) return;
  float u = -1.0f, v = -1.0f, r = -1.0f;
  const int o = a.oct[i];
  if (a.valid[i]) {
    const float* ps = a.pose12 + 12 * (size_t)(a.q_frame ? a.q_frame[i] : 0);
    const float p0 = a.Xw[3 * (size_t)i], p1 = a.Xw[3 * (size_t)i + 1], p2 = a.Xw[3 * (size_t)i + 2];
    float xc[3];
#pragma unroll
    for (int k = 0; k < 3; ++k) {
      float t = __fmul_rn(ps[3 * k], p0);
      t = __fadd_rn(t, __fmul_rn(ps[3 * k + 1], p1));
      t = __fadd_rn(t, __fmul_rn(ps[3 * k + 2], p2));
      xc[k] = (float)((double)t * 1.0 + (double)ps[9 + k] * 1.0);
    }
    if (!(xc[2] < a.cos_fov) && track_rays_to_cubemap(a.F, xc[0], xc[1], xc[2], u, v) >= 0) r = __fmul_rn(a.th, a.sf[o & 15]);
  }
  a.qx[i] = u; a.qy[i] = v; a.qr[i] = r; a.qmin[i] = o - 1; a.qmax[i] = o + 1;
}

struct CmsProjectKfArgs {
  int n;
  const int* pt_job;
  const float* pose12;
  const int* job_frame;
  const int* job_kp0;
  const CmsKeyPoint* kf_kp;
  const int* kf_feat;
  const float* kf_angle;
  const float* pos; const float* min_dist; const float* max_dist;
  float th, cos_fov, log_scale; int nlevels, F, bounds_scaled; float sf[16];
  int* q_frame; float* qx; float* qy; float* qr; int* qmin; int* qmax; float* angle;
  int* level;
};
extern "C" __global__ void __launch_bounds__(256) k_project_keyframe(CmsProjectKfArgs a) {
  const int i = blockIdx.x * blockDim.x + threadIdx.x;
  if (i >= a.n) return;
  const int j = a.pt_job[i];
  const float* ps = a.pose12 + 12 * (size_t)j;
  const float p[3] = {a.pos[3 * (size_t)i], a.pos[3 * (size_t)i + 1], a.pos[3 * (size_t)i + 2]};
  float xc[3], PO[3];
#pragma unroll
  for (int k = 0; k < 3; ++k) {
    float t = __fmul_rn(ps[3 * k], p[0]);
    t = __fadd_rn(t, __fmul_rn(ps[3 * k + 1], p[1]));
    t = __fadd_rn(t, __fmul_rn(ps[3 * k + 2], p[2]));
    xc[k] = (float)((double)t * 1.0 + (double)ps[9 + k] * 1.0);
    double s = 0;
#pragma unroll
    for (int r = 0; r < 3; ++r) s = __dadd_rn(s, __dmul_rn((double)ps[3 * r + k], (double)ps[9 + r]));
    PO[k] = __fsub_rn(p[k], (float)(-1.0 * s));
  }
  float u = -1.0f, v = -1.0f, r = -1.0f, maxd, dist;
  int lvl = -1;
  if (!(xc[2] < a.cos_fov) && track_rays_to_cubemap(a.F, xc[0], xc[1], xc[2], u, v) >= 0 &&
      track_distance_in_bounds(a.bounds_scaled, a.min_dist[i], a.max_dist[i], PO, dist, maxd)) {
    lvl = track_predict_scale(maxd, dist, a.log_scale, a.nlevels);
    r = __fmul_rn(a.th, a.sf[lvl]);
  }
  const int kp0 = a.job_kp0[j];
  a.angle[i] = kp0 >= 0 ? a.kf_kp[(size_t)kp0 + a.kf_feat[i]].angle : a.kf_angle[i];
  a.q_frame[i] = a.job_frame[j];
  a.qx[i] = u; a.qy[i] = v; a.qr[i] = r; a.qmin[i] = lvl - 1; a.qmax[i] = lvl + 1;
  if (a.level) a.level[i] = lvl;
}


__device__ __forceinline__ int track_rot_bin(float angle_ref, float angle_cur) {
  float rot = __fsub_rn(angle_ref, angle_cur);
  if (rot < 0.0f) rot = __fadd_rn(rot, 360.0f);
  int bin = (int)roundf(__fmul_rn(rot, 1.0f / 12));
  return bin == 30 ? 0 : bin;
}
__device__ __forceinline__ void track_three_maxima(const int* hist, int* keep) {
  int max1 = 0, max2 = 0, max3 = 0, i1 = -1, i2 = -1, i3 = -1;
  for (int b = 0; b < 30; ++b) {
    const int s = hist[b];
    if (s > max1) { max3 = max2; max2 = max1; max1 = s; i3 = i2; i2 = i1; i1 = b; }
    else if (s > max2) { max3 = max2; max2 = s; i3 = i2; i2 = b; }
    else if (s > max3) { max3 = s; i3 = b; }
  }
  if ((float)max2 < __fmul_rn(0.1f, (float)max1)) { i2 = -1; i3 = -1; } else if ((float)max3 < __fmul_rn(0.1f, (float)max1)) i3 = -1;
  keep[0] = i1; keep[1] = i2; keep[2] = i3;
}

struct CmsRotFilterArgs {
  const int* mp_off; const float* last_angle; const CmsKeyPoint* kp; int* kp_mp; int* mp_match; int* n_matches; int check_orientation;
  const int* total; int cap;
  const int* wg_frame; int kp_cap;
};
extern "C" __global__ void __launch_bounds__(1024) k_rot_filter(CmsRotFilterArgs a) {
  __shared__ int hist[32];
  __shared__ int keep[3];
  __shared__ int s_n;
  const int f = blockIdx.x, tid = threadIdx.x, nt = blockDim.x;
  if (a.total && *a.total > a.cap) return;
  const int m0 = a.mp_off[f], m1 = a.mp_off[f + 1];
  int* const kp_mp = a.wg_frame ? a.kp_mp + ((ptrdiff_t)f - a.wg_frame[f]) * a.kp_cap : a.kp_mp;
  if (tid < 32) hist[tid] = 0;
  if (tid == 0) s_n = 0;
  __syncthreads();
  auto bin_of = [&](int i, int row) { return track_rot_bin(a.last_angle[i], a.kp[row].angle); };
  for (int i = m0 + tid; i < m1; i += nt) {
    const int row = a.mp_match[i];
    if (row >= 0 && a.check_orientation) atomicAdd(&hist[bin_of(i, row)], 1);
  }
  __syncthreads();
  if (tid == 0) track_three_maxima(hist, keep);
  __syncthreads();
  int mine = 0;
  for (int i = m0 + tid; i < m1; i += nt) {
    const int row = a.mp_match[i];
    if (row < 0) continue;
    if (a.check_orientation) {
      const int b = bin_of(i, row);
      if (b != keep[0] && b != keep[1] && b != keep[2]) { kp_mp[row] = -1; a.mp_match[i] = -1; continue; }
    }
    ++mine;
  }
  atomicAdd(&s_n, mine);
  __syncthreads();
  if (tid == 0 && a.n_matches) a.n_matches[f] = s_n;
}

struct CmsInitArgs {
  int nq; const int* q_i1;
  const int* cand_off; const int* cand_idx;
  const uint4* desc1; const uint4* t_desc; const CmsKeyPoint* kp2; int row0, kp_cap;
  const float* angle1; uint16_t* pair_dist;
  int n1; int* matches12; float* prev_matched; int* n_matches; int8_t* bin_of;
  float nnratio; int check_orientation;
  const int* total; int cap;
};
extern "C" __global__ void __launch_bounds__(64) k_init_dist(CmsInitArgs a) {
  if (*a.total > a.cap) return;
  const int q = blockIdx.x, i1 = a.q_i1[q];
  const uint4 q0 = a.desc1[2 * (size_t)i1], q1 = a.desc1[2 * (size_t)i1 + 1];
// ... 83 lines not shown
```

include/cubemapslam_hip.h:

```cpp
#ifndef CUBEMAPSLAM_HIP_H
#define CUBEMAPSLAM_HIP_H
#include <stddef.h>
#include <stdint.h>
#ifdef __cplusplus
extern "C" {
#endif

#define CMS_OK 0
#define CMS_ERR_ARG (-1)
#define CMS_ERR_HIP (-2)
#define CMS_ERR_UNSUPPORTED (-3)
#define CMS_ERR_OVERFLOW (-4)
#define CMS_ERR_NO_DEVICE (-5)

enum { CMS_FACE_UNKNOWN = -1, CMS_FACE_FRONT = 0, CMS_FACE_LEFT = 1, CMS_FACE_RIGHT = 2, CMS_FACE_UPPER = 3, CMS_FACE_LOWER = 4 };

typedef struct {
  double c, d, e, u0, v0;
  double invpol[12];
  double pol[5];
  int Iw, Ih;
  int face;
  double fov_deg;
} cms_camera;

typedef struct { int nfeatures; float scale_factor; int nlevels; int ini_th_fast; int min_th_fast; } cms_orb_params;

typedef struct { float x, y, size, angle, response; int octave; } cms_keypoint;

typedef struct {
  int W, F, nlevels, kp_cap, max_batch;
  int level_w[12], level_h[12], level_quota[12], level_cells[12];
  float scale[12], inv_scale[12], sigma2[12], inv_sigma2[12];
  size_t pyramid_bytes_per_frame, candidate_entries_per_frame;
  int fisheye_stride;
} cms_geometry;

typedef struct cms_ctx cms_ctx;

const char* cms_last_error(void);
int cms_device_count(void);

int cms_ctx_create(cms_ctx** out, int device, const cms_camera* cam, const cms_orb_params* orb, int max_batch);
void cms_ctx_destroy(cms_ctx* ctx);
int cms_ctx_geometry(const cms_ctx* ctx, cms_geometry* out);
void* cms_ctx_stream(cms_ctx* ctx);

int cms_remap(cms_ctx* ctx, const uint8_t* fisheye, int fstride, uint8_t* cubemap, int cstride);
int cms_set_mask(cms_ctx* ctx, const uint8_t* mask, int mstride);
int cms_set_gaussian_mode(cms_ctx* ctx, int column_mode);
int cms_extract(cms_ctx* ctx, const uint8_t* cubemap, int cstride, cms_keypoint* kps, uint8_t* desc, int cap, int* n);
int cms_remap_extract(cms_ctx* ctx, const uint8_t* fisheye, int fstride, cms_keypoint* kps, uint8_t* desc, int cap, int* n);
int cms_remap_extract_rays(cms_ctx* ctx, const uint8_t* fisheye, int fstride, cms_keypoint* kps, uint8_t* desc, float* rays, int cap, int* n);
int cms_frames_rays(cms_ctx* ctx, void** d_rays);
int cms_frames_fetch_rays(cms_ctx* ctx, int b, float* rays, int cap, int* n);

void* cms_frames_input(cms_ctx* ctx);
int cms_frames_upload(cms_ctx* ctx, const uint8_t* fisheye, int fstride, size_t frame_pitch, int B);
int cms_frames_upload_async(cms_ctx* ctx, const uint8_t* fisheye, int fstride, size_t frame_pitch, int B);
int cms_frames_upload_wait(cms_ctx* ctx);
int cms_stream_wait_extracted(cms_ctx* ctx, void* hip_stream);
int cms_frames_upload_device(cms_ctx* ctx, const void* d_src, int B);
int cms_stream_copy_device(cms_ctx* ctx, void* d_dst, const void* d_src, size_t bytes);
int cms_host_alloc(void** out, size_t bytes);
void cms_host_free(void* p);
int cms_frames_process(cms_ctx* ctx, int B, int from_fisheye);
int cms_frames_process_device(cms_ctx* ctx, const void* d_src, int B);
int cms_frames_sync(cms_ctx* ctx);
int cms_frames_results(cms_ctx* ctx, void** d_kps, void** d_desc, void** d_counts);
int cms_frames_fetch(cms_ctx* ctx, int b, cms_keypoint* kps, uint8_t* desc, int cap, int* n);

typedef struct { uint16_t tx, ty, x0, y0, nd, rows, flags, pad; } cms_remap_tile;
int cms_remap_lut_host(const cms_camera* cam, uint32_t* lut, int lut_stride);
int cms_remap_tiles_host(const cms_camera* cam, const uint32_t* lut, int lut_stride, int tile_w, int tile_h, int lds_budget,
                         cms_remap_tile* out, int cap, int* n_live, int* n_all, int* lds_bytes);

int cms_fast_cells_host(const cms_camera* cam, const cms_orb_params* orb, int which, int* out, int cap, int* n);

int cms_debug_lut(cms_ctx* ctx, uint32_t* out, int* stride);
int cms_debug_cubemap(cms_ctx* ctx, int b, uint8_t* dst, int dstride);
int cms_debug_level(cms_ctx* ctx, int b, int level, uint8_t* dst, int dstride);
int cms_debug_candidates(cms_ctx* ctx, int b, int level, int* xys, int cap, int* n);
int cms_debug_distributed(cms_ctx* ctx, int b, int level, int* xys, int cap, int* n);

int cms_profile_enable(cms_ctx* ctx, int on);
int cms_profile_get(cms_ctx* ctx, float* ms7);

int cms_hamming_best2(cms_ctx* ctx, const uint8_t* qdesc, int nq, const uint8_t* tdesc, int nt, const int* cand_off,
                      const int* cand_idx, const int* t_level, const uint8_t* t_excluded, int* best_idx, int* best_dist,
                      int* best_level, int* second_dist, int* second_level);
int cms_hamming_best2_device(cms_ctx* ctx, const void* qdesc, const void* q_row, int nq, const void* tdesc, const void* cand_off,
                             const void* cand_idx, const void* t_level, const void* t_excluded, void* best_idx,
                             void* best_dist, void* best_level, void* second_dist, void* second_level);
int cms_hamming_matrix(cms_ctx* ctx, const uint8_t* a, int na, const uint8_t* b, int nb, uint16_t* out);

typedef struct cms_ba cms_ba;
typedef struct {
  int iterations_done[2];
  double chi2_initial[2], chi2_final[2], lambda_final[2];
  int n_outliers_mid, n_outliers_final;
} cms_ba_stats;
int cms_ba_create(cms_ba** out, int device, int K, const double* poses, const uint8_t* fixed, int P, const double* points,
                  int E, const int* e_pose, const int* e_point, const double* e_obs, const double* e_invsig2,
                  const int8_t* e_face, double fx, double fy, double cx, double cy);
typedef struct cms_ba_window {
  int K; const double* poses; const uint8_t* fixed; int P; const double* points; int E; const int* e_pose; const int* e_point;
  const double* e_obs; const double* e_invsig2; const int8_t* e_face; double fx, fy, cx, cy;
  int flags;
} cms_ba_window;
#define CMS_BA_INPUTS_PINNED 1
#define CMS_BA_PLAN_ON_DEVICE 2
int cms_ba_create_many(cms_ba** out, int n, int device, const cms_ba_window* windows, int threads);
int cms_ba_read_many(cms_ba** bas, int n, double** poses, double** points, uint8_t** outlier_flags);
int cms_ba_reset(cms_ba* ba);
int cms_ba_optimize(cms_ba* ba, int its_robust, int its_final, const volatile uint8_t* stop, cms_ba_stats* stats);
int cms_ba_optimize_many(cms_ba** bas, int n, int its_robust, int its_final, const volatile uint8_t* stop, cms_ba_stats* stats);
int cms_ba_optimize_global(cms_ba* ba, int iterations, int robust, const volatile uint8_t* stop, cms_ba_stats* stats);
int cms_ba_optimize_global_many(cms_ba** bas, int n, int iterations, int robust, const volatile uint8_t* stop, cms_ba_stats* stats);
int cms_ba_debug_solve_tiled(int device, int n, const double* A, const double* b, double* x, int* status);
int cms_ba_debug_solve_timed(int device, int which, int n, const double* A, const double* b, double* x, int* status, int reps, double* ms);
int cms_ba_read(cms_ba* ba, double* poses, double* points, uint8_t* outlier_flags);
void* cms_ba_stream(cms_ba* ba);
int cms_ba_set_stream(cms_ba* ba, void* hip_stream);
int cms_ba_debug_clocks(cms_ba* ba, long long* out16);
int cms_ba_profile_kernel(cms_ba* ba, int kernel_id);
int cms_ba_profile_get(cms_ba* ba, double* total_ms, long* launches);
int cms_ba_debug_compose(int K, const uint8_t* fixed, int P, int E, const int* e_pose, const int* e_point, int lookahead,
                         int* pinv, int* chunk_pt0, int* n_chunks, uint8_t* rank);
int cms_ba_debug_plan(int K, const uint8_t* fixed, int P, int E, const int* e_pose, const int* e_point, int* pinv, int* perm, uint32_t* info,
                      int* chunk_pt0, int* rm_chunk, uint32_t* run_lane, int* counts, uint32_t* run_mf, uint32_t* run_fl);
int cms_ba_debug_fetch_plan(cms_ba* ba, int* pinv, int* perm, uint32_t* info, int* pt_off, int* e_pose, int* e_point, int8_t* e_face, int* chunk_e0,
                            int* rm_chunk, uint32_t* rm_cost, uint32_t* run_mf, uint32_t* run_fl, int* counts);
int cms_ba_debug_plan_fast(int K, const uint8_t* fixed, int P, int E, const int* e_pose, const int* e_point, int* pinv, int* perm, uint32_t* info,
                           int* chunk_pt0, int* rm_chunk, int* counts, uint32_t* run_mf, uint32_t* run_fl);
int cms_ba_debug_run_fg(int K, const uint8_t* fixed, int P, int E, const int* e_pose, const int* e_point, int fast, uint32_t* run_fg, int* rm_cut, int* counts);
int cms_ba_debug_match(int which, int n, const int* slots, int np, int* choice_out);
void cms_ba_destroy(cms_ba* ba);
int cms_ba_pool_trim(int device, size_t* released);
int cms_ba_set_deterministic(int on);
int cms_ba_get_deterministic(void);
int cms_ba_run(int device, int K, double* poses, const uint8_t* fixed, int P, double* points, int E, const int* e_pose,
               const int* e_point, const double* e_obs, const double* e_invsig2, const int8_t* e_face, double fx, double fy,
               double cx, double cy, int its_robust, int its_final, const volatile uint8_t* stop, uint8_t* outlier_flags,
               cms_ba_stats* stats);
int cms_ba_linearize(int device, int K, const double* poses, const uint8_t* fixed, int P, const double* points, int E,
                     const int* e_pose, const int* e_point, const double* e_obs, const double* e_invsig2,
                     const int8_t* e_face, double fx, double fy, double cx, double cy, int robust, double huber_delta,
                     double* err, double* Hpp, double* bp, double* Hll, double* bl, double* Hpl, double* robust_chi2_sum);

int cms_area_set_keypoints(cms_ctx* ctx, int b, int n, const cms_keypoint* kps);
int cms_area_grid(cms_ctx* ctx, int B);
int cms_features_in_area(cms_ctx* ctx, int b, int nq, const float* qx, const float* qy, const float* qr, const int* min_level,
                         const int* max_level, int* cand_off, int* cand_idx, int cap, int* total);
int cms_features_in_area_device(cms_ctx* ctx, int b, int nq, const void* d_qx, const void* d_qy, const void* d_qr, const void* d_min_level,
                                const void* d_max_level, void* d_cnt_scratch, void* d_cand_off, void* d_cand_idx, int cap, int idx_base,
                                void* d_total);
int cms_features_in_area_batch_device(cms_ctx* ctx, int nq, const void* d_qframe, const void* d_qx, const void* d_qy, const void* d_qr,
                                      const void* d_min_level, const void* d_max_level, void* d_cnt_scratch, void* d_cand_off,
                                      void* d_cand_idx, int cap, void* d_total);

int cms_area_set_descriptors(cms_ctx* ctx, int b, int n, const uint8_t* desc);
int cms_set_distance_bounds_mode(cms_ctx* ctx, int scaled);
int cms_search_by_projection(cms_ctx* ctx, int b, const float* pose12, int nlast, const uint8_t* valid, const float* Xw, const int* octave,
                             const float* angle, const uint8_t* mp_desc, float th, int check_orientation, int th_high, int nkp, int* kp_mp,
                             int* match, int* n_matches);
int cms_search_for_initialization(cms_ctx* ctx, int b2, int n1, const cms_keypoint* kps1, const uint8_t* desc1, float* prev_matched,
                                  int window_size, float nnratio, int check_orientation, int* matches12, int* n_matches);
int cms_project_last_frame_device(cms_ctx* ctx, int n, const void* d_qframe, const void* d_pose12, const void* d_valid, const void* d_Xw,
                                  const void* d_oct, float th, void* d_qx, void* d_qy, void* d_qr, void* d_qmin, void* d_qmax);
int cms_rotation_filter_device(cms_ctx* ctx, int B, const void* d_mp_off, const void* d_last_angle, void* d_kp_mp, void* d_mp_match,
                               void* d_n_matches, int check_orientation);
int cms_search_local_points(cms_ctx* ctx, int b, const float* pose15, int nmp, const float* pos, const float* normal,
                            const float* min_dist, const float* max_dist, const uint8_t* mp_desc, float viewing_cos_limit, float th,
                            float nnratio, int th_high, int nkp, int* kp_mp, uint8_t* in_view, float* proj_x, float* proj_y, int* level,
                            float* view_cos, int* mp_match, int* n_matches, int* rounds);
int cms_is_in_frustum_device(cms_ctx* ctx, int nmp, const void* d_mp_frame, const void* d_pose15, const void* d_pos, const void* d_normal,
                             const void* d_min_dist, const void* d_max_dist, float viewing_cos_limit, float th, void* d_in_view,
                             void* d_proj_x, void* d_proj_y, void* d_level, void* d_view_cos, void* d_qr, void* d_qmin, void* d_qmax);
int cms_search_local_points_device(cms_ctx* ctx, int B, const void* d_mp_off, const void* d_mp_desc, const void* d_cand_off,
                                   const void* d_cand_idx, void* d_pair_dist, float nnratio, int th_high, void* d_kp_mp, void* d_mp_match,
                                   void* d_rounds);

typedef struct {
  int n; const cms_keypoint* kps; const uint8_t* desc; const float* rays; const int* mp;
  float Rcw[9], tcw[3], Ow[3];
  int nnodes; const int* node_id; const int* node_off; const int* node_feat;
  float median_depth;
} cms_keyframe;
int cms_create_new_map_points(cms_ctx* ctx, int njobs, const cms_keyframe* cur, const int* neigh_off, const cms_keyframe* neigh,
                              int check_orientation, int cap_per_job, int* n_new, int* out_neigh, int* out_idx1, int* out_idx2,
                              float* out_x3d);
int cms_search_for_triangulation(cms_ctx* ctx, const cms_keyframe* kf1, const cms_keyframe* kf2, const float* E12, int check_orientation,
                                 int* matches12, int* n_matches);
typedef struct cms_kfstore cms_kfstore;
int cms_kfstore_create(cms_kfstore** out, cms_ctx* ctx, int max_keyframes, int max_features, int max_nodes);
void cms_kfstore_destroy(cms_kfstore* st);
int cms_kfstore_put(cms_kfstore* st, int slot, const cms_keyframe* kf);
int cms_kfstore_update(cms_kfstore* st, int slot, const float* Rcw, const float* tcw, const float* Ow, const float* median_depth, const int* mp);
int cms_kfstore_put_from_frame(cms_kfstore* st, int slot, cms_ctx* src, int b, int n, const float* Rcw, const float* tcw, const float* Ow, float median_depth,
                               const int* mp, int nnodes, const int* node_id, const int* node_off, const int* node_feat);
typedef struct {
  int slot, b, n;
  const float* Rcw; const float* tcw; const float* Ow; float median_depth;
  const int* mp; int nnodes; const int* node_id; const int* node_off; const int* node_feat;
} cms_kf_from_frame;
int cms_kfstore_put_from_frames(cms_kfstore* st, cms_ctx* src, int n_items, const cms_kf_from_frame* items);
int cms_kfstore_update_poses(cms_kfstore* st, int n, const int* slots, const float* Rcw, const float* tcw, const float* Ow);
int cms_kfstore_debug_fetch(cms_kfstore* st, int slot, cms_keypoint* kps, uint8_t* desc, float* rays, int* mp, int* feat_node, uint16_t* sorted,
                            int* node_id, int* node_off, int* node_feat, int* cell_start, uint32_t* header, int* misc);
int cms_kfstore_fuse_search(cms_kfstore* st, int njobs, const int* job_slot, const int* mp_off, const uint8_t* skip, const float* pos,
                            const float* normal, const float* min_dist, const float* max_dist, const uint8_t* mp_desc, float th, int* best_idx,
                            int* best_dist);
int cms_kfstore_fuse_search_sets(cms_kfstore* st, int nsets, const int* set_off, const float* pos, const float* normal, const float* min_dist,
                                 const float* max_dist, const uint8_t* mp_desc, int njobs, const int* job_slot, const int* job_set, const uint8_t* skip,
                                 float th, int* best_idx, int* best_dist);
int cms_kfstore_create_new_map_points(cms_kfstore* st, int njobs, const int* cur_slot, const int* neigh_off, const int* neigh_slot,
                                      int check_orientation, int cap_per_job, int* n_new, int* out_neigh, int* out_idx1, int* out_idx2,
                                      float* out_x3d);
int cms_distinctive_descriptors(cms_ctx* ctx, int npts, const int* obs_off, const uint8_t* desc, int* best_idx);
int cms_update_normal_and_depth(cms_ctx* ctx, int npts, const int* obs_off, const float* pos, const float* obs_Ow, const float* ref_Ow,
                                const int* ref_level, float* normal, float* min_dist, float* max_dist);
int cms_fuse_search(cms_ctx* ctx, int b, const float* pose15, int nmp, const uint8_t* skip, const float* pos, const float* normal,
                    const float* min_dist, const float* max_dist, const uint8_t* mp_desc, float th, int* best_idx, int* best_dist);

int cms_search_by_bow(cms_ctx* ctx, int b, int n, int nnodes, const int* node_id, const int* node_off, const int* node_feat,
                      const cms_keyframe* kf, const uint8_t* kf_skip, float nnratio, int check_orientation,
                      int* kf_idx , int* n_matches);
typedef struct {
  int slot;
  int b, n;
  int nnodes; const int* node_id; const int* node_off; const int* node_feat;
  const uint8_t* kf_skip;
} cms_bow_job;
int cms_kfstore_search_by_bow(cms_kfstore* st, cms_ctx* src, int njobs, const cms_bow_job* jobs, float nnratio,
                              int check_orientation, int* kf_idx , int* n_matches );

typedef struct {
  int slot1, n1;
  int slot2, n2;
  const uint8_t* skip1;
  const uint8_t* skip2;
} cms_bow_kf_job;
int cms_kfstore_search_by_bow_keyframes(cms_kfstore* st, cms_ctx* src, int njobs, const cms_bow_kf_job* jobs,
                                        float nnratio, int check_orientation,
                                        int* idx2 , int* n_matches );

typedef struct cms_vocab cms_vocab;
int cms_vocab_create(cms_vocab** out, int device, int k, int L, int scoring, int weighting, int n_nodes, const int* parent, const uint8_t* is_leaf,
                     const uint8_t* desc, const double* weight);
void cms_vocab_destroy(cms_vocab* v);
int cms_vocab_info(const cms_vocab* v, int* info);
int cms_vocab_profile_enable(int on);
int cms_vocab_profile_get(float* ms2);
int cms_vocab_transform(cms_vocab* v, cms_ctx* ctx, int n, const uint8_t* desc, int levelsup, int* nwords, int* word_id, double* word_val, int* nnodes,
                        int* node_id, int* node_off, int* node_feat);
int cms_frames_compute_bow(cms_ctx* ctx, cms_vocab* v, int levelsup, int n_rows, const int* rows, const int* n);
int cms_frames_fetch_bow(cms_ctx* ctx, int b, int* nwords, int* word_id, double* word_val, int word_cap, int* nnodes, int* node_id, int* node_off,
                         int* node_feat, int node_cap, int feat_cap);
int cms_kfstore_compute_bow(cms_kfstore* st, cms_vocab* v, int levelsup, int n_slots, const int* slots);
int cms_kfstore_fetch_bow(cms_kfstore* st, int slot, int* nwords, int* word_id, double* word_val, int word_cap, int* nnodes, int* node_id, int* node_off,
                          int* node_feat, int node_cap, int feat_cap);
int cms_kfstore_search_by_bow_frames(cms_kfstore* st, cms_ctx* src, int njobs, const cms_bow_job* jobs, float nnratio, int check_orientation,
                                     int* kf_idx, int* n_matches);

int cms_kfstore_set_bow(cms_kfstore* st, int slot, int nwords, const int* word_id, const double* word_val);
int cms_kfdb_add(cms_kfstore* st, int n, const int* slots, const int* groups);
int cms_kfdb_erase(cms_kfstore* st, int n, const int* slots);
int cms_kfdb_clear(cms_kfstore* st, int group);
int cms_kfdb_set_covisibles(cms_kfstore* st, int n, const int* slots, const int* neigh);
#define CMS_KFDB_RELOC 0
#define CMS_KFDB_LOOP 1
#define CMS_KFDB_QUERY_ROW 0
#define CMS_KFDB_QUERY_SLOT 1
#define CMS_KFDB_QUERY_WORDS 2
typedef struct cms_kfdb_job {
  int mode, group, query;
  int b, slot;
  int nwords; const int* word_id; const double* word_val;
  float min_score; int n_connected; const int* connected;
} cms_kfdb_job;
int cms_kfdb_detect(cms_kfstore* st, cms_ctx* src, int njobs, const cms_kfdb_job* jobs, int cand_cap, int* cand_slot, int* n_cand, int* diag_common,
                    float* diag_score);
int cms_kfstore_bow_score(cms_kfstore* st, int npairs, const int* slot_a, const int* slot_b, double* score);
int cms_kfdb_profile_enable(int on);
int cms_kfdb_profile_get(float* ms);

typedef struct {
  int slot;
  int b, n;
  float pose12[12];
  int nmp;
  const int* kf_feat;
  const float* pos; const float* min_dist; const float* max_dist; const uint8_t* mp_desc;
  int* kp_mp;
  int* match;
} cms_kfproj_job;
int cms_kfstore_search_by_projection(cms_kfstore* st, cms_ctx* src, int njobs, const cms_kfproj_job* jobs, float th, int orb_dist,
                                     int check_orientation, int* n_matches );
int cms_search_by_projection_keyframe(cms_ctx* ctx, int b, const float* pose12, int nmp, const float* kf_angle, const float* pos,
                                      const float* min_dist, const float* max_dist, const uint8_t* mp_desc, float th, int orb_dist,
                                      int check_orientation, int nkp, int* kp_mp, int* match, int* n_matches);

int cms_pnp_ransac_parameters(int N, double probability, int minInliers, int maxIterations, int minSet, float epsilon,
                              int* min_inliers, int* max_its, float* epsilon_out);
typedef struct cms_pnp cms_pnp;
int cms_pnp_create(cms_pnp** out, int device, int max_jobs, int max_corr_total, int max_hyp_total);
void cms_pnp_destroy(cms_pnp* p);
typedef struct {
  int N;
  const float* p3d;
  const float* p2d;
  const float* bearing;
  const float* sigma2;
  const int* kp_idx;
  int b, n;
  float th2; int min_inliers, max_its, min_set;
  int n_iterations;
  int n_draws; const int* draws;
  int iterations, best_inliers; float best_Tcw[12]; uint8_t* best_mask;
  int status, no_more, n_inliers, iterations_run; float Tcw[12]; uint8_t* inliers;
} cms_pnp_job;
int cms_pnp_iterate(cms_pnp* p, cms_ctx* ctx , int njobs, cms_pnp_job* jobs);
int cms_pnp_iterate_frames(cms_pnp* p, cms_ctx* ctx, int njobs, cms_pnp_job* jobs);

int cms_sim3_ransac_parameters(int N, double probability, int minInliers, int maxIterations, int* max_its);
typedef struct cms_sim3 cms_sim3;
int cms_sim3_create(cms_sim3** out, int device, int max_jobs, int max_corr_total, int max_hyp_total);
void cms_sim3_destroy(cms_sim3* p);
typedef struct {
  int N;
  const float* x3dc1;
  const float* x3dc2;
  const float* max_err1;
  const float* max_err2;
// ... 113 lines not shown
```

Measured before the change: 25110.

## Replace O(n^2) area-grid rank sort with counting sort; LDS-resident greedy local search

The area grid kernel drops its quadratic rank-by-comparison sort of keypoints in favor of a per-cell histogram, a wave-shuffle prefix scan and a scatter, followed by a small within-cell rank that keeps the index order deterministic. The local-points search kernel gains an LDS-resident path: it packs candidate row, Hamming distance and octave into LDS once, keeps taken flags in LDS, and iterates greedy rounds over compacted worklists instead of rescanning global memory every round. This path falls back to the old global-memory path when the budgets are exceeded or the inputs look malformed. The change also adds debug entry points, and the larger dynamic LDS allocations may limit occupancy.

Result: no change. 25300, median of 5 (+0.8%).

```diff
diff --git a/cubemapslam_amd/api.py b/cubemapslam_amd/api.py
--- a/cubemapslam_amd/api.py
+++ b/cubemapslam_amd/api.py
@@ -101,6 +101,7 @@
                                        C.c_double, C.c_int, C.c_double] + [C.c_void_p] * 7
         L.cms_area_set_keypoints.argtypes = [C.c_void_p, C.c_int, C.c_int, C.c_void_p]
         L.cms_area_grid.argtypes = [C.c_void_p, C.c_int]
+        L.cms_debug_area_grid.argtypes = [C.c_void_p, C.c_int, C.c_void_p, C.c_void_p, C.c_void_p]
         L.cms_features_in_area.argtypes = [C.c_void_p, C.c_int, C.c_int] + [C.c_void_p] * 7 + [C.c_int, C.c_void_p]
         L.cms_features_in_area_device.argtypes = [C.c_void_p, C.c_int, C.c_int] + [C.c_void_p] * 8 + [C.c_int, C.c_int, C.c_void_p]
         L.cms_features_in_area_batch_device.argtypes = [C.c_void_p, C.c_int] + [C.c_void_p] * 9 + [C.c_int, C.c_void_p]
@@ -405,6 +406,11 @@
     def area_grid(self, B):
         _chk(lib().cms_area_grid(self.h, B), "cms_area_grid")
 
+    def debug_area_grid(self, b):
+        si = np.zeros(max(1, self.geom.kp_cap), np.uint16); cs = np.zeros(5 * 50 * 50 + 1, np.int32); nv = C.c_int(0)
+        _chk(lib().cms_debug_area_grid(self.h, b, _p(si), _p(cs), C.byref(nv)), "cms_debug_area_grid")
+        return si[:nv.value].copy(), cs, nv.value
+
     def features_in_area(self, b, qx, qy, qr, qmin, qmax, cap=None):
         qx = np.ascontiguousarray(qx, np.float32); qy = np.ascontiguousarray(qy, np.float32); qr = np.ascontiguousarray(qr, np.float32)
         qmin = np.ascontiguousarray(qmin, np.int32); qmax = np.ascontiguousarray(qmax, np.int32)
@@ -498,6 +504,11 @@
         v = lambda a: C.c_void_p(int(a)) if a else None
         _chk(lib().cms_search_local_points_device(self.h, B, v(d_mp_off), v(d_mp_desc), v(d_cand_off), v(d_cand_idx), v(d_pair_dist), nnratio,
                                                   th_high, v(d_kp_mp), v(d_mp_match), v(d_rounds)), "cms_search_local_points_device")
+
+    def debug_search_local_budget(self, max_points, max_cands):
+        L = lib()
+        L.cms_debug_search_local_budget.argtypes = [C.c_void_p, C.c_int, C.c_int]
+        _chk(L.cms_debug_search_local_budget(self.h, max_points, max_cands), "cms_debug_search_local_budget")
 
     def hamming_best2_device(self, qdesc, q_row, nq, tdesc, cand_off, cand_idx, t_level, t_excl, outs):
         _chk(lib().cms_hamming_best2_device(self.h, _p(qdesc), _p(q_row), nq, _p(tdesc), _p(cand_off), _p(cand_idx), _p(t_level),
diff --git a/cubemapslam_amd/csrc/cms_api_area.hip b/cubemapslam_amd/csrc/cms_api_area.hip
--- a/cubemapslam_amd/csrc/cms_api_area.hip
+++ b/cubemapslam_amd/csrc/cms_api_area.hip
@@ -2,7 +2,7 @@
 
 static int cms_area_grid_attr(int device) {
   static bool done[64] = {false};
-  return cms_lds_ceiling_once((const void*)k_area_grid, (CMS_AREA_MAXKP + 1) * 8, device, done);
+  return cms_lds_ceiling_once((const void*)k_area_grid, (int)cms_area_grid_lds(CMS_AREA_MAXKP), device, done);
 }
 static int cms_area_reserve(cms_ctx* c) {
   if (c->d_area_sorted) return CMS_OK;
@@ -94,10 +94,23 @@
   HIPCHK(hipSetDevice(c->device));
   int rc = cms_area_reserve(c);
   if (rc) return rc;
-  hipLaunchKernelGGL(k_area_grid, dim3(B), dim3(1024), (size_t)(c->g.kp_cap + 1) * 8, c->stream, (const CmsKeyPoint*)c->d_kps, (const int*)c->d_kp_cnt, c->g.kp_cap, c->g.F, cms_grid_inv(c),
+  hipLaunchKernelGGL(k_area_grid, dim3(B), dim3(CMS_AREA_GT), cms_area_grid_lds(c->g.kp_cap), c->stream, (const CmsKeyPoint*)c->d_kps, (const int*)c->d_kp_cnt, c->g.kp_cap, c->g.F, cms_grid_inv(c),
                      c->d_area_sorted, c->d_area_cell_start, c->d_area_nvalid);
   HIPCHK(hipGetLastError());
   c->area_frames = B;
+  return CMS_OK;
+}
+
+extern "C" int cms_debug_area_grid(cms_ctx* c, int b, uint16_t* sorted_idx, int* cell_start, int* n_valid) {
+  if (!c || !sorted_idx || !cell_start || !n_valid || b < 0 || b >= c->area_frames) return cms_fail(CMS_ERR_ARG, "cms_debug_area_grid: bad argument (cms_area_grid first)");
+  HIPCHK(hipSetDevice(c->device));
+  HIPCHK(hipStreamSynchronize(c->stream));
+  int nv = 0;
+  HIPCHK(hipMemcpy(&nv, c->d_area_nvalid + b, sizeof(int), hipMemcpyDeviceToHost));
+  *n_valid = nv;
+  if (nv < 0 || nv > c->g.kp_cap) return cms_fail(CMS_ERR_HIP, "cms_debug_area_grid: the grid's count is out of range");
+  if (nv > 0) HIPCHK(hipMemcpy(sorted_idx, c->d_area_sorted + (size_t)b * c->g.kp_cap, (size_t)nv * sizeof(uint16_t), hipMemcpyDeviceToHost));
+  HIPCHK(hipMemcpy(cell_start, c->d_area_cell_start + (size_t)b * (CMS_AREA_CELLS + 1), (CMS_AREA_CELLS + 1) * sizeof(int), hipMemcpyDeviceToHost));
   return CMS_OK;
 }
 
diff --git a/cubemapslam_amd/csrc/cms_api_frames.hip b/cubemapslam_amd/csrc/cms_api_frames.hip
--- a/cubemapslam_amd/csrc/cms_api_frames.hip
+++ b/cubemapslam_amd/csrc/cms_api_frames.hip
@@ -83,6 +83,7 @@
   hipStream_t copy_stream = nullptr; hipEvent_t ev_upload_done = nullptr, ev_remap_done = nullptr;
   bool upload_pending = false, remap_recorded = false;
   int dist_bounds_scaled = 0;
+  int sl_lds_points = CMS_TRACK_LDS_POINTS, sl_lds_cands = CMS_TRACK_LDS_CANDS;
   hipEvent_t ev_block = nullptr; int last_batch = 0;
   hipEvent_t ev_extracted = nullptr; bool extracted_recorded = false;
   CmsKeyPoint* d_kps = nullptr; uint32_t* d_aux = nullptr; uint8_t* d_desc = nullptr; int* d_kp_cnt = nullptr;
diff --git a/cubemapslam_amd/csrc/cms_api_reloc.hip b/cubemapslam_amd/csrc/cms_api_reloc.hip
--- a/cubemapslam_amd/csrc/cms_api_reloc.hip
+++ b/cubemapslam_amd/csrc/cms_api_reloc.hip
@@ -68,7 +68,8 @@
     CmsSearchLocalArgs g = track_search_local_args(c, p + o_mpoff, p + o_desc, p + o_off, p + o_idx, p + o_pd, (int*)(p + o_kpmp), p + o_match, nullptr, -1.0f, orb_dist, 0,
                                                    p + o_tot, cap);
     g.wg_frame = (const int*)(p + o_jframe);
-    hipLaunchKernelGGL(k_search_local, dim3(njobs), dim3(1024), 0, s, g);
+    rc = track_search_local_launch(c, s, njobs, g);
+    if (rc) return rc;
     CmsRotFilterArgs r = {};
     r.mp_off = g.mp_off; r.last_angle = (const float*)(p + o_ang); r.kp = g.kp; r.kp_mp = g.kp_mp; r.mp_match = g.mp_match; r.n_matches = (int*)(p + o_nm);
     r.check_orientation = check_orientation; r.total = g.total; r.cap = cap; r.wg_frame = g.wg_frame; r.kp_cap = kp_cap;
diff --git a/cubemapslam_amd/csrc/cms_api_track.hip b/cubemapslam_amd/csrc/cms_api_track.hip
--- a/cubemapslam_amd/csrc/cms_api_track.hip
+++ b/cubemapslam_amd/csrc/cms_api_track.hip
@@ -45,7 +45,21 @@
   a.t_desc = (const uint4*)c->d_desc; a.kp = (const CmsKeyPoint*)c->d_kps; a.kp_cap = c->g.kp_cap;
   a.pair_dist = (uint16_t*)pair_dist; a.kp_mp = kp_mp; a.mp_match = (int*)mp_match; a.rounds = (int*)rounds;
   a.nnratio = nnratio; a.th_high = th_high; a.frame0 = frame0; a.total = (const int*)total; a.cap = cap;
+  a.lds_points = c->sl_lds_points; a.lds_cands = c->sl_lds_cands;
   return a;
+}
+static int track_search_local_launch(const cms_ctx* c, hipStream_t s, int grid, const CmsSearchLocalArgs& a) {
+  static bool done[64] = {false};
+  const int rc = cms_lds_ceiling_once((const void*)k_search_local, (int)track_search_local_lds(CMS_TRACK_LDS_POINTS, CMS_TRACK_LDS_CANDS), c->device, done);
+  if (rc) return rc;
+  hipLaunchKernelGGL(k_search_local, dim3(grid), dim3(CMS_TRACK_SLT), track_search_local_lds(a.lds_points, a.lds_cands), s, a);
+  return CMS_OK;
+}
+extern "C" int cms_debug_search_local_budget(cms_ctx* c, int max_points, int max_cands) {
+  if (!c || max_points < 0 || max_cands < 0 || max_points > CMS_TRACK_LDS_POINTS || max_cands > CMS_TRACK_LDS_CANDS)
+    return cms_fail(CMS_ERR_ARG, "cms_debug_search_local_budget: a budget between 0 and the built-in one");
+  c->sl_lds_points = max_points; c->sl_lds_cands = max_cands;
+  return CMS_OK;
 }
 
 extern "C" int cms_search_local_points_device(cms_ctx* c, int B, const void* d_mp_off, const void* d_mp_desc, const void* d_cand_off,
@@ -56,7 +70,7 @@
   if (c->g.kp_cap > CMS_TRACK_KPMAX) return cms_fail(CMS_ERR_UNSUPPORTED, "cms_search_local_points_device: more than 4096 key points per frame");
   HIPCHK(hipSetDevice(c->device));
   const CmsSearchLocalArgs a = track_search_local_args(c, d_mp_off, d_mp_desc, d_cand_off, d_cand_idx, d_pair_dist, (int*)d_kp_mp, d_mp_match, d_rounds, nnratio, th_high, 0, nullptr, 0);
-  hipLaunchKernelGGL(k_search_local, dim3(B), dim3(1024), 0, c->stream, a);
+  { const int rcl = track_search_local_launch(c, c->stream, B, a); if (rcl) return rcl; }
   HIPCHK(hipGetLastError());
   return CMS_OK;
 }
@@ -117,7 +131,8 @@
     if (rc) return rc;
     const CmsSearchLocalArgs a = track_search_local_args(c, p + o_mpoff, p + o_desc, p + o_off, p + o_idx, p + o_pd, track_kp_mp_of_frame(c, p, o_kpmp, b), p + o_match,
                                                          p + o_rounds, nnratio, th_high, b, p + o_tot, cap);
-    hipLaunchKernelGGL(k_search_local, dim3(1), dim3(1024), 0, s, a);
+    rc = track_search_local_launch(c, s, 1, a);
+    if (rc) return rc;
     HIPCHK(hipGetLastError());
     rc = c->stage.back_and_wait(s, out_begin, out_end, "cms_search_local_points");
     if (rc) return rc;
@@ -205,7 +220,8 @@
     if (rc) return rc;
     const CmsSearchLocalArgs a = track_search_local_args(c, p + o_mpoff, p + o_desc, p + o_off, p + o_idx, p + o_pd, track_kp_mp_of_frame(c, p, o_kpmp, b), p + o_match,
                                                          nullptr, -1.0f, th_high, b, p + o_tot, cap);
-    hipLaunchKernelGGL(k_search_local, dim3(1), dim3(1024), 0, s, a);
+    rc = track_search_local_launch(c, s, 1, a);
+    if (rc) return rc;
     CmsRotFilterArgs r = {};
     r.mp_off = a.mp_off; r.last_angle = (const float*)(p + o_ang); r.kp = a.kp; r.kp_mp = a.kp_mp;
     r.mp_match = a.mp_match; r.n_matches = (int*)(p + o_nm); r.check_orientation = check_orientation; r.total = a.total; r.cap = cap;
diff --git a/cubemapslam_amd/csrc/cms_api_tri.hip b/cubemapslam_amd/csrc/cms_api_tri.hip
--- a/cubemapslam_amd/csrc/cms_api_tri.hip
+++ b/cubemapslam_amd/csrc/cms_api_tri.hip
@@ -412,7 +412,7 @@
   }
   HIPCHK(hipMemcpyAsync(st->d_kf + slot, &d, sizeof(d), hipMemcpyHostToDevice, s));
   HIPCHK(hipMemcpyAsync(st->d_kp_cnt + slot, &kf->n, sizeof(int), hipMemcpyHostToDevice, s));
-  hipLaunchKernelGGL(k_area_grid, dim3(1), dim3(1024), (size_t)(st->maxf + 1) * 8, s, (const CmsKeyPoint*)(st->d_kp + f0), (const int*)(st->d_kp_cnt + slot), st->maxf, c->g.F,
+  hipLaunchKernelGGL(k_area_grid, dim3(1), dim3(CMS_AREA_GT), cms_area_grid_lds(st->maxf), s, (const CmsKeyPoint*)(st->d_kp + f0), (const int*)(st->d_kp_cnt + slot), st->maxf, c->g.F,
                      cms_grid_inv(c), st->d_sorted + f0, st->d_cell_start + (size_t)slot * (CMS_AREA_CELLS + 1), st->d_nvalid + slot);
   HIPCHK(hipGetLastError());
   HIPCHK(hipStreamSynchronize(s));
diff --git a/cubemapslam_amd/csrc/cms_area_kernels.hip b/cubemapslam_amd/csrc/cms_area_kernels.hip
--- a/cubemapslam_amd/csrc/cms_area_kernels.hip
+++ b/cubemapslam_amd/csrc/cms_area_kernels.hip
@@ -7,17 +7,22 @@
 #define CMS_AREA_CELLS (5 * CMS_AREA_G * CMS_AREA_G)
 #define CMS_AREA_MAXKP 16383
 
-extern "C" __global__ void __launch_bounds__(1024)
+#define CMS_AREA_GT 1024
+#define CMS_AREA_GCH ((CMS_AREA_CELLS + CMS_AREA_GT - 1) / CMS_AREA_GT)
+static inline size_t cms_area_grid_lds(int kp_cap) { return (size_t)CMS_AREA_CELLS * 4 + (size_t)(kp_cap + 1) * 4; }
+
+extern "C" __global__ void __launch_bounds__(CMS_AREA_GT)
 k_area_grid(const CmsKeyPoint* __restrict__ kps, const int* __restrict__ kp_cnt, int kp_cap, int F, float inv,
             uint16_t* __restrict__ sorted_idx, int* __restrict__ cell_start, int* __restrict__ n_valid_out) {
-  extern __shared__ uint32_t area_lds[];
-  uint32_t* keys = area_lds;
-  uint32_t* sorted = area_lds + (kp_cap + 1);
-  __shared__ int s_nvalid;
-  const int b = blockIdx.x, tid = threadIdx.x, T = blockDim.x;
+  extern __shared__ int area_lds[];
+  int* cell = area_lds;
+  uint16_t* cell_of = (uint16_t*)(area_lds + CMS_AREA_CELLS);
+  uint16_t* scat = cell_of + (kp_cap + 1);
+  __shared__ int s_wave[CMS_AREA_GT / 64];
+  const int b = blockIdx.x, tid = threadIdx.x, T = CMS_AREA_GT;
   const int n = min(kp_cnt[b], min(kp_cap, CMS_AREA_MAXKP));
   const CmsKeyPoint* kp = kps + (size_t)b * kp_cap;
-  if (tid == 0) s_nvalid = 0;
+  for (int c = tid; c < CMS_AREA_CELLS; c += T) cell[c] = 0;
   __syncthreads();
   for (int i = tid; i < n; i += T) {
     const float x = kp[i].x, y = kp[i].y;
@@ -28,32 +33,45 @@
     else if (fi >= 1 && fi < 2 && fj >= 1 && fj < 2) f = 0;
     else if (fi >= 1 && fi < 2 && fj >= 2 && fj < 3) f = 4;
     else if (fi >= 2 && fi < 3 && fj >= 1 && fj < 2) f = 2;
-    uint32_t key = 0xFFFFC000u | (uint32_t)i;
+    int c = CMS_AREA_CELLS;
     if (f >= 0) {
       const int px = (int)(x * inv) % CMS_AREA_G, py = (int)(y * inv) % CMS_AREA_G;
-      key = ((uint32_t)((f * CMS_AREA_G + px) * CMS_AREA_G + py) << 14) | (uint32_t)i;
-      atomicAdd(&s_nvalid, 1);
+      c = (f * CMS_AREA_G + px) * CMS_AREA_G + py;
+      atomicAdd(&cell[c], 1);
     }
-    keys[i] = key;
-  }
+    cell_of[i] = (uint16_t)c;
+  }
+  __syncthreads();
+  const int c0 = tid * CMS_AREA_GCH, lane = tid & 63, wv = tid >> 6;
+  int v[CMS_AREA_GCH], sum = 0;
+#pragma unroll
+  for (int k = 0; k < CMS_AREA_GCH; ++k) { v[k] = c0 + k < CMS_AREA_CELLS ? cell[c0 + k] : 0; sum += v[k]; }
+  int incl = sum;
+#pragma unroll
+  for (int o = 1; o < 64; o <<= 1) { const int t = __shfl_up(incl, o); if (lane >= o) incl += t; }
+  if (lane == 63) s_wave[wv] = incl;
+  __syncthreads();
+  int run = incl - sum;
+  for (int w = 0; w < wv; ++w) run += s_wave[w];
+#pragma unroll
+  for (int k = 0; k < CMS_AREA_GCH; ++k) { if (c0 + k < CMS_AREA_CELLS) cell[c0 + k] = run; run += v[k]; }
   __syncthreads();
   for (int i = tid; i < n; i += T) {
-    const uint32_t k = keys[i];
-    int r = 0;
-    for (int q = 0; q < n; ++q) r += keys[q] < k ? 1 : 0;
-    sorted[r] = k;
-  }
-  __syncthreads();
-  const int nv = s_nvalid;
+    const int c = cell_of[i];
+    if (c < CMS_AREA_CELLS) scat[atomicAdd(&cell[c], 1)] = (uint16_t)i;
+  }
+  __syncthreads();
+  const int nv = cell[CMS_AREA_CELLS - 1];
   uint16_t* si = sorted_idx + (size_t)b * kp_cap;
   int* cs = cell_start + (size_t)b * (CMS_AREA_CELLS + 1);
   for (int s = tid; s < nv; s += T) {
-    const int c = (int)(sorted[s] >> 14), prev = s ? (int)(sorted[s - 1] >> 14) : -1;
-    si[s] = (uint16_t)(sorted[s] & 0x3FFFu);
-    for (int cc = prev + 1; cc <= c; ++cc) cs[cc] = s;
-  }
-  const int last = nv ? (int)(sorted[nv - 1] >> 14) : -1;
-  for (int cc = last + 1 + tid; cc <= CMS_AREA_CELLS; cc += T) cs[cc] = nv;
+    const int i = scat[s], c = cell_of[i];
+    const int s0 = c ? cell[c - 1] : 0, s1 = cell[c];
+    int r = s0;
+    for (int q = s0; q < s1; ++q) r += (int)scat[q] < i ? 1 : 0;
+    si[r] = (uint16_t)i;
+  }
+  for (int c = tid; c <= CMS_AREA_CELLS; c += T) cs[c] = c ? cell[c - 1] : 0;
   if (tid == 0) n_valid_out[b] = nv;
 }
 
diff --git a/cubemapslam_amd/csrc/cms_track_kernels.hip b/cubemapslam_amd/csrc/cms_track_kernels.hip
--- a/cubemapslam_amd/csrc/cms_track_kernels.hip
+++ b/cubemapslam_amd/csrc/cms_track_kernels.hip
@@ -77,6 +77,7 @@
   int frame0;
   const int* wg_frame;
   const int* total; int cap;
+  int lds_points, lds_cands;
 };
 
 __device__ __forceinline__ int track_hamming256(const uint4& a0, const uint4& a1, const uint4& b0, const uint4& b1) {
@@ -85,14 +86,137 @@
 }
 
 #define CMS_TRACK_KPMAX 4096
-extern "C" __global__ void __launch_bounds__(1024) k_search_local(CmsSearchLocalArgs a) {
-  __shared__ int min_open[CMS_TRACK_KPMAX];
-  const int f = blockIdx.x, tid = threadIdx.x, nt = blockDim.x;
+#define CMS_TRACK_SLT 1024
+#define CMS_TRACK_LDS_POINTS 4096
+#define CMS_TRACK_LDS_CANDS 8192
+static_assert(CMS_TRACK_LDS_POINTS < 0x8000 && CMS_TRACK_LDS_CANDS < 0x10000, "resident lists hold 15-bit points and 16-bit candidate offsets");
+static inline size_t track_search_local_lds(int points, int cands) {
+  return (size_t)CMS_TRACK_KPMAX * 5 + (size_t)cands * 4 + (size_t)((points + 2) & ~1) * 2 + (size_t)points * 4;
+}
+
+template <class S> __device__ __forceinline__ void track_greedy_claim(const S& s, int i, int* min_open) {
+  for (int c = s.begin(i), e = s.end(i); c < e; ++c) {
+    const int r = s.row(c);
+    if (!s.taken(r)) atomicMin(&min_open[r], s.key(i));
+  }
+}
+template <class S> __device__ __forceinline__ bool track_greedy_ready(const S& s, int i) {
+  bool ok = true;
+  for (int c = s.begin(i), e = s.end(i); c < e && ok; ++c) {
+    const int r = s.row(c);
+    ok = s.taken(r) || s.lowest(r) == s.key(i);
+  }
+  return ok;
+}
+template <class S> __device__ __forceinline__ int track_greedy_decide(const S& s, int i, float nnratio, int th_high) {
+  int bestDist = 256, bestLevel = -1, bestDist2 = 256, bestLevel2 = -1, bestRow = -1;
+  for (int c = s.begin(i), e = s.end(i); c < e; ++c) {
+    const int r = s.row(c);
+    if (s.taken(r)) continue;
+    const int dist = s.dist(c);
+    if (dist < bestDist) { bestDist2 = bestDist; bestDist = dist; bestLevel2 = bestLevel; bestLevel = s.octave(c); bestRow = r; }
+    else if (dist < bestDist2) { bestLevel2 = s.octave(c); bestDist2 = dist; }
+  }
+  const bool ratio_ok = nnratio < 0.0f || !(bestLevel == bestLevel2 && (float)bestDist > __fmul_rn(nnratio, (float)bestDist2));
+  return (bestDist <= th_high && ratio_ok) ? bestRow : -1;
+}
+struct TrackGreedyGlobal {
+  const CmsSearchLocalArgs& a; const int* kp_mp; const int* min_open; int row0;
+  __device__ __forceinline__ int begin(int i) const { return a.cand_off[i]; }
+  __device__ __forceinline__ int end(int i) const { return a.cand_off[i + 1]; }
+  __device__ __forceinline__ int row(int c) const { return a.cand_idx[c] - row0; }
+  __device__ __forceinline__ bool taken(int r) const { return kp_mp[row0 + r] >= 0; }
+  __device__ __forceinline__ int dist(int c) const { return a.pair_dist[c]; }
+  __device__ __forceinline__ int octave(int c) const { return a.kp[a.cand_idx[c]].octave; }
+  __device__ __forceinline__ int key(int i) const { return i; }
+  __device__ __forceinline__ int lowest(int r) const { return min_open[r]; }
+};
+#define CMS_TRACK_OCT_MAX 2047
+struct TrackGreedyLds {
+  const uint16_t* off; const uint32_t* cand; const uint8_t* tk; const int* min_open; int tag;
+  __device__ __forceinline__ int begin(int i) const { return off[i]; }
+  __device__ __forceinline__ int end(int i) const { return off[i + 1]; }
+  __device__ __forceinline__ int row(int c) const { return (int)(cand[c] & 0xFFFu); }
+  __device__ __forceinline__ bool taken(int r) const { return tk[r] != 0; }
+  __device__ __forceinline__ int dist(int c) const { return (int)((cand[c] >> 12) & 0x1FFu); }
+  __device__ __forceinline__ int octave(int c) const { return (int)(cand[c] >> 21); }
+  __device__ __forceinline__ int key(int i) const { return tag | i; }
+  __device__ __forceinline__ int lowest(int r) const { return min_open[r]; }
+};
+
+extern "C" __global__ void __launch_bounds__(CMS_TRACK_SLT) k_search_local(CmsSearchLocalArgs a) {
+  extern __shared__ int sl_lds[];
+  int* const min_open = sl_lds;
+  __shared__ int s_n[2];
+  __shared__ int s_bad;
+  const int f = blockIdx.x, tid = threadIdx.x, nt = CMS_TRACK_SLT;
   if (a.total && *a.total > a.cap) return;
   const int m0 = a.mp_off[f], m1 = a.mp_off[f + 1];
   const int frame = a.wg_frame ? a.wg_frame[f] : f + a.frame0;
   const int row0 = frame * a.kp_cap;
   int* const kp_mp = a.wg_frame ? a.kp_mp + ((ptrdiff_t)f - frame) * a.kp_cap : a.kp_mp;
+  const int nP = m1 - m0, cb = a.cand_off[m0], nC = a.cand_off[m1 > m0 ? m1 : m0] - cb;
+  bool resident = nP >= 0 && nC >= 0 && nP <= a.lds_points && nC <= a.lds_cands;
+  uint8_t* const tk = (uint8_t*)(sl_lds + CMS_TRACK_KPMAX);
+  uint32_t* const cand = (uint32_t*)(sl_lds + CMS_TRACK_KPMAX + CMS_TRACK_KPMAX / 4);
+  uint16_t* const off = (uint16_t*)(cand + a.lds_cands);
+  uint16_t* const list0 = off + ((a.lds_points + 2) & ~1);
+  if (resident) {
+    if (tid == 0) { s_bad = 0; s_n[0] = 0; }
+    for (int k = tid; k < a.kp_cap; k += nt) { min_open[k] = 0x7FFFFFFF; tk[k] = kp_mp[row0 + k] >= 0 ? 1 : 0; }
+    __syncthreads();
+    const int sub = tid & 3;
+    for (int i = tid >> 2; i < nP; i += nt >> 2) {
+      const int c0 = a.cand_off[m0 + i] - cb, c1 = a.cand_off[m0 + i + 1] - cb;
+      if (c0 < 0 || c1 < c0 || c1 > nC) { s_bad = 1; continue; }
+      if (sub == 0) off[i] = (uint16_t)c0;
+      if (c0 == c1) continue;
+      const uint4 q0 = a.mp_desc[2 * (size_t)(m0 + i)], q1 = a.mp_desc[2 * (size_t)(m0 + i) + 1];
+      for (int c = c0 + sub; c < c1; c += 4) {
+        const int row = a.cand_idx[cb + c], r = row - row0;
+        if (r < 0 || r >= a.kp_cap) { s_bad = 1; continue; }
+        const int oct = a.kp[row].octave;
+        if (oct < 0 || oct > CMS_TRACK_OCT_MAX) s_bad = 1;
+        const int dist = track_hamming256(q0, q1, a.t_desc[2 * (size_t)row], a.t_desc[2 * (size_t)row + 1]);
+        cand[c] = (uint32_t)r | ((uint32_t)dist << 12) | ((uint32_t)(oct & CMS_TRACK_OCT_MAX) << 21);
+      }
+    }
+    if (tid == 0) off[nP] = (uint16_t)nC;
+    __syncthreads();
+    if (s_bad) resident = false;
+  }
+  if (resident) {
+    for (int i = tid; i < nP; i += nt) {
+      if (off[i] == off[i + 1]) a.mp_match[m0 + i] = -1; else list0[atomicAdd(&s_n[0], 1)] = (uint16_t)i;
+    }
+    __syncthreads();
+    int cur = 0, round = 0;
+    for (;;) {
+      const int n = s_n[cur];
+      uint16_t* const L = list0 + (cur ? a.lds_points : 0);
+      uint16_t* const Lnext = list0 + (cur ? 0 : a.lds_points);
+      const TrackGreedyLds s = {off, cand, tk, min_open, (0x7FFF - round) << 16};
+      for (int j = tid; j < n; j += nt) track_greedy_claim(s, (int)L[j], min_open);
+      __syncthreads();
+      for (int j = tid; j < n; j += nt) { const int i = L[j]; if (track_greedy_ready(s, i)) L[j] = (uint16_t)(i | 0x8000); }
+      if (tid == 0) s_n[cur ^ 1] = 0;
+      __syncthreads();
+      for (int j = tid; j < n; j += nt) {
+        const int e = L[j];
+        if (!(e & 0x8000)) { Lnext[atomicAdd(&s_n[cur ^ 1], 1)] = (uint16_t)e; continue; }
+        const int i = e & 0x7FFF;
+        const int m = track_greedy_decide(s, i, a.nnratio, a.th_high);
+        if (m >= 0) { tk[m] = 1; kp_mp[row0 + m] = m0 + i; }
+        a.mp_match[m0 + i] = m >= 0 ? row0 + m : -1;
+      }
+      ++round;
+      __syncthreads();
+      if (s_n[cur ^ 1] == 0) break;
+      cur ^= 1;
+    }
+    if (a.rounds && tid == 0) a.rounds[f] = round;
+    return;
+  }
   {
     const int sub = tid & 3;
     for (int i = m0 + (tid >> 2); i < m1; i += nt >> 2) {
@@ -107,44 +231,25 @@
   }
   for (int i = m0 + tid; i < m1; i += nt) a.mp_match[i] = a.cand_off[i] == a.cand_off[i + 1] ? -1 : -2;
   __syncthreads();
+  const TrackGreedyGlobal g = {a, kp_mp, min_open, row0};
   int round = 0;
   for (;;) {
     for (int k = tid; k < a.kp_cap; k += nt) min_open[k] = 0x7FFFFFFF;
     __syncthreads();
-    for (int i = m0 + tid; i < m1; i += nt) {
-      if (a.mp_match[i] != -2) continue;
-      for (int c = a.cand_off[i]; c < a.cand_off[i + 1]; ++c) {
-        const int row = a.cand_idx[c];
-        if (kp_mp[row] < 0) atomicMin(&min_open[row - row0], i);
-      }
-    }
+    for (int i = m0 + tid; i < m1; i += nt)
+      if (a.mp_match[i] == -2) track_greedy_claim(g, i, min_open);
     __syncthreads();
     int open = 0;
     for (int i = m0 + tid; i < m1; i += nt) {
       if (a.mp_match[i] != -2) continue;
-      bool ok = true;
-      for (int c = a.cand_off[i]; c < a.cand_off[i + 1] && ok; ++c) {
-        const int row = a.cand_idx[c];
-        ok = kp_mp[row] >= 0 || min_open[row - row0] == i;
-      }
-      if (ok) a.mp_match[i] = -3; else ++open;
+      if (track_greedy_ready(g, i)) a.mp_match[i] = -3; else ++open;
     }
     __syncthreads();
     for (int i = m0 + tid; i < m1; i += nt) {
       if (a.mp_match[i] != -3) continue;
-      int bestDist = 256, bestLevel = -1, bestDist2 = 256, bestLevel2 = -1, bestRow = -1;
-      for (int c = a.cand_off[i]; c < a.cand_off[i + 1]; ++c) {
-        const int row = a.cand_idx[c];
-        if (kp_mp[row] >= 0) continue;
-        const int dist = a.pair_dist[c];
-        if (dist < bestDist) { bestDist2 = bestDist; bestDist = dist; bestLevel2 = bestLevel; bestLevel = a.kp[row].octave; bestRow = row; }
-        else if (dist < bestDist2) { bestLevel2 = a.kp[row].octave; bestDist2 = dist; }
-      }
-      int m = -1;
-      const bool ratio_ok = a.nnratio < 0.0f || !(bestLevel == bestLevel2 && (float)bestDist > __fmul_rn(a.nnratio, (float)bestDist2));
-      if (bestDist <= a.th_high && ratio_ok) m = bestRow;
-      if (m >= 0) kp_mp[m] = i;
-      a.mp_match[i] = m;
+      const int m = track_greedy_decide(g, i, a.nnratio, a.th_high);
+      if (m >= 0) kp_mp[row0 + m] = i;
+      a.mp_match[i] = m >= 0 ? row0 + m : -1;
     }
     ++round;
     if (__syncthreads_count(open > 0) == 0) break;
diff --git a/include/cubemapslam_hip.h b/include/cubemapslam_hip.h
--- a/include/cubemapslam_hip.h
+++ b/include/cubemapslam_hip.h
@@ -150,6 +150,7 @@
 
 int cms_area_set_keypoints(cms_ctx* ctx, int b, int n, const cms_keypoint* kps);
 int cms_area_grid(cms_ctx* ctx, int B);
+int cms_debug_area_grid(cms_ctx* ctx, int b, uint16_t* sorted_idx, int* cell_start, int* n_valid);
 int cms_features_in_area(cms_ctx* ctx, int b, int nq, const float* qx, const float* qy, const float* qr, const int* min_level,
                          const int* max_level, int* cand_off, int* cand_idx, int cap, int* total);
 int cms_features_in_area_device(cms_ctx* ctx, int b, int nq, const void* d_qx, const void* d_qy, const void* d_qr, const void* d_min_level,
@@ -180,6 +181,7 @@
 int cms_search_local_points_device(cms_ctx* ctx, int B, const void* d_mp_off, const void* d_mp_desc, const void* d_cand_off,
                                    const void* d_cand_idx, void* d_pair_dist, float nnratio, int th_high, void* d_kp_mp, void* d_mp_match,
                                    void* d_rounds);
+int cms_debug_search_local_budget(cms_ctx* ctx, int max_points, int max_cands);
 
 typedef struct {
   int n; const cms_keypoint* kps; const uint8_t* desc; const float* rays; const int* mp;
```
